# LepistaBioinformatics/classeq2

Measured on AMD Instinct MI355X. Metric: query placements/sec, 10k-leaf tree, 150 bp reads, higher is better.
Workload: dtype u64

## Files before the change

classeq2_amd/_abi.py:

```python

import ctypes as C

ABI_VERSION = 2
SETS_EXPLICIT, SETS_LEAVES = 0, 1

KIND_ROOT, KIND_NODE, KIND_LEAF = 0, 1, 2
NO_PARENT = (1 << 64) - 1

HAS_MAX_ITERATIONS = 1
HAS_MIN_MATCH_COVERAGE = 2
HAS_REMOVE_INTERSECTION = 4

(
    UNCLASSIFIABLE_NO_MATCH,
    UNCLASSIFIABLE_NO_ROOT,
    UNCLASSIFIABLE_COVERAGE,
    UNCLASSIFIABLE_LEVEL1,
    IDENTITY_FOUND,
    MAX_RESOLUTION,
    INCONCLUSIVE,
    ERR_TOO_FEW_KMERS,
    ERR_MAX_ITER,
    ERR_ROOT_NO_CHILDREN,
    ERR_INVALID_BASE,
    ERR_READ_TOO_LONG,
) = range(12)

STATUS_NAMES = [
    "UNCLASSIFIABLE_NO_MATCH",
    "UNCLASSIFIABLE_NO_ROOT",
    "UNCLASSIFIABLE_COVERAGE",
    "UNCLASSIFIABLE_LEVEL1",
    "IDENTITY_FOUND",
    "MAX_RESOLUTION",
    "INCONCLUSIVE",
    "ERR_TOO_FEW_KMERS",
    "ERR_MAX_ITER",
    "ERR_ROOT_NO_CHILDREN",
    "ERR_INVALID_BASE",
    "ERR_READ_TOO_LONG",
]


class Node(C.Structure):
    _fields_ = [
        ("id", C.c_uint64),
        ("parent", C.c_uint64),
        ("first_child", C.c_uint32),
        ("n_children", C.c_uint32),
        ("kind", C.c_uint8),
        ("has_children", C.c_uint8),
        ("pad_", C.c_uint8 * 6),
    ]


class DbDesc(C.Structure):
    _fields_ = [
        ("abi_version", C.c_uint32),
        ("n_nodes", C.c_uint32),
        ("nodes", C.POINTER(Node)),
        ("k_size", C.c_uint64),
        ("m_size", C.c_uint64),
        ("n_buckets", C.c_uint64),
        ("bucket_key", C.POINTER(C.c_uint64)),
        ("bucket_kmer_off", C.POINTER(C.c_uint64)),
        ("n_kmers", C.c_uint64),
        ("kmer_hash", C.POINTER(C.c_uint64)),
        ("kmer_node_off", C.POINTER(C.c_uint64)),
        ("node_ids", C.POINTER(C.c_uint64)),
        ("node_set_kind", C.c_uint32),
        ("pad_", C.c_uint32),
    ]


BUILD_REFERENCE_HEADER_SHIFT, BUILD_FORWARD_ONLY, BUILD_LEAVES_ONLY = 1, 2, 4


class BuildDesc(C.Structure):
    _fields_ = [
        ("abi_version", C.c_uint32),
        ("n_nodes", C.c_uint32),
        ("nodes", C.POINTER(Node)),
        ("k_size", C.c_uint64),
        ("m_size", C.c_uint64),
        ("n_records", C.c_uint32),
        ("flags", C.c_uint32),
        ("bases", C.c_void_p),
        ("offsets", C.POINTER(C.c_uint64)),
        ("leaf_id", C.POINTER(C.c_uint64)),
    ]


class KmersInfo(C.Structure):
    _fields_ = [
        ("n_windows", C.c_uint64),
        ("n_kmers", C.c_uint64),
        ("n_leaf_postings", C.c_uint64),
        ("n_node_ids", C.c_uint64),
        ("n_buckets", C.c_uint64),
        ("peak_device_bytes", C.c_uint64),
        ("ms_hash", C.c_double),
        ("ms_sort", C.c_double),
        ("ms_group", C.c_double),
        ("ms_d2h", C.c_double),
        ("ms_expand", C.c_double),
        ("sort_passes", C.c_uint32),
        ("full_key", C.c_uint32),
    ]


class Params(C.Structure):
    _fields_ = [
        ("flags", C.c_uint32),
        ("max_iterations", C.c_int32),
        ("min_match_coverage", C.c_double),
        ("remove_intersection", C.c_uint8),
        ("pad_", C.c_uint8 * 7),
    ]


class Placement(C.Structure):
    _fields_ = [
        ("status", C.c_uint8),
        ("pad_", C.c_uint8 * 3),
        ("one", C.c_int32),
        ("rest", C.c_int32),
        ("levels", C.c_uint32),
        ("clade_id", C.c_uint64),
    ]


class QueryStats(C.Structure):
    _fields_ = [
        ("n_query_kmers", C.c_uint32),
        ("n_matched", C.c_uint32),
        ("n_with_root", C.c_uint32),
        ("index_bytes", C.c_uint32),
        ("leaf_postings", C.c_uint64),
    ]


class DbInfo(C.Structure):
    _fields_ = [
        ("n_nodes", C.c_uint32),
        ("max_depth", C.c_uint32),
        ("max_nonleaf_arity", C.c_uint32),
        ("k_size", C.c_uint32),
        ("m_size", C.c_uint32),
        ("n_buckets", C.c_uint32),
        ("n_kmers", C.c_uint64),
        ("n_closed_kmers", C.c_uint64),
        ("table_slots", C.c_uint64),
        ("postings_words", C.c_uint64),
        ("hbm_bytes", C.c_uint64),
        ("max_read_kmers", C.c_uint32),
        ("device", C.c_int32),
        ("format", C.c_uint32),
        ("binary_tree", C.c_uint32),
        ("direct_table", C.c_uint32),
        ("n_tip_sets", C.c_uint32),
        ("scratch_slots", C.c_uint32),
# ... 103 lines not shown
```

classeq2_amd/csrc/cls_api.cpp:

```cpp
#include <hip/hip_runtime.h>
#include <ctype.h>
#include <stdio.h>
#include <stdlib.h>
#include <string.h>

#include <algorithm>
#include <mutex>
#include <new>
#include <string>
#include <thread>
#include <vector>

#include "cls_db.h"
#include "cls_device.h"
#include "cls_kernels.h"
#include "cls_pair.h"
#include "cls_place.h"
#include "cls_tally.h"
#include "cls_tuning.h"

namespace {

thread_local std::string g_err;

int fail(int code, const std::string& msg) {
    g_err = msg;
    return code;
}

#define CLS_HIP(expr)                                                                       \
    do {                                                                                    \
        hipError_t e_ = (expr);                                                             \
        if (e_ != hipSuccess) return fail(CLS_E_HIP, std::string(#expr) + ": " + hipGetErrorString(e_)); \
    } while (0)

struct Workspace {
    uint32_t* ptr = nullptr;
    uint64_t words = 0;
    hipEvent_t done = nullptr;
    hipStream_t stream = nullptr;
    uint64_t seq = 0;
    int launching = 0;
    bool busy = false;
    bool recorded = false;
};
struct TimedPair {
    hipEvent_t t0 = nullptr, t1 = nullptr;
    bool pending = false;
    bool in_use = false;
};
constexpr size_t MAX_WS_SLOTS = 8;
constexpr size_t MAX_TIMED_PAIRS = 256;

struct CallSlot {
    hipStream_t stream = nullptr;
    void *d_bases = nullptr, *d_off = nullptr, *d_out = nullptr, *d_stats = nullptr;
    uint64_t cap_bytes = 0;
    uint32_t cap_reads = 0, cap_stats = 0;
    bool busy = false;
};

cls::PlaceParams resolve(const cls_params* p) {
    cls::PlaceParams r;
    r.max_iterations = (p && (p->flags & CLS_HAS_MAX_ITERATIONS)) ? p->max_iterations : 1000;
    r.remove_intersection = (p && (p->flags & CLS_HAS_REMOVE_INTERSECTION)) ? (p->remove_intersection != 0) : 0;
    double c = 0.7;
    if (p && (p->flags & CLS_HAS_MIN_MATCH_COVERAGE)) {
        c = p->min_match_coverage;
        if (c > 1.0) c = 1.0; else if (c < 0.0) c = 0.0;
    }
    r.min_match_coverage = c;
    return r;
}

}

struct cls_db {
    int device = 0;
    int n_cu = 0;
    cls::DbDev dev{};
    cls_db_info info{};
    void* d_nodes = nullptr;
    void* d_kids = nullptr;
    void* d_table = nullptr;
    void* d_postings = nullptr;
    void* d_postings2 = nullptr;
    void* d_bucket_key = nullptr;
    void* d_mz_bucket = nullptr;
    void* d_direct = nullptr;
    void* d_direct16 = nullptr;
    void* d_sets = nullptr;
    void* d_sets2 = nullptr;
    std::mutex ws_mu;
    uint64_t max_read_len = 0;
    double kernel_ms_sum = 0.0;
    uint64_t kernel_launches = 0;
    std::vector<Workspace> ws;
    std::vector<TimedPair> timed;
    uint64_t ws_seq = 0;
    std::vector<CallSlot> calls;
    struct TreeRow { uint64_t id; uint32_t pre, size; };
    std::vector<TreeRow> tree_rows;
};

namespace cls {
Tuning& tuning() {
    static Tuning t;
    return t;
}
}
namespace {
struct Knob { const char* name; int cls::Tuning::*field; };
const Knob KNOBS[] = {
    {"no_fast", &cls::Tuning::no_fast}, {"no_order", &cls::Tuning::no_order}, {"force_list", &cls::Tuning::force_list},
    {"no_mask_halves", &cls::Tuning::no_mask_halves}, {"no_fat_direct", &cls::Tuning::no_fat_direct}, {"no_tile", &cls::Tuning::no_tile}, {"tile_pass_codes", &cls::Tuning::tile_pass_codes}, {"tile_set_words", &cls::Tuning::tile_set_words}, {"time_class", &cls::Tuning::time_class}, {"tile_one_per_cu", &cls::Tuning::tile_one_per_cu}, {"tile_min_kmers", &cls::Tuning::tile_min_kmers}, {"no_tile_order", &cls::Tuning::no_tile_order}, {"tile_deal", &cls::Tuning::tile_deal}, {"blocks_per_cu", &cls::Tuning::blocks_per_cu}, {"key_blocks_per_cu", &cls::Tuning::key_blocks_per_cu},
    {"long_blocks_per_cu", &cls::Tuning::long_blocks_per_cu}, {"order_mode", &cls::Tuning::order_mode},
    {"order_windows", &cls::Tuning::order_windows}, {"order_both_strands", &cls::Tuning::order_both_strands},
    {"order_block_shift", &cls::Tuning::order_block_shift}, {"order_sample_shift", &cls::Tuning::order_sample_shift},
    {"profile_stop", &cls::Tuning::profile_stop}, {"timing", &cls::Tuning::timing},
    {"build_full_key", &cls::Tuning::build_full_key}, {"tally_no_wave_combine", &cls::Tuning::tally_no_wave_combine},
};
}

extern "C" int cls_set_tuning(const char* name, int value) {
    if (!name) return fail(CLS_E_INVALID_ARG, "cls_set_tuning: null name");
    for (const Knob& k : KNOBS)
        if (strcmp(k.name, name) == 0) { cls::tuning().*(k.field) = value; return CLS_OK; }
    return fail(CLS_E_INVALID_ARG, std::string("cls_set_tuning: unknown knob ") + name);
}

extern "C" void cls_tuning_from_env(void) {
    for (const Knob& k : KNOBS) {
        std::string var = "CLS_";
        for (const char* c = k.name; *c; ++c) var += (char)toupper((unsigned char)*c);
        if (const char* v = getenv(var.c_str())) cls::tuning().*(k.field) = *v ? atoi(v) : 1;
    }
}

extern "C" const char* cls_last_error(void) { return g_err.c_str(); }
extern "C" void cls_internal_set_error(const char* msg) { g_err = msg ? msg : ""; }

extern "C" const char* cls_version(void) { return "classeq2_amd 0.1.0 gfx950 abi1"; }

extern "C" int cls_device_count(void) {
    int n = 0;
    if (hipGetDeviceCount(&n) != hipSuccess) return 0;
    return n;
}

extern "C" void cls_db_destroy(cls_db* db) {
    if (!db) return;
    int prev = 0;
    bool have_prev = hipGetDevice(&prev) == hipSuccess;
    (void)hipSetDevice(db->device);
    for (auto& w : db->ws) {
        if (w.done) { if (w.recorded) (void)hipEventSynchronize(w.done); (void)hipEventDestroy(w.done); }
        if (w.ptr) (void)hipFree(w.ptr);
    }
    for (auto& t : db->timed) {
        if (t.t0) (void)hipEventDestroy(t.t0);
        if (t.t1) (void)hipEventDestroy(t.t1);
    }
    for (auto& c : db->calls) {
        if (c.stream) { (void)hipStreamSynchronize(c.stream); (void)hipStreamDestroy(c.stream); }
        for (void* p : {c.d_bases, c.d_off, c.d_out, c.d_stats}) if (p) (void)hipFree(p);
    }
    if (db->d_nodes) (void)hipFree(db->d_nodes);
    if (db->d_kids) (void)hipFree(db->d_kids);
    if (db->d_table) (void)hipFree(db->d_table);
    if (db->d_postings) (void)hipFree(db->d_postings);
    if (db->d_postings2) (void)hipFree(db->d_postings2);
    if (db->d_bucket_key) (void)hipFree(db->d_bucket_key);
    if (db->d_mz_bucket) (void)hipFree(db->d_mz_bucket);
    if (db->d_direct) (void)hipFree(db->d_direct);
    if (db->d_direct16) (void)hipFree(db->d_direct16);
    if (db->d_sets) (void)hipFree(db->d_sets);
    if (db->d_sets2) (void)hipFree(db->d_sets2);
    if (have_prev) (void)hipSetDevice(prev);
    delete db;
}

static int encode(const cls_db_desc* d, cls::EncodedDb& E, const char* who) {
    std::string err;
    int rc = cls::encode_db(d, E, err);
    if (rc != CLS_OK) return fail(rc, std::string(who) + ": " + err);
    if (E.format == cls::FMT_LIST && E.postings.size() >= (1ULL << 32)) return fail(CLS_E_BAD_DB, std::string(who) + ": sorted-list postings exceed 2^32 words");
    return CLS_OK;
}

static int upload(const cls::EncodedDb& E, uint32_t n_buckets, int device, cls_db** out) {
    *out = nullptr;
    int n_dev = 0;
    if (hipGetDeviceCount(&n_dev) != hipSuccess || n_dev == 0)
        return fail(CLS_E_NO_DEVICE, "cls_db_create: no HIP device is visible (the placement path has no CPU fallback)");
    if (device < 0) CLS_HIP(hipGetDevice(&device));
    if (device >= n_dev) return fail(CLS_E_INVALID_ARG, "cls_db_create: device ordinal out of range");
    CLS_HIP(hipSetDevice(device));
    hipDeviceProp_t prop;
    CLS_HIP(hipGetDeviceProperties(&prop, device));
    std::vector<cls_db::TreeRow> tree_rows(E.nodes.size());
    for (size_t r = 0; r < E.nodes.size(); ++r) tree_rows[E.desc_row[r]] = {E.nodes[r].id, E.nodes[r].pre, E.nodes[r].size};
    cls_db* db = new cls_db();
    db->device = device;
    db->n_cu = prop.multiProcessorCount;
    db->tree_rows = std::move(tree_rows);
    auto up = [&](void** dst, const void* src, size_t bytes) -> hipError_t {
        hipError_t e = hipMalloc(dst, bytes + 64);
        if (e != hipSuccess) return e;
        return bytes ? hipMemcpy(*dst, src, bytes, hipMemcpyHostToDevice) : hipSuccess;
    };
    hipError_t e;
    if ((e = up(&db->d_nodes, E.nodes.data(), E.nodes.size() * sizeof(cls::DNode))) != hipSuccess ||
        (e = up(&db->d_kids, E.kids.data(), E.kids.size() * 4)) != hipSuccess ||
        (e = up(&db->d_table, E.table.data(), E.table.size() * sizeof(cls::Slot))) != hipSuccess ||
        (e = up(&db->d_postings, E.postings.data(), E.postings.size() * 4)) != hipSuccess ||
        (!E.postings2.empty() && (e = up(&db->d_postings2, E.postings2.data(), E.postings2.size() * 4)) != hipSuccess) ||
        (e = up(&db->d_bucket_key, E.bucket_key.data(), E.bucket_key.size() * 8)) != hipSuccess ||
        (!E.mz_bucket.empty() && (e = up(&db->d_mz_bucket, E.mz_bucket.data(), E.mz_bucket.size() * 4)) != hipSuccess) ||
        (!E.direct.empty() && (e = up(&db->d_direct, E.direct.data(), E.direct.size() * 4)) != hipSuccess) ||
        (!E.direct16.empty() && (e = up(&db->d_direct16, E.direct16.data(), E.direct16.size() * 4)) != hipSuccess) ||
        (!E.sets.empty() && (e = up(&db->d_sets, E.sets.data(), E.sets.size() * sizeof(cls::SetRec))) != hipSuccess) ||
        (!E.sets2.empty() && (e = up(&db->d_sets2, E.sets2.data(), E.sets2.size() * sizeof(cls::SetRec))) != hipSuccess)) {
        cls_db_destroy(db);
        return fail(e == hipErrorOutOfMemory ? CLS_E_NOMEM : CLS_E_HIP, std::string("cls_db_create: upload failed: ") + hipGetErrorString(e));
    }
    cls::DbDev& v = db->dev;
    v.nodes = (const cls::DNode*)db->d_nodes;
    v.kids = (const uint32_t*)db->d_kids;
    v.table = (const cls::Slot*)db->d_table;
    v.postings = (const uint32_t*)db->d_postings;
    v.postings2 = (const uint32_t*)db->d_postings2;
    v.bucket_key = (const uint64_t*)db->d_bucket_key;
    v.mz_bucket = (const uint32_t*)db->d_mz_bucket;
    v.direct = (const uint32_t*)db->d_direct;
    v.direct16 = (const uint32_t*)db->d_direct16;
    v.sets = (const cls::SetRec*)db->d_sets;
    v.sets2 = (const cls::SetRec*)db->d_sets2;
    v.table_mask = E.table.size() - 1;
    v.n_nodes = (uint32_t)E.nodes.size();
    v.n_buckets = (uint32_t)E.bucket_key.size();
    v.k = E.k;
    v.m_eff = E.m_eff;
    v.max_nonleaf_arity = E.max_nonleaf_arity;
    v.format = E.format;
    v.binary_tree = E.strictly_binary ? 1u : 0u;
    v.canonical = E.canonical ? 1u : 0u;
    v.n_sets = (uint32_t)E.sets.size();
    v.set_bits = 1;
    while (v.set_bits < 32 && (1ull << v.set_bits) < (uint64_t)E.sets.size()) ++v.set_bits;
    v.addr32 = (E.postings.size() * 4 < (1ull << 32) && E.direct.size() * 4 < (1ull << 32) && E.sets.size() * sizeof(cls::SetRec) < (1ull << 32)) ? 1u : 0u;
    cls_db_info& i = db->info;
    i.n_nodes = v.n_nodes;
    i.max_depth = E.max_depth;
    i.max_nonleaf_arity = E.max_nonleaf_arity;
    i.k_size = E.k;
    i.m_size = E.m;
    i.n_buckets = n_buckets;
    i.n_kmers = E.n_kmers;
    i.n_closed_kmers = E.n_closed;
    i.table_slots = E.table.size();
    i.postings_words = E.postings.size();
    i.hbm_bytes = E.nodes.size() * sizeof(cls::DNode) + E.table.size() * sizeof(cls::Slot) + (E.postings.size() + E.postings2.size()) * 4 + E.bucket_key.size() * 8 + E.mz_bucket.size() * 4 + E.direct.size() * 4 + E.direct16.size() * 4 + (E.sets.size() + E.sets2.size()) * sizeof(cls::SetRec);
    i.device = device;
    i.format = E.format;
    i.binary_tree = E.strictly_binary ? 1u : 0u;
    i.direct_table = E.direct.empty() ? 0u : (E.canonical ? 2u : 1u);
    i.n_tip_sets = (uint32_t)E.n_sets;
    i.fat_direct_table = E.direct16.empty() ? 0u : 1u;
    *out = db;
    return CLS_OK;
}

extern "C" int cls_db_create(const cls_db_desc* d, int device, cls_db** out) {
    if (!out) return fail(CLS_E_INVALID_ARG, "cls_db_create: out is null");
    *out = nullptr;
    try {
        cls::EncodedDb E;
        int rc = encode(d, E, "cls_db_create");
        if (rc != CLS_OK) return rc;
        return upload(E, (uint32_t)d->n_buckets, device, out);
    } catch (const std::bad_alloc&) {
        return fail(CLS_E_NOMEM, "cls_db_create: out of host memory");
    } catch (const std::exception& ex) {
        return fail(CLS_E_INTERNAL, std::string("cls_db_create: ") + ex.what());
    } catch (...) {
        return fail(CLS_E_INTERNAL, "cls_db_create: unknown exception");
    }
}

extern "C" int cls_db_validate(const cls_db_desc* d) {
    try {
        cls::EncodedDb E;
        std::string err;
        int rc = cls::encode_db(d, E, err);
        if (rc != CLS_OK) return fail(rc, "cls_db_validate: " + err);
        return CLS_OK;
    } catch (const std::bad_alloc&) {
        return fail(CLS_E_NOMEM, "cls_db_validate: out of host memory");
    } catch (...) {
        return fail(CLS_E_INTERNAL, "cls_db_validate: unknown exception");
    }
}

static cls::PlacePlan device_plan(const cls_db* db, uint64_t n_bases, bool stats) {
    return cls::plan_place(db->dev, 4096, (uint32_t)db->n_cu, stats, (uint32_t)(2 * n_bases), n_bases ? 4096 : 0);
}

static uint64_t declared_read_len(const cls_db* db) {
    std::lock_guard<std::mutex> g(const_cast<cls_db*>(db)->ws_mu);
    return db->max_read_len;
}

extern "C" int cls_db_info_get(const cls_db* db, cls_db_info* info) {
    if (!db || !info) return fail(CLS_E_INVALID_ARG, "cls_db_info_get: null argument");
    try {
        uint32_t cap[cls::N_LISTS];
        device_plan(db, declared_read_len(db), false).class_caps(cap);
        cls_db* mdb = const_cast<cls_db*>(db);
        std::lock_guard<std::mutex> g(mdb->ws_mu);
        *info = db->info;
        info->scratch_slots = (uint32_t)db->ws.size();
        info->max_read_kmers = *std::max_element(cap, cap + cls::N_LISTS);
        return CLS_OK;
    } catch (...) {
        return fail(CLS_E_INTERNAL, "cls_db_info_get: unknown exception");
    }
}

extern "C" int cls_db_info_get2(const cls_db* db, void* info, size_t info_size) {
    if (!db || !info) return fail(CLS_E_INVALID_ARG, "cls_db_info_get2: null argument");
    cls_db_info full;
    const int rc = cls_db_info_get(db, &full);
    if (rc != CLS_OK) return rc;
    memcpy(info, &full, info_size < sizeof(full) ? info_size : sizeof(full));
    return CLS_OK;
}

static void harvest(cls_db* db, bool wait) {
    for (auto& t : db->timed) {
        if (!t.pending) continue;
        if (wait ? hipEventSynchronize(t.t1) != hipSuccess : hipEventQuery(t.t1) != hipSuccess) continue;
        float ms = 0.f;
        if (hipEventElapsedTime(&ms, t.t0, t.t1) == hipSuccess) { db->kernel_ms_sum += ms; db->kernel_launches++; }
        t.pending = false;
    }
}

static size_t acquire_timed(cls_db* db) {
    harvest(db, false);
    for (size_t i = 0; i < db->timed.size(); ++i)
        if (!db->timed[i].pending && !db->timed[i].in_use && db->timed[i].t0) { db->timed[i].in_use = true; return i; }
    if (db->timed.size() >= MAX_TIMED_PAIRS) return SIZE_MAX;
    TimedPair t;
    if (hipEventCreate(&t.t0) != hipSuccess) return SIZE_MAX;
    if (hipEventCreate(&t.t1) != hipSuccess) { (void)hipEventDestroy(t.t0); return SIZE_MAX; }
    t.in_use = true;
    db->timed.push_back(t);
    return db->timed.size() - 1;
}

static int acquire_ws(cls_db* db, uint64_t words, hipStream_t stream, size_t* slot, Workspace* use) {
    std::unique_lock<std::mutex> g(db->ws_mu);
    for (;;) {
        size_t oldest = SIZE_MAX;
        for (size_t i = 0; i < db->ws.size(); ++i) {
            Workspace& w = db->ws[i];
            if (w.busy && w.recorded && w.launching == 0 && hipEventQuery(w.done) == hipSuccess) w.busy = false;
            const bool same_stream = w.busy && w.recorded && w.launching == 0 && w.stream == stream && stream != hipStreamPerThread;
            if ((!w.busy || same_stream) && w.words >= words) {
                w.busy = true; w.recorded = false; w.launching = 1; w.stream = stream; w.seq = ++db->ws_seq;
                *slot = i; *use = w;
                return CLS_OK;
            }
            if (w.busy && w.recorded && w.launching == 0 && (oldest == SIZE_MAX || w.seq < db->ws[oldest].seq)) oldest = i;
        }
        for (size_t i = 0; i < db->ws.size();) {
            Workspace& w = db->ws[i];
            if (!w.busy) {
                (void)hipEventDestroy(w.done);
                (void)hipFree(w.ptr);
                db->ws.erase(db->ws.begin() + (ptrdiff_t)i);
                oldest = SIZE_MAX;
            } else ++i;
        }
        if (db->ws.size() < MAX_WS_SLOTS) break;
        if (oldest == SIZE_MAX) {
            for (size_t i = 0; i < db->ws.size(); ++i)
                if (db->ws[i].busy && db->ws[i].recorded && db->ws[i].launching == 0 && (oldest == SIZE_MAX || db->ws[i].seq < db->ws[oldest].seq)) oldest = i;
        }
        if (oldest == SIZE_MAX) {
            g.unlock();
            std::this_thread::yield();
            g.lock();
            continue;
        }
        hipEvent_t ev = db->ws[oldest].done;
        g.unlock();
        if (hipEventSynchronize(ev) != hipSuccess) return fail(CLS_E_HIP, "hipEventSynchronize failed while waiting for a scratch slot");
        g.lock();
    }
    Workspace w;
    if (hipMalloc((void**)&w.ptr, words * 4) != hipSuccess) return fail(CLS_E_NOMEM, "scratch workspace allocation failed");
    if (hipEventCreateWithFlags(&w.done, hipEventDisableTiming) != hipSuccess) {
        (void)hipFree(w.ptr);
        return fail(CLS_E_HIP, "hipEventCreate failed");
    }
    w.words = words;
    w.busy = true;
    w.recorded = false;
    w.launching = 1;
    w.stream = stream;
    w.seq = ++db->ws_seq;
    db->ws.push_back(w);
    *slot = db->ws.size() - 1;
    *use = w;
    return CLS_OK;
}

static constexpr uint64_t HARD_MAX_READ_LEN = 1ull << 25;

extern "C" int cls_db_set_max_read_len(cls_db* db, uint64_t n_bases) {
    if (!db) return fail(CLS_E_INVALID_ARG, "cls_db_set_max_read_len: null handle");
    if (n_bases > HARD_MAX_READ_LEN) return fail(CLS_E_INVALID_ARG, "cls_db_set_max_read_len: at most 2^25 bases per read");
    std::lock_guard<std::mutex> g(db->ws_mu);
    db->max_read_len = n_bases;
    return CLS_OK;
}

static int place_device(cls_db* db, const void* d_bases, const void* d_offsets, uint32_t n, const cls_params* params,
                        void* d_out, void* d_stats, hipStream_t stream, uint32_t long_cap, uint32_t n_long) {
    const cls::PlaceParams prm = resolve(params);
    const cls::PlacePlan plan = cls::plan_place(db->dev, n, (uint32_t)db->n_cu, d_stats != nullptr, long_cap, n_long);
    size_t slot = 0;
    Workspace use;
    int rc = acquire_ws(db, (plan.ws_bytes + 3) / 4, stream, &slot, &use);
    if (rc != CLS_OK) return rc;
    size_t tp = SIZE_MAX;
    hipEvent_t t0 = nullptr, t1 = nullptr;
    {
        std::lock_guard<std::mutex> g(db->ws_mu);
        tp = acquire_timed(db);
        if (tp != SIZE_MAX) { t0 = db->timed[tp].t0; t1 = db->timed[tp].t1; }
    }
    hipError_t e = cls::launch_place(db->dev, prm, plan, (const uint8_t*)d_bases, (const uint64_t*)d_offsets, n,
                                     (cls_placement*)d_out, (cls_query_stats*)d_stats, use.ptr, stream, t0, t1);
    bool record_failed = false;
    {
        std::lock_guard<std::mutex> g(db->ws_mu);
        if (tp != SIZE_MAX) { db->timed[tp].pending = (e == hipSuccess); db->timed[tp].in_use = false; }
        for (size_t i = 0; i < db->ws.size(); ++i)
            if (db->ws[i].ptr == use.ptr) { slot = i; break; }
        record_failed = hipEventRecord(db->ws[slot].done, stream) != hipSuccess;
    }
    if (record_failed) (void)hipStreamSynchronize(stream);
    {
        std::lock_guard<std::mutex> g(db->ws_mu);
        for (size_t i = 0; i < db->ws.size(); ++i)
            if (db->ws[i].ptr == use.ptr) { slot = i; break; }
        db->ws[slot].launching = 0;
        db->ws[slot].recorded = !record_failed;
        if (record_failed) db->ws[slot].busy = false;
    }
    if (e != hipSuccess) return fail(CLS_E_HIP, std::string("kernel launch failed: ") + hipGetErrorString(e));
    return CLS_OK;
}

extern "C" int cls_place_batch_device(cls_db* db, const void* d_bases, const void* d_offsets, uint32_t n,
                                      const cls_params* params, void* d_out, void* d_stats, void* hip_stream) {
    if (!db) return fail(CLS_E_INVALID_ARG, "cls_place_batch_device: null handle");
    if (n == 0) return CLS_OK;
    if (!d_offsets || !d_out) return fail(CLS_E_INVALID_ARG, "cls_place_batch_device: null buffer");
    int prev = 0;
    CLS_HIP(hipGetDevice(&prev));
    if (prev != db->device) CLS_HIP(hipSetDevice(db->device));
    int rc;
    try {
        uint64_t max_len;
        { std::lock_guard<std::mutex> g(db->ws_mu); max_len = db->max_read_len; }
        rc = place_device(db, d_bases, d_offsets, n, params, d_out, d_stats, (hipStream_t)hip_stream, (uint32_t)(2 * max_len), max_len ? n : 0);
    } catch (...) {
        rc = fail(CLS_E_INTERNAL, "cls_place_batch_device: unknown exception");
    }
    if (prev != db->device) (void)hipSetDevice(prev);
    return rc;
}

extern "C" int cls_db_kernel_name(const cls_db* db, char* buf, size_t len) {
    if (!db || !buf || !len) return fail(CLS_E_INVALID_ARG, "cls_db_kernel_name: null argument");
    try {
        snprintf(buf, len, "%s", device_plan(db, declared_read_len(db), false).timed_name.c_str());
        return CLS_OK;
    } catch (...) {
        return fail(CLS_E_INTERNAL, "cls_db_kernel_name: unknown exception");
    }
}

extern "C" int cls_db_read_classes(const cls_db* db, uint64_t n_bases, int stats, cls_read_class* out, int max, int* n_out) {
    if (!db || !n_out || max < 0 || (max > 0 && !out)) return fail(CLS_E_INVALID_ARG, "cls_db_read_classes: null argument");
    if (n_bases > HARD_MAX_READ_LEN) return fail(CLS_E_INVALID_ARG, "cls_db_read_classes: at most 2^25 bases per read");
    try {
        const cls::PlacePlan plan = device_plan(db, n_bases, stats != 0);
        uint32_t cap[cls::N_LISTS];
        plan.class_caps(cap);
        int n = 0;
        uint32_t below = 0;
        for (int c = 0; c < cls::N_LISTS; ++c) {
            if (c > 0 && cap[c] <= below) continue;
            below = cap[c];
            if (n < max) {
                out[n].list = (uint32_t)c;
                out[n].max_kmers = cap[c];
                snprintf(out[n].kernel, sizeof out[n].kernel, "%s", plan.class_kernel_name(db->dev, c, stats != 0).c_str());
            }
            ++n;
        }
        *n_out = n;
        return CLS_OK;
    } catch (...) {
        return fail(CLS_E_INTERNAL, "cls_db_read_classes: unknown exception");
    }
}

extern "C" int cls_db_kernel_time(cls_db* db, double* sum_ms, uint64_t* launches, int reset) {
    if (!db) return fail(CLS_E_INVALID_ARG, "cls_db_kernel_time: null handle");
    std::lock_guard<std::mutex> g(db->ws_mu);
    harvest(db, true);
    if (sum_ms) *sum_ms = db->kernel_ms_sum;
    if (launches) *launches = db->kernel_launches;
    if (reset) { db->kernel_ms_sum = 0.0; db->kernel_launches = 0; }
    return CLS_OK;
}

static int check_host_args(const char* bases, const uint64_t* offsets, uint32_t n, const cls_placement* out) {
    if (!offsets || !out || (!bases && offsets[n] != offsets[0])) return fail(CLS_E_INVALID_ARG, "cls_place_batch: null buffer");
    for (uint32_t i = 0; i < n; ++i)
        if (offsets[i] > offsets[i + 1]) return fail(CLS_E_INVALID_ARG, "cls_place_batch: offsets not monotone");
    return CLS_OK;
}

static int place_host_checked(cls_db* db, const char* bases, const uint64_t* offsets, uint32_t n, const cls_params* params,
                              cls_placement* out, cls_query_stats* stats);

static int place_host(cls_db* db, const char* bases, const uint64_t* offsets, uint32_t n, const cls_params* params,
                      cls_placement* out, cls_query_stats* stats) {
    if (!db) return fail(CLS_E_INVALID_ARG, "cls_place_batch: null handle");
    if (n == 0) return CLS_OK;
    const int rc = check_host_args(bases, offsets, n, out);
    if (rc != CLS_OK) return rc;
    return place_host_checked(db, bases, offsets, n, params, out, stats);
}

static int place_host_checked(cls_db* db, const char* bases, const uint64_t* offsets, uint32_t n, const cls_params* params,
                              cls_placement* out, cls_query_stats* stats) {
    int prev = 0;
    CLS_HIP(hipGetDevice(&prev));
    CLS_HIP(hipSetDevice(db->device));
    const uint32_t chunk_reads = 256u << 10;
    const uint64_t chunk_bytes = 256ull << 20;
    const bool two = n > chunk_reads || offsets[n] - offsets[0] > chunk_bytes;
    size_t ci[2] = {0, 0};
    CallSlot cs[2];
    const int n_slots = two ? 2 : 1;
    {
        std::lock_guard<std::mutex> g(db->ws_mu);
        for (int k = 0; k < n_slots; ++k) {
            size_t i = 0;
            while (i < db->calls.size() && db->calls[i].busy) ++i;
            if (i == db->calls.size()) db->calls.emplace_back();
            db->calls[i].busy = true;
            ci[k] = i;
            cs[k] = db->calls[i];
        }
    }
    auto cleanup = [&]() {
        for (int k = 0; k < n_slots; ++k) if (cs[k].stream) (void)hipStreamSynchronize(cs[k].stream);
        std::lock_guard<std::mutex> g(db->ws_mu);
        for (int k = 0; k < n_slots; ++k) { cs[k].busy = false; db->calls[ci[k]] = cs[k]; }
        (void)hipSetDevice(prev);
    };
#define CLS_TRY(expr)                                                                                     \
    do {                                                                                                  \
        hipError_t e_ = (expr);                                                                           \
        if (e_ != hipSuccess) { cleanup(); return fail(e_ == hipErrorOutOfMemory ? CLS_E_NOMEM : CLS_E_HIP, std::string(#expr) + ": " + hipGetErrorString(e_)); } \
    } while (0)
    try {
        std::vector<uint64_t> rel[2];
        struct Pending { bool on = false; uint32_t first = 0, cnt = 0; } pend[2];
        auto copy_out = [&](int k) -> hipError_t {
            if (!pend[k].on) return hipSuccess;
            pend[k].on = false;
            hipError_t e = hipMemcpyAsync(out + pend[k].first, cs[k].d_out, (size_t)pend[k].cnt * sizeof(cls_placement), hipMemcpyDeviceToHost, cs[k].stream);
            if (e == hipSuccess && stats)
                e = hipMemcpyAsync(stats + pend[k].first, cs[k].d_stats, (size_t)pend[k].cnt * sizeof(cls_query_stats), hipMemcpyDeviceToHost, cs[k].stream);
            return e;
        };
        int turn = 0;
        for (uint32_t first = 0; first < n; turn ^= (n_slots - 1)) {
            CallSlot& c = cs[turn];
            uint32_t cnt = 0;
            while (first + cnt < n && cnt < chunk_reads && (cnt == 0 || offsets[first + cnt + 1] - offsets[first] <= chunk_bytes)) ++cnt;
            const uint64_t nbytes = offsets[first + cnt] - offsets[first];
            CLS_TRY(copy_out(turn));
            if (!c.stream) CLS_TRY(hipStreamCreateWithFlags(&c.stream, hipStreamNonBlocking));
            if (nbytes > c.cap_bytes || !c.d_bases) {
                CLS_TRY(hipStreamSynchronize(c.stream));
                if (c.d_bases) { (void)hipFree(c.d_bases); c.d_bases = nullptr; c.cap_bytes = 0; }
                const uint64_t want = std::max<uint64_t>(nbytes + nbytes / 4, 1 << 16);
                CLS_TRY(hipMalloc(&c.d_bases, want));
                c.cap_bytes = want;
            }
            if (cnt > c.cap_reads) {
                CLS_TRY(hipStreamSynchronize(c.stream));
                for (void** pp : {&c.d_off, &c.d_out, &c.d_stats}) if (*pp) { (void)hipFree(*pp); *pp = nullptr; }
                c.cap_reads = c.cap_stats = 0;
                const uint32_t want = (uint32_t)std::max<uint64_t>((uint64_t)cnt + cnt / 4, 1024);
                CLS_TRY(hipMalloc(&c.d_off, ((size_t)want + 1) * 8));
                CLS_TRY(hipMalloc(&c.d_out, (size_t)want * sizeof(cls_placement)));
                c.cap_reads = want;
            }
            if (stats && c.cap_stats < c.cap_reads) {
                CLS_TRY(hipStreamSynchronize(c.stream));
                if (c.d_stats) { (void)hipFree(c.d_stats); c.d_stats = nullptr; }
                CLS_TRY(hipMalloc(&c.d_stats, (size_t)c.cap_reads * sizeof(cls_query_stats)));
                c.cap_stats = c.cap_reads;
            }
            std::vector<uint64_t>& ro = rel[turn];
            ro.resize((size_t)cnt + 1);
            for (uint32_t i = 0; i <= cnt; ++i) ro[i] = offsets[first + i] - offsets[first];
            uint64_t longest = 1;
            uint32_t n_long = 1;
            for (uint32_t i = 0; i < cnt; ++i) {
                const uint64_t len = ro[i + 1] - ro[i];
                const uint64_t nk = len < db->dev.k ? 0 : 2 * (len - db->dev.k + 1);
                longest = std::max(longest, std::min(len, HARD_MAX_READ_LEN));
                if (nk > cls::MAX_READ_KMERS) ++n_long;
// ... 1141 lines not shown
```

classeq2_amd/csrc/cls_db.cpp:

```cpp
#include "cls_db.h"

#include "cls_murmur.h"
#include "cls_tuning.h"

#include <stdio.h>
#include <stdlib.h>
#include <string.h>

#include <algorithm>
#include <atomic>
#include <chrono>
#include <exception>
#include <functional>
#include <mutex>
#include <thread>

namespace cls {

namespace {

struct WorkerError {
    std::mutex mu;
    std::exception_ptr first;
    void capture() { std::lock_guard<std::mutex> g(mu); if (!first) first = std::current_exception(); }
// ... 382 lines not shown
                    while (!stk.empty()) {
                        const uint32_t x = stk.back(); stk.pop_back();
                        pos[x] = next++;
                        const uint32_t l = L[x], r = R[x];
                        if (l) { span_lo[l] = span_lo[x]; span_hi[l] = x; }
                        if (r) { span_lo[r] = x; span_hi[r] = span_hi[x]; }
                        const bool left_heavy = (x - span_lo[x]) >= (span_hi[x] - x);
                        if (left_heavy) { if (r) stk.push_back(r); if (l) stk.push_back(l); }
                        else { if (l) stk.push_back(l); if (r) stk.push_back(r); }
                    }
                }
                auto at = [&](uint32_t i) { return (uint32_t)(base + pos[i]); };
                for (uint32_t i = 1; i < n; ++i) {
                    uint32_t* t = &recs[(size_t)at(i) * 4];
                    t[0] = tip[i - 1];
                    t[1] = L[i] ? at(L[i]) : 0;
                    t[2] = tip[i];
                    t[3] = R[i] ? at(R[i]) : 0;
                    if (mask_halves) {
                        uint32_t* u = &recs2[(size_t)at(i) * 4];
                        u[0] = t[0]; u[1] = t[1]; u[2] = t[2]; u[3] = t[3];
                        const uint32_t l0 = span_lo[i], r1 = span_hi[i];
                        if (tip[i - 1] - tip[l0] < MASK_HALF_SPAN) {
                            uint32_t bits = 0;
                            for (uint32_t j = l0; j < i; ++j) bits |= 1u << (tip[j] - tip[l0]);
                            u[0] = tip[i - 1] | MASK_HALF; u[1] = bits;
                        }
                        if (tip[r1 - 1] - tip[i] < MASK_HALF_SPAN) {
                            uint32_t bits = 0;
                            for (uint32_t j = i; j < r1; ++j) bits |= 1u << (tip[j] - tip[i]);
                            u[2] = tip[i] | MASK_HALF; u[3] = bits;
                        }
                    }
                }
                if (mask_halves && n && tip[n - 1] - tip[0] < MASK_HALF_SPAN) {
                    uint32_t bits = 0;
                    for (uint32_t j = 0; j < n; ++j) bits |= 1u << (tip[j] - tip[0]);
                    set_mask[g + 1] = bits;
                }
                uint32_t lg = 0;
                while (lg < 31 && (1u << lg) <= n) ++lg;
                SetRec& sr = E.sets[g + 1];
                sr.x = root ? at(root) : 0;
                sr.vlo_lg = n ? ((lg << DIRECT_TIP_BITS) | tip[0]) : 0xFFFFFFFFu;
                sr.vhi_root = (n ? tip[n - 1] : 0u) | ((w[0] & POST_HAS_ROOT) ? 0x80000000u : 0u);
                sr.n_leaf = w[1];
            }
        });
        E.postings.swap(recs);
        E.postings2.swap(recs2);
        if (mask_halves) {
            E.sets2.assign(E.sets.begin(), E.sets.end());
            parallel_chunks(NS + 1, nt, [&](unsigned, uint64_t lo, uint64_t hi) {
                for (uint64_t g = lo; g < hi; ++g)
                    if (set_mask[g]) { E.sets2[g].x = set_mask[g]; E.sets2[g].vhi_root |= FAT_X_IS_BITS; }
            });
        }
        lap("split trees");
    }
    uint64_t cap = 16;
    while (cap < 2 * NK) cap <<= 1;
    if (cap >= (1ULL << 32)) { err = "k-mer table exceeds 2^32 slots"; return CLS_E_BAD_DB; }
    const uint64_t mask = cap - 1;
    const bool split = E.format == FMT_SPLIT;
    E.table.assign(cap, split ? Slot{0, 0} : Slot{0, SLOT_EMPTY});
    {
        uint64_t* raw = reinterpret_cast<uint64_t*>(E.table.data());
        const uint64_t empty = split ? 0ull : SLOT_EMPTY;
        auto tier_of = [&](uint32_t sid) -> uint64_t { const uint32_t lg = E.sets[sid].vlo_lg >> DIRECT_TIP_BITS; return lg <= 3 ? 0 : lg <= 6 ? 1 : lg <= 9 ? 2 : 3; };
        parallel_chunks(NK, nt, [&](unsigned, uint64_t lo, uint64_t hi) {
            for (uint64_t j = lo; j < hi; ++j) {
                const uint64_t h = d->kmer_hash[j];
                const uint64_t val = split ? ((uint64_t)set_of[j] | (((uint64_t)bucket_of[j] | (tier_of(set_of[j]) << TIER_SHIFT)) << 32))
                                           : ((kmer_off[j] << LOC_BUCKET_BITS) | bucket_of[j]);
                for (uint64_t i = h & mask;; i = (i + 1) & mask) {
                    uint64_t expect = empty;
                    if (__atomic_load_n(&raw[2 * i + 1], __ATOMIC_RELAXED) == empty &&
                        __atomic_compare_exchange_n(&raw[2 * i + 1], &expect, val, false, __ATOMIC_ACQ_REL, __ATOMIC_RELAXED)) {
                        raw[2 * i] = h;
                        break;
                    }
                }
            }
        });
        std::atomic<bool> has_dup{false};
        std::atomic<uint64_t> dup{0};
        parallel_chunks(cap, nt, [&](unsigned, uint64_t lo, uint64_t hi) {
            for (uint64_t s = lo; s < hi; ++s) {
                if (raw[2 * s + 1] == empty) continue;
                const uint64_t h = raw[2 * s];
                for (uint64_t i = h & mask; i != s; i = (i + 1) & mask)
                    if (raw[2 * i] == h) { dup.store(h, std::memory_order_relaxed); has_dup.store(true, std::memory_order_relaxed); break; }
            }
        });
        if (has_dup.load()) { err = "k-mer hash " + std::to_string(dup.load()) + " occurs more than once in the index (unsupported)"; return CLS_E_BAD_DB; }
    }
    lap("hash table");
    if (split && d->k_size <= DIRECT_MAX_K && E.n_sets < SET_ID_MASK) {
        const uint32_t K = (uint32_t)d->k_size, M = (uint32_t)std::min<uint64_t>(d->m_size, d->k_size);
        const uint64_t n_codes = 1ULL << (2 * K);
        E.direct.assign(n_codes, 0);
        const TSlot* tab = reinterpret_cast<const TSlot*>(E.table.data());
        std::atomic<bool> foreign{false};
        std::atomic<uint64_t> found{0};
        parallel_chunks(n_codes, nt, [&](unsigned, uint64_t lo, uint64_t hi) {
            static const char LETTER[4] = {'A', 'C', 'T', 'G'};
            constexpr int B = 32;
            char buf[DIRECT_MAX_K + 1];
            uint64_t hs[B];
            uint64_t cnt = 0;
            for (uint64_t c0 = lo; c0 < hi; c0 += B) {
                const int nb = (int)std::min<uint64_t>(B, hi - c0);
                for (int q = 0; q < nb; ++q) {
                    const uint64_t code = c0 + q;
                    for (uint32_t i = 0; i < K; ++i) buf[i] = LETTER[(code >> (2 * i)) & 3];
                    hs[q] = murmur3_h1_bytes(buf, K);
                    __builtin_prefetch(&tab[hs[q] & mask]);
                }
                for (int q = 0; q < nb; ++q) {
                    const uint64_t code = c0 + q, h = hs[q];
                    for (uint64_t i = h & mask; tab[i].set != 0; i = (i + 1) & mask) {
                        if (tab[i].hash != h) continue;
                        for (uint32_t t = 0; t < M; ++t) buf[t] = LETTER[(code >> (2 * t)) & 3];
                        if (d->bucket_key[tab[i].bucket & (uint32_t)LOC_BUCKET_MASK] != (M ? murmur3_h1_bytes(buf, M) : 0ull)) foreign = true;
                        E.direct[code] = tab[i].set | (tab[i].bucket & ~SET_ID_MASK);
                        ++cnt;
                        break;
                    }
                }
            }
            found += cnt;
        });
        if (foreign.load() || found.load() != NK) HugeVec<uint32_t>().swap(E.direct);
        if (!E.direct.empty()) {
            std::atomic<bool> asym{false};
            parallel_chunks(n_codes, nt, [&](unsigned, uint64_t lo, uint64_t hi) {
                for (uint64_t code = lo; code < hi && !asym.load(std::memory_order_relaxed); ++code) {
                    uint64_t rc = 0;
                    for (uint32_t i = 0; i < K; ++i) rc |= (((code >> (2 * i)) & 3) ^ 2) << (2 * (K - 1 - i));
                    if (rc > code && E.direct[code] != E.direct[rc]) asym = true;
                }
            });
            E.canonical = !asym.load();
            if (K <= FAT_DIRECT_MAX_K && !tuning().no_fat_direct) {
                E.direct16.resize(4 * n_codes);
                parallel_chunks(n_codes, nt, [&](unsigned, uint64_t lo, uint64_t hi) {
                    for (uint64_t code = lo; code < hi; ++code) {
                        const uint32_t e = E.direct[code];
                        const SetRec& sr = E.sets[e & SET_ID_MASK];
                        uint32_t* o = &E.direct16[4 * code];
                        o[0] = sr.x; o[1] = sr.vlo_lg; o[2] = sr.vhi_root; o[3] = e;
                        const uint32_t bits = set_mask.empty() ? 0u : set_mask[e & SET_ID_MASK];
                        if (bits) { o[0] = bits; o[2] |= FAT_X_IS_BITS; }
                    }
                });
            }
        }
    }
    lap("direct table");
    E.bucket_key.assign(d->bucket_key, d->bucket_key + d->n_buckets);
    if (E.bucket_key.empty()) E.bucket_key.push_back(0);
    {
        const uint32_t M = (uint32_t)std::min<uint64_t>(d->m_size, d->k_size);
        std::unordered_map<uint64_t, uint32_t> by_key;
        bool distinct = true;
        for (uint64_t b = 0; b < d->n_buckets; ++b) distinct &= by_key.emplace(d->bucket_key[b], (uint32_t)b).second;
        if (M <= MZ_TABLE_MAX_M && distinct) {
            static const char LETTER[4] = {'A', 'C', 'T', 'G'};
            E.mz_bucket.assign((size_t)1 << (2 * M), MZ_NO_BUCKET);
            char buf[MZ_TABLE_MAX_M + 1];
            for (uint32_t code = 0; code < E.mz_bucket.size(); ++code) {
                for (uint32_t t = 0; t < M; ++t) buf[t] = LETTER[(code >> (2 * t)) & 3];
                const auto it = by_key.find(M ? murmur3_h1_bytes(buf, M) : 0ull);
                if (it != by_key.end()) E.mz_bucket[code] = it->second;
            }
        }
    }
    E.k = (uint32_t)d->k_size;
    E.m = (uint32_t)std::min<uint64_t>(d->m_size, UINT32_MAX);
    E.m_eff = (uint32_t)std::min<uint64_t>(d->m_size, d->k_size);
    E.n_kmers = NK;
    E.n_closed = n_closed.load();
    E.root_has_children = d->nodes[0].has_children != 0;
    return CLS_OK;
}

}

extern "C" int cls_db_debug_mask_halves(const cls_db_desc* d, uint64_t* counts) {
    try {
        cls::EncodedDb E;
        std::string err;
        const int rc = cls::encode_db(d, E, err);
        if (rc != CLS_OK) return rc;
        using namespace cls;
        counts[0] = counts[1] = counts[2] = 0;
        if (E.format != FMT_SPLIT || E.postings2.empty()) return CLS_OK;
        if (E.postings2.size() != E.postings.size()) return CLS_E_INTERNAL;
        const TipRec* recs = reinterpret_cast<const TipRec*>(E.postings.data());
        const TipRec* rec2 = reinterpret_cast<const TipRec*>(E.postings2.data());
        const uint64_t n_recs = E.postings.size() / 4;
        std::function<void(uint32_t, uint32_t, int, std::vector<uint32_t>&)> part = [&](uint32_t end_tip, uint32_t x, int side, std::vector<uint32_t>& out) {
            if (!x) { out.push_back(end_tip); return; }
            const TipRec& t = recs[x];
            part(t.tip_prev, t.l, 0, out);
            part(t.tip, t.r, 1, out);
            (void)side;
        };
        std::vector<uint32_t> tips;
        for (uint64_t x = 1; x + 1 < n_recs; ++x) {
            const TipRec& t = recs[x];
            const TipRec& u = rec2[x];
            if (t.tip_prev == 0 && t.tip == 0 && t.l == 0 && t.r == 0) continue;
            ++counts[0];
            for (int side = 0; side < 2; ++side) {
                const uint32_t end_tip = side ? t.tip : t.tip_prev, sub = side ? t.r : t.l;
                const uint32_t uw = side ? u.tip : u.tip_prev, ux = side ? u.r : u.l;
                tips.clear();
                part(end_tip, sub, side, tips);
                if (!std::is_sorted(tips.begin(), tips.end()) || (side ? tips.front() : tips.back()) != end_tip) return CLS_E_INTERNAL;
                const bool narrow = tips.back() - tips.front() < MASK_HALF_SPAN;
                if (uw & MASK_HALF) {
                    uint32_t bits = 0;
                    for (uint32_t v : tips) bits |= 1u << (v - tips.front());
                    if (!narrow || (uw & ~MASK_HALF) != end_tip || ux != bits) return CLS_E_INTERNAL;
                    ++counts[1];
                } else {
                    if (narrow || uw != end_tip || ux != sub) return CLS_E_INTERNAL;
                    ++counts[2];
                }
            }
        }
        return CLS_OK;
    } catch (const std::bad_alloc&) {
        return CLS_E_NOMEM;
    } catch (...) {
        return CLS_E_INTERNAL;
    }
}

extern "C" int cls_db_debug_members(const cls_db_desc* d, const uint64_t* hashes, const uint64_t* clade_ids, uint64_t n, uint8_t* out) {
    try {
        cls::EncodedDb E;
        std::string err;
        const int rc = cls::encode_db(d, E, err);
        if (rc != CLS_OK) return rc;
        using namespace cls;
        std::vector<std::pair<uint64_t, uint32_t>> id2row(E.nodes.size());
        for (uint32_t r = 0; r < E.nodes.size(); ++r) id2row[r] = {E.nodes[r].id, r};
        std::sort(id2row.begin(), id2row.end());
        const uint64_t mask = E.table.size() - 1;
        std::vector<uint32_t> tips, stk;
        for (uint64_t i = 0; i < n; ++i) {
            auto it = std::lower_bound(id2row.begin(), id2row.end(), std::make_pair(clade_ids[i], (uint32_t)0));
            if (it == id2row.end() || it->first != clade_ids[i]) { out[i] = 3; continue; }
            const DNode& c = E.nodes[it->second];
            const uint64_t h = hashes[i];
            bool found = false, has_root = false, closed = true;
            tips.clear();
            if (E.format == FMT_SPLIT) {
                const TSlot* tab = reinterpret_cast<const TSlot*>(E.table.data());
                for (uint64_t s = h & mask; tab[s].set != 0; s = (s + 1) & mask) {
                    if (tab[s].hash != h) continue;
                    found = true;
                    const SetRec& sr = E.sets[tab[s].set];
                    has_root = (sr.vhi_root >> 31) != 0;
                    if (sr.vlo_lg != 0xFFFFFFFFu) {
                        const uint32_t lo = sr.vlo_lg & DIRECT_TIP_MASK, hi = sr.vhi_root & 0x7FFFFFFFu;
                        if (!sr.x) { tips.push_back(lo); if (hi != lo) return CLS_E_INTERNAL; }
                        else {
                            const TipRec* recs = reinterpret_cast<const TipRec*>(E.postings.data());
                            std::vector<std::pair<uint32_t, int>> st{{sr.x, 0}};
                            tips.push_back(lo);
                            while (!st.empty()) {
                                auto [x, phase] = st.back();
                                st.pop_back();
                                const TipRec& t = recs[x];
                                if (phase == 0) { st.push_back({x, 1}); if (t.l) st.push_back({t.l, 0}); }
                                else { if (tips.back() != t.tip_prev) return CLS_E_INTERNAL; tips.push_back(t.tip); if (t.r) st.push_back({t.r, 0}); }
                            }
                            if (tips.back() != hi) return CLS_E_INTERNAL;
                        }
                    }
                    break;
                }
            } else {
                for (uint64_t s = h & mask; E.table[s].loc != SLOT_EMPTY; s = (s + 1) & mask) {
                    if (E.table[s].hash != h) continue;
                    found = true;
                    const uint32_t* w = &E.postings[E.table[s].loc >> LOC_BUCKET_BITS];
                    has_root = (w[0] & POST_HAS_ROOT) != 0;
                    closed = (w[0] & POST_CLOSED) != 0;
                    tips.assign(w + POST_HEADER_WORDS, w + POST_HEADER_WORDS + (w[0] & POST_LEN_MASK));
                    break;
                }
            }
            if (!found) { out[i] = 2; continue; }
            bool in = false;
            if (c.pre == 0) in = has_root;
            else if (closed) { auto t = std::lower_bound(tips.begin(), tips.end(), c.pre); in = t != tips.end() && *t < c.pre + c.size; }
            else in = std::binary_search(tips.begin(), tips.end(), c.pre);
            out[i] = in ? 1 : 0;
        }
        return CLS_OK;
    } catch (...) {
        return CLS_E_INTERNAL;
    }
}
```

classeq2_amd/csrc/cls_db.h:

```cpp
#pragma once
#include <stdlib.h>
#include <sys/mman.h>

#include <new>
#include <string>
#include <vector>

#include "cls_device.h"

namespace cls {

constexpr uint64_t MAX_K = 1024;

template <class T>
struct HugeAlloc {
    using value_type = T;
    HugeAlloc() = default;
    template <class U> HugeAlloc(const HugeAlloc<U>&) {}
    T* allocate(size_t n) {
        const size_t bytes = n * sizeof(T);
        if (bytes < (8u << 20)) { void* p = malloc(bytes ? bytes : 1); if (!p) throw std::bad_alloc(); return static_cast<T*>(p); }
        const size_t huge = 2u << 20, padded = (bytes + huge - 1) & ~(huge - 1);
        void* p = aligned_alloc(huge, padded);
        if (!p) throw std::bad_alloc();
        (void)madvise(p, padded, MADV_HUGEPAGE);
        return static_cast<T*>(p);
    }
    void deallocate(T* p, size_t) { free(p); }
    template <class U> bool operator==(const HugeAlloc<U>&) const { return true; }
    template <class U> bool operator!=(const HugeAlloc<U>&) const { return false; }
};
template <class T> using HugeVec = std::vector<T, HugeAlloc<T>>;

struct EncodedDb {
    std::vector<DNode> nodes;
    std::vector<uint32_t> desc_row;
    std::vector<uint32_t> kids;
    HugeVec<Slot> table;
    HugeVec<uint32_t> postings2;
    HugeVec<uint32_t> postings;
    uint32_t format = FMT_LIST;
    bool strictly_binary = false;
    bool canonical = false;
    std::vector<uint64_t> bucket_key;
    std::vector<uint32_t> mz_bucket;
    HugeVec<SetRec> sets;
    HugeVec<SetRec> sets2;
    HugeVec<uint32_t> direct;
    HugeVec<uint32_t> direct16;
    uint32_t k = 0, m = 0, m_eff = 0;
    uint32_t max_depth = 0, max_nonleaf_arity = 0;
    uint64_t n_kmers = 0, n_closed = 0;
    uint64_t n_sets = 0;
    bool root_has_children = false;
};

int encode_db(const cls_db_desc* d, EncodedDb& E, std::string& err);

}
```

classeq2_amd/csrc/cls_device.h:

```cpp
#pragma once
#include <stdint.h>

#include "cls_place.h"

namespace cls {

struct DNode {
    uint32_t pre;
    uint32_t size;
    uint32_t first_child;
    uint32_t n_nonleaf;
    uint64_t id;
    uint32_t split;
    uint32_t flags;
};
static_assert(sizeof(DNode) == 32, "DNode");

struct Slot {
    uint64_t hash;
    uint64_t loc;
};
static_assert(sizeof(Slot) == 16, "Slot");
constexpr uint64_t SLOT_EMPTY = ~0ULL;
struct TSlot {
    uint64_t hash;
    uint32_t set;
    uint32_t bucket;
};
constexpr int TIER_SHIFT = 30;
constexpr uint32_t MZ_TABLE_MAX_M = 8;
constexpr uint32_t MZ_NO_BUCKET = 0xFFFFFFFFu;
constexpr uint32_t SET_ID_MASK = (1u << TIER_SHIFT) - 1;
static_assert(sizeof(TSlot) == 16, "TSlot");
constexpr int LOC_BUCKET_BITS = 24;
constexpr uint64_t LOC_BUCKET_MASK = (1ULL << LOC_BUCKET_BITS) - 1;

constexpr uint32_t POST_HAS_ROOT = 1u << 31;
constexpr uint32_t POST_CLOSED = 1u << 30;
constexpr uint32_t POST_LEN_MASK = (1u << 30) - 1;
constexpr uint32_t POST_HEADER_WORDS = 2;

struct SetRec {
    uint32_t x;
    uint32_t vlo_lg;
    uint32_t vhi_root;
    uint32_t n_leaf;
};
static_assert(sizeof(SetRec) == 16, "SetRec");
constexpr uint32_t DIRECT_MAX_K = 15;
constexpr uint32_t FAT_DIRECT_MAX_K = 12;
constexpr uint32_t DIRECT_TIP_BITS = 27;
constexpr uint32_t DIRECT_TIP_MASK = (1u << DIRECT_TIP_BITS) - 1;
struct TipRec {
    uint32_t tip_prev;
    uint32_t l;
    uint32_t tip;
    uint32_t r;
};
static_assert(sizeof(TipRec) == 16, "TipRec");
constexpr uint32_t MASK_HALF = 0x80000000u;
constexpr uint32_t MASK_HALF_SPAN = 32;
constexpr uint32_t FAT_X_IS_BITS = 0x40000000u;

enum : uint32_t { FMT_LIST = 0, FMT_SPLIT = 1 };

struct DbDev {
    const DNode* nodes;
    const uint32_t* kids;
    const Slot* table;
    const uint32_t* postings;
    const uint32_t* postings2;
    const uint64_t* bucket_key;
    const uint32_t* mz_bucket;
    const uint32_t* direct;
    const uint32_t* direct16;
    const SetRec* sets;
    const SetRec* sets2;
    uint64_t table_mask;
    uint32_t n_nodes;
    uint32_t n_buckets;
    uint32_t k;
    uint32_t m_eff;
    uint32_t max_nonleaf_arity;
    uint32_t format;
    uint32_t addr32;
    uint32_t binary_tree;
    uint32_t canonical;
    uint32_t set_bits;
    uint32_t n_sets;
};

struct PlaceParams {
    int32_t max_iterations;
    uint32_t remove_intersection;
    double min_match_coverage;
};

constexpr uint32_t MAX_READ_KMERS = 64 * 8 * 16;

}
```

classeq2_amd/csrc/cls_kernels.h:

```cpp
#pragma once
#include <hip/hip_runtime.h>

#include <string>
#include <tuple>
#include <type_traits>
#include <utility>

#include "cls_device.h"

namespace cls {

template <int V> using Int = std::integral_constant<int, V>;
template <class F> auto with_bool(bool b, F&& f) { return b ? f(std::true_type{}) : f(std::false_type{}); }
template <class... V> std::string instance_name(const char* kernel, V...) {
    auto arg = [](auto v) { if constexpr (std::is_same_v<decltype(v), bool>) return std::string(v ? "true" : "false"); else return std::to_string(v); };
    std::string s = std::string(kernel) + "<";
    const char* sep = "";
    ((s += sep + arg(V::value), sep = ", "), ...);
    return s + ">";
}
template <class F> struct Pick {
    F* fn;
    size_t smem;
    std::string name;
};
template <class F, class... V> Pick<F> pick(F* fn, size_t smem, const char* kernel, V... v) { return {fn, smem, instance_name(kernel, v...)}; }
template <class... P, class... A>
hipError_t launch_kernel(void (*kfn)(P...), dim3 grid, dim3 block, size_t smem, hipStream_t stream, A&&... a) {
    static_assert(sizeof...(P) == sizeof...(A), "launch_kernel: one argument per kernel parameter");
    const void* f = reinterpret_cast<const void*>(kfn);
    hipError_t e = smem > 64 * 1024 ? hipFuncSetAttribute(f, hipFuncAttributeMaxDynamicSharedMemorySize, (int)smem) : hipSuccess;
    if (e == hipSuccess) {
        std::tuple<P...> v{P{std::forward<A>(a)}...};
        e = std::apply([&](auto&... x) { void* args[] = {&x...}; return hipLaunchKernel(f, grid, block, args, smem, stream); }, v);
    }
    if (e != hipSuccess) (void)hipGetLastError();
    return e;
}

struct TileCfg {
    uint32_t threads, grid, lookups, bases, cap_kmers, set_words, cap_entries;
    size_t smem;
    uint64_t scratch_off;
};
constexpr int TILE_MAX_SUB = 3;
struct TilePlan {
    TileCfg sub[TILE_MAX_SUB];
    uint32_t n_sub;
    TileCfg whole;
    uint64_t scratch_words;
    std::string name;
};

constexpr int N_LISTS = 8;

struct PlacePlan {
    uint32_t grid[2];
    uint32_t grid_blk;
    uint32_t grid_key;
    bool ordered;
    uint64_t keys_off_words;
    uint64_t sort_off_words;
    size_t sort_bytes;
    uint64_t child_off_words;
    uint32_t grid_long;
    uint32_t long_cap;
    uint32_t long_arity;
    uint64_t long_set;
    uint64_t long_stride_words;
    uint64_t long_off_words;
    uint32_t max_kmers;
    bool blk;
    bool tiled;
    TilePlan tile;
    uint32_t tile_from;
    uint64_t tile_off_words;
    enum Timed : uint8_t { TIME_CLASS0, TIME_BLOCK, TIME_TILE } timed;
    std::string timed_name;
    uint64_t ws_bytes;
    void class_caps(uint32_t (&cap)[N_LISTS]) const;
    std::string class_kernel_name(const DbDev& db, int c, bool stats) const;
};
bool tile_usable(const DbDev& db);
TilePlan tile_plan(const DbDev& db, bool stats, uint32_t from_kmers, uint32_t max_kmers, uint32_t n_reads, uint32_t n_cu);
std::string tile_kernel_name(const DbDev& db, bool stats, const TileCfg& c);
hipError_t tile_launch(const DbDev& db, const PlaceParams& prm, const TilePlan& p, bool stats, const uint8_t* d_bases, const uint64_t* d_offsets,
                       const uint32_t* const* sub_lists, const uint32_t* const* sub_lens, uint32_t* big_list, uint32_t* big_len,
                       cls_placement* d_out, cls_query_stats* d_stats, uint32_t* spill_list, uint32_t* spill_len, uint32_t* scratch, bool ordered, hipStream_t stream);
PlacePlan plan_place(const DbDev& db, uint32_t n_reads, uint32_t n_cu, bool stats, uint32_t long_cap, uint32_t n_long);
hipError_t launch_place(const DbDev& db, const PlaceParams& prm, const PlacePlan& plan, const uint8_t* d_bases,
                        const uint64_t* d_offsets, uint32_t n_reads, cls_placement* d_out, cls_query_stats* d_stats,
                        uint32_t* d_ws, hipStream_t stream, hipEvent_t ev_start, hipEvent_t ev_stop);

}
```

classeq2_amd/csrc/cls_kernels.hip:

```cpp
#include <hip/hip_runtime.h>
#include <stdlib.h>

#include <algorithm>
#include <type_traits>

#include "cls_device.h"
#include "cls_devutil.h"
#include "cls_kernels.h"
#include "cls_murmur.h"
#include "cls_sort.h"
#include "cls_tuning.h"

namespace cls {

namespace {

constexpr int WAVES_PER_BLOCK = 4;
#ifndef MIN_WAVES_PER_EU
#define MIN_WAVES_PER_EU 4
#endif
#ifndef FAST_MIN_WAVES
#define FAST_MIN_WAVES 5
#endif
#ifndef CLS_NARROW_CANON_BITS
// ... 1340 lines not shown
    uint32_t nm_lane = 0;
#pragma unroll
    for (int s = 0; s < LS; ++s) {
        sid[s] &= SET_ID_MASK;
        if (sid[s] != 0) {
            uint32_t pos = (key[s] * 2654435761u) >> (32 - tb);
#pragma unroll 1
            for (;;) {
                const uint32_t old = atomicCAS(&cx.set[pos], SET_EMPTY, key[s]);
                if (old == SET_EMPTY) break;
                if (old == key[s]) { sid[s] = 0; kw[s] = 0; break; }
                pos = (pos + 1) & ((1u << tb) - 1);
            }
        }
        nm_lane += sid[s] != 0 ? kw[s] : 0u;
    }
    if (profile_stop == 1) { write_record(out, r, 0xFE, (int32_t)(sid[0] + sid[LS - 1]), 0, 0, 0); return; }
    uint32_t pos[LS];
    uint32_t owner = 0;
#pragma unroll
    for (int s = 0; s < LS; ++s) {
        pos[s] = 0;
        if (sid[s] != 0) {
            uint32_t p = (sid[s] * 2654435761u) >> (32 - tb);
#pragma unroll 1
            for (;;) {
                const uint32_t old = atomicCAS(&cx.gkey[p], SET_EMPTY, sid[s]);
                if (old == SET_EMPTY) { owner |= 1u << s; break; }
                if (old == sid[s]) break;
                p = (p + 1) & ((1u << tb) - 1);
            }
            atomicAdd(&cx.gcnt[p], kw[s]);
            pos[s] = p;
        }
    }
    wave_sync();
#pragma unroll
    for (int s = 0; s < LS; ++s) pos[s] = ((owner >> s) & 1u) ? cx.gcnt[pos[s]] : 0u;
    wave_sync();
    const uint4* __restrict__ sets = reinterpret_cast<const uint4*>(db.sets2 ? db.sets2 : db.sets);
    uint32_t cnt = nm_lane;
    uint64_t leafp = 0;
    uint32_t n_sets = 0;
    constexpr int G = LS <= 4 ? LS : 4;
#pragma unroll
    for (int g0 = 0; g0 < LS; g0 += G) {
        uint4 sr[G];
#pragma unroll
        for (int i = 0; i < G; ++i) {
            const int s = g0 + i;
            const bool own = s < LS && ((owner >> s) & 1u);
            if constexpr (FAT) {
                const FatRec fr = frec[s < LS ? s : 0];
                sr[i] = own ? uint4{fr.x, fr.vlo_lg, fr.vhi_root, 0u} : uint4{0u, 0xFFFFFFFFu, 0u, 0u};
                if (STATS && own) sr[i].w = ldx<uint4, ADDR32>(sets, sid[s < LS ? s : 0]).w;
            } else {
                sr[i] = ldx<uint4, ADDR32>(sets, own ? sid[s < LS ? s : 0] : 0u);
                if (STATS && own) ib += 16;
            }
        }
#pragma unroll
        for (int i = 0; i < G; ++i) {
            const int s = g0 + i;
            if (s >= LS) continue;
            const uint32_t w = pos[s];
            cnt += ((sr[i].z >> 31) * w) << 16;
            if (STATS) leafp += (uint64_t)w * sr[i].w;
            const bool live = ((owner >> s) & 1u) && sr[i].y != 0xFFFFFFFFu;
            const uint64_t m = __ballot(live);
            if (live)
                cx.stage[n_sets + popc64(m & ((1ull << lane) - 1))] = uint4{sr[i].y & DIRECT_TIP_MASK, sr[i].z & DIRECT_TIP_MASK, sr[i].x,
                                                                              w | ((sr[i].z & FAT_X_IS_BITS) << 1)};
            n_sets += popc64(m);
        }
    }
    cnt = wave_sum(cnt);
    const uint32_t n_m = cnt & 0xFFFFu, n_root = cnt >> 16;
    if (STATS) {
        for (int o = 32; o > 0; o >>= 1) leafp += ((uint64_t)__shfl_xor((uint32_t)(leafp >> 32), o) << 32) | __shfl_xor((uint32_t)leafp, o);
        put_stats(nk, n_m, n_root, leafp);
    }
    if (profile_stop == 2) { write_record(out, r, 0xFE, (int32_t)n_sets, 0, 0, 0); return; }
    if (n_m == 0) { put_index_bytes(); write_record(out, r, CLS_UNCLASSIFIABLE_NO_MATCH, 0, 0, 0, 0); return; }
    if (n_root == 0) { put_index_bytes(); write_record(out, r, CLS_UNCLASSIFIABLE_NO_ROOT, 0, 0, 0, 0); return; }
    snode_t P = load_node(db.nodes, 0);
    if (STATS && lane == 0) ib += 32;
    if (!(P.s[7] & 1u)) { put_index_bytes(); write_record(out, r, CLS_ERR_ROOT_NO_CHILDREN, 0, 0, 0, 0); return; }
    {
        const double expected = round((double)n_m * prm.min_match_coverage);
        const uint64_t exp_usize = (expected != expected) ? 0ull : (uint64_t)expected;
        if ((uint64_t)n_root < exp_usize) { put_index_bytes(); write_record(out, r, CLS_UNCLASSIFIABLE_COVERAGE, (int32_t)n_root, 0, 0, 0); return; }
    }
    bool in_registers = false;
    if constexpr (!POLY) in_registers = uniform(n_sets) <= 128;
    constexpr bool REG2 = !POLY || MODE != 2;
    if (in_registers) descend_groups<ADDR32, POLY, STATS, false, REG2>(db, prm, cx, n_sets, P, r, out, ib);
    else descend_groups<ADDR32, POLY, STATS, true, REG2>(db, prm, cx, n_sets, P, r, out, ib);
    put_index_bytes();
}

template <int SLOTS, int SET_BITS, bool STATS, bool ADDR32, int MODE, bool POLY>
__global__ __launch_bounds__(64 * WAVES_PER_BLOCK, SLOTS > 5 ? FAST_MIN_WAVES_WIDE : POLY ? FAST_MIN_WAVES_POLY : FAST_MIN_WAVES) void place_fast_kernel(
    DbDev db, PlaceParams prm, const uint8_t* __restrict__ bases, const uint64_t* __restrict__ offsets,
    const uint32_t* __restrict__ list, const uint32_t* __restrict__ list_len, uint32_t list_n, uint32_t xcd_chunks,
    cls_placement* __restrict__ out, cls_query_stats* __restrict__ stats, uint32_t ascii_cap, uint32_t profile_stop) {
    extern __shared__ __align__(16) uint8_t smem[];
    const uint32_t wave = threadIdx.x >> 6;
    const uint32_t packed_words = MODE == 2 ? 0u : ((ascii_cap >> 4) + 2 + 3) & ~3u;
    constexpr bool FITS = (12u << SET_BITS) >= 16u * 64 * ((MODE == 1 || MODE == 4) ? (SLOTS + 1) / 2 : SLOTS);
    if constexpr (FITS) {
    const uint32_t per_wave = ascii_cap + 4u * packed_words + (12u << SET_BITS) + (POLY ? 12u * FAST_MAX_ARITY + 16u : 0u);
    FastCtx cx;
    cx.ascii = smem + wave * per_wave;
    cx.packed = reinterpret_cast<uint32_t*>(cx.ascii + ascii_cap);
    cx.set = cx.packed + packed_words;
    cx.gkey = cx.set + (1u << SET_BITS);
    cx.gcnt = cx.gkey + (1u << SET_BITS);
    cx.stage = reinterpret_cast<uint4*>(cx.set);
    cx.ccnt = cx.gcnt + (1u << SET_BITS);
    cx.conly = cx.ccnt + FAST_MAX_ARITY;
    cx.cpre = cx.conly + FAST_MAX_ARITY;
    if (xcd_chunks && SLOTS > FAST_SLOTS_NARROW && *list_len == 0) return;
    const uint32_t n_list = xcd_chunks ? list_n : *list_len;
    const uint32_t xcd = blockIdx.x & 7u, bpx = gridDim.x >> 3;
    const uint32_t chunk = xcd_chunks ? (n_list + 7u) >> 3 : n_list;
    const uint32_t first = xcd_chunks ? (blockIdx.x >> 3) * WAVES_PER_BLOCK + wave : blockIdx.x * WAVES_PER_BLOCK + wave;
    const uint32_t stride = (xcd_chunks ? bpx : gridDim.x) * WAVES_PER_BLOCK;
    const uint32_t origin = xcd_chunks ? xcd * chunk : 0u;
    constexpr uint32_t cap = 64 * SLOTS;
    for (uint32_t ql = first; ql < chunk; ql += stride) {
        const uint32_t q = origin + ql;
        if (q >= n_list) break;
        const uint32_t r = list[q];
        const uint64_t b0 = offsets[r], b1 = offsets[r + 1];
        if (xcd_chunks) {
            const uint64_t L64 = b1 - b0;
            if (L64 >= db.k && 2 * (L64 - db.k + 1) > cap) continue;
            if (SLOTS > FAST_SLOTS_NARROW && (L64 < db.k || 2 * (L64 - db.k + 1) <= 64 * FAST_SLOTS_NARROW)) continue;
        }
        place_read_fast<SLOTS, SET_BITS, STATS, ADDR32, MODE, POLY>(db, prm, cx, bases, b0, b1, r, out, stats, profile_stop);
        wave_sync();
    }
    }
}

__device__ __forceinline__ uint64_t make_order_key(uint32_t key_mode, uint32_t median, uint32_t mh_spec, uint32_t mh_all, uint32_t block_shift, uint32_t set_bits) {
    if (key_mode == 1) return ((uint64_t)(mh_all >> 12) << set_bits) | median;
    return ((uint64_t)(median >> block_shift) << 16) | (mh_spec >> 16);
}

template <int SLOTS, bool ADDR32, bool FWD, bool HASHED>
__global__ __launch_bounds__(64 * WAVES_PER_BLOCK) void order_key_kernel(DbDev db, const uint8_t* __restrict__ bases,
                                                                       const uint64_t* __restrict__ offsets, uint32_t n_reads,
                                                                       uint64_t* __restrict__ keys, uint32_t* __restrict__ idx,
                                                                       uint32_t ascii_cap, uint32_t key_mode,
                                                                       uint32_t block_shift, uint32_t sample_shift, uint32_t fwd_only,
                                                                       uint32_t key_cap) {
    extern __shared__ __align__(16) uint8_t smem[];
    const uint32_t wave = threadIdx.x >> 6, lane = threadIdx.x & 63;
    const uint32_t packed_words = HASHED ? 0u : ((ascii_cap >> 4) + 2 + 3) & ~3u;
    const uint32_t per_wave = ascii_cap + 4u * packed_words + 16u;
    FastCtx cx;
    cx.ascii = smem + wave * per_wave;
    cx.packed = reinterpret_cast<uint32_t*>(cx.ascii + ascii_cap);
    cx.set = cx.packed + packed_words;
    cx.gkey = cx.gcnt = nullptr;
    cx.stage = nullptr;
    const uint32_t gw = blockIdx.x * WAVES_PER_BLOCK + wave;
    const uint32_t n_waves = gridDim.x * WAVES_PER_BLOCK;
    for (uint32_t r = gw; r < n_reads; r += n_waves) {
        const uint64_t b0 = offsets[r], L64 = offsets[r + 1] - b0;
        uint64_t key = ~0ull;
        if (L64 >= db.k && 2 * (L64 - db.k + 1) <= (uint64_t)key_cap) {
            const uint32_t L = (uint32_t)std::min<uint64_t>(L64, 32 * SLOTS + db.k - 1), nf = L - db.k + 1, nk = 2 * nf;
            constexpr int LS = FWD ? (SLOTS + 1) / 2 : SLOTS;
            uint32_t e[LS], code[LS], kw[LS];
            bool valid_read;
            uint32_t ib_unused = 0;
            if constexpr (HASHED) valid_read = hash_front<LS, 0, ADDR32>(db, cx, bases, b0, L, nf, FWD ? nf : nk, e, code, kw, 0, ib_unused);
            else { FatRec unused[LS]; valid_read = fast_front<LS, 0, ADDR32>(db, cx, bases, b0, L, nf, FWD ? nf : nk, e, code, kw, unused, sample_shift, FWD); }
            if (valid_read) {
                uint32_t cand = 0, n_cand = 0;
                for (uint32_t tier = 0; tier < 4 && n_cand < 4; ++tier) {
                    cand = 0; n_cand = 0;
#pragma unroll
                    for (int s = 0; s < LS; ++s) {
                        const bool c = (e[s] & SET_ID_MASK) != 0 && (e[s] >> TIER_SHIFT) <= tier;
                        cand |= (c ? 1u : 0u) << s;
                        n_cand += popc64(__ballot(c));
                    }
                }
                if (n_cand) {
                    uint32_t rank = n_cand >> 1, prefix = 0;
                    for (int bit = (int)db.set_bits - 1; bit >= 0; --bit) {
                        uint32_t c0 = 0;
#pragma unroll
                        for (int s = 0; s < LS; ++s) {
                            const uint32_t t = e[s] & SET_ID_MASK;
                            const bool z = ((cand >> s) & 1u) && ((t ^ prefix) >> (bit + 1)) == 0 && !((t >> bit) & 1u);
                            c0 += popc64(__ballot(z));
                        }
                        if (rank >= c0) { rank -= c0; prefix |= 1u << bit; }
                    }
                    uint32_t mh = 0xFFFFFFFFu, mha = 0xFFFFFFFFu;
#pragma unroll
                    for (int s = 0; s < LS; ++s) {
                        const uint32_t hsh = mix32(code[s]);
                        if ((cand >> s) & 1u) mh = hsh < mh ? hsh : mh;
                        if ((e[s] & SET_ID_MASK) != 0) mha = hsh < mha ? hsh : mha;
                    }
                    for (int o = 32; o > 0; o >>= 1) {
                        const uint32_t o1 = __shfl_xor(mh, o), o2 = __shfl_xor(mha, o);
                        mh = o1 < mh ? o1 : mh;
                        mha = o2 < mha ? o2 : mha;
                    }
                    key = make_order_key(key_mode, prefix, mh, mha, block_shift, db.set_bits);
                }
            }
            wave_sync();
        }
        if (lane == 0) { keys[r] = key; idx[r] = r; }
    }
}

template <bool ADDR32>
__global__ __launch_bounds__(64 * WAVES_PER_BLOCK) void order_key_half_kernel(DbDev db, const uint8_t* __restrict__ bases,
                                                                            const uint64_t* __restrict__ offsets, uint32_t n_reads,
                                                                            uint64_t* __restrict__ keys, uint32_t* __restrict__ idx,
                                                                            uint32_t key_mode, uint32_t block_shift,
                                                                            uint32_t key_cap) {
    constexpr uint32_t MAXL = 64 + DIRECT_MAX_K - 1 + 1;
    constexpr uint32_t WORDS = (MAXL + 15) / 16 + 2;
    __shared__ __align__(16) uint8_t s_ascii[WAVES_PER_BLOCK * 2][(MAXL + 19) & ~3u];
    __shared__ uint32_t s_packed[WAVES_PER_BLOCK * 2][WORDS];
    const uint32_t wave = threadIdx.x >> 6, lane = threadIdx.x & 63, half = lane >> 5, hl = lane & 31;
    uint8_t* ascii = s_ascii[wave * 2 + half];
    uint32_t* packed = s_packed[wave * 2 + half];
    const uint32_t k = db.k;
    const uint32_t kmask = (1u << (2 * k)) - 1u;
    const uint32_t* __restrict__ direct = db.direct;
    const uint32_t pair0 = (blockIdx.x * WAVES_PER_BLOCK + wave) * 2, stride = gridDim.x * WAVES_PER_BLOCK * 2;
    auto half_of = [&](uint64_t m) { return (uint32_t)(m >> (32 * half)); };
    for (uint32_t r0 = pair0; r0 < n_reads; r0 += stride) {
        const uint32_t r = r0 + half;
        const bool have = r < n_reads;
        const uint64_t b0 = have ? offsets[r] : 0, L64 = have ? offsets[r + 1] - b0 : 0;
        const bool keyed = have && L64 >= k && 2 * (L64 - k + 1) <= (uint64_t)key_cap;
        const uint32_t L = keyed ? (uint32_t)std::min<uint64_t>(L64, 64 + k - 1) : 0, nf = keyed ? L - k + 1 : 0;
        bool bad = false;
        for (uint32_t i = hl; i < L; i += 32) {
            uint8_t c = bases[b0 + i];
            if (c >= 'a' && c <= 'z') c -= 32;
            bad |= !(c == 'A' || c == 'C' || c == 'G' || c == 'T');
            ascii[i] = c;
        }
        const bool ok = keyed && half_of(__ballot(bad)) == 0;
        wave_sync();
        for (uint32_t w = hl; w < (L + 15) / 16 + 1; w += 32) {
            uint32_t acc = 0;
#pragma unroll
            for (int q = 0; q < 4; ++q) {
                uint32_t t = *reinterpret_cast<const uint32_t*>(ascii + 16 * w + 4 * q);
                t = (t >> 1) & 0x03030303u;
                t = (t | (t >> 6) | (t >> 12) | (t >> 18)) & 0xFFu;
                acc |= t << (8 * q);
            }
            if (w < WORDS) packed[w] = acc;
        }
        wave_sync();
        uint32_t e[2], hs[2];
#pragma unroll
        for (int s = 0; s < 2; ++s) {
            const uint32_t p = hl + 32 * s;
            const bool valid = ok && p < nf;
            const uint32_t w = valid ? p >> 4 : 0, sh = valid ? (2 * p) & 31 : 0;
            const uint32_t d0 = packed[w], d1 = packed[w + 1];
            uint32_t code = (uint32_t)((((uint64_t)d1 << 32) | d0) >> sh) & kmask;
            uint32_t rcc = __builtin_bitreverse32(code ^ (0xAAAAAAAAu & kmask));
            rcc = ((rcc >> 1) & 0x55555555u) | ((rcc & 0x55555555u) << 1);
            rcc >>= (32 - 2 * k);
            code = rcc < code ? rcc : code;
            const uint32_t v = ldx<uint32_t, ADDR32>(direct, valid ? code : 0u);
            e[s] = valid ? v : 0u;
            hs[s] = mix32(code);
        }
        uint32_t cand = 0, n_cand = 0;
        for (uint32_t tier = 0; tier < 4; ++tier) {
            const bool need = n_cand < 4;
            uint32_t c_new = 0, n_new = 0;
#pragma unroll
            for (int s = 0; s < 2; ++s) {
                const bool c = (e[s] & SET_ID_MASK) != 0 && (e[s] >> TIER_SHIFT) <= tier;
                c_new |= (c ? 1u : 0u) << s;
                n_new += (uint32_t)__popc(half_of(__ballot(c)));
            }
            if (need) { cand = c_new; n_cand = n_new; }
            if (__ballot(n_cand < 4) == 0) break;
        }
        uint32_t rank = n_cand >> 1, prefix = 0;
        for (int bit = (int)db.set_bits - 1; bit >= 0; --bit) {
            uint32_t c0 = 0;
#pragma unroll
            for (int s = 0; s < 2; ++s) {
                const uint32_t t = e[s] & SET_ID_MASK;
                const bool z = ((cand >> s) & 1u) && ((t ^ prefix) >> (bit + 1)) == 0 && !((t >> bit) & 1u);
                c0 += (uint32_t)__popc(half_of(__ballot(z)));
            }
            if (rank >= c0) { rank -= c0; prefix |= 1u << bit; }
        }
        uint32_t mh = 0xFFFFFFFFu, mha = 0xFFFFFFFFu;
#pragma unroll
        for (int s = 0; s < 2; ++s) {
            if ((cand >> s) & 1u) mh = hs[s] < mh ? hs[s] : mh;
            if ((e[s] & SET_ID_MASK) != 0) mha = hs[s] < mha ? hs[s] : mha;
        }
        for (int o = 16; o > 0; o >>= 1) {
            const uint32_t o1 = __shfl_xor(mh, o), o2 = __shfl_xor(mha, o);
            mh = o1 < mh ? o1 : mh;
            mha = o2 < mha ? o2 : mha;
        }
        if (have && hl == 0) {
            keys[r] = (ok && n_cand) ? make_order_key(key_mode, prefix, mh, mha, block_shift, db.set_bits) : ~0ull;
            idx[r] = r;
        }
        wave_sync();
    }
}

constexpr int LONG_THREADS = 256;
constexpr int LONG_STATE_WORDS = 5;

constexpr uint32_t LONG_LDS_ARITY = 256;
struct LongSh {
    uint32_t acc[4];
    unsigned long long acc64;
    uint32_t n_next;
    uint32_t n_pass, n_best, best_row;
    int32_t best_diff, best_one, best_rest;
    uint32_t cpre[LONG_LDS_ARITY + 1];
    uint32_t cnt_l[LONG_LDS_ARITY], only_l[LONG_LDS_ARITY];
};

__device__ __forceinline__ uint32_t append_slot(bool keep, uint32_t* counter) {
    const uint32_t lane = threadIdx.x & 63;
    const uint64_t m = __ballot(keep);
    if (!m) return 0;
    const int leader = __ffsll((unsigned long long)m) - 1;
    uint32_t base = 0;
    if ((int)lane == leader) base = atomicAdd(counter, (uint32_t)__popcll(m));
    base = __shfl(base, leader);
    return base + (uint32_t)__popcll(m & ((1ull << lane) - 1));
}

template <int N>
__device__ __forceinline__ void long_sum(uint32_t (&v)[N], LongSh& sh) {
    __syncthreads();
    if (threadIdx.x < N) sh.acc[threadIdx.x] = 0;
    __syncthreads();
#pragma unroll
    for (int i = 0; i < N; ++i) {
        const uint32_t w = wave_sum(v[i]);
        if ((threadIdx.x & 63) == 0 && w) atomicAdd(&sh.acc[i], w);
    }
    __syncthreads();
#pragma unroll
    for (int i = 0; i < N; ++i) v[i] = sh.acc[i];
}

template <bool SPLIT, bool STATS>
__global__ __launch_bounds__(LONG_THREADS) void place_long_kernel(DbDev db, PlaceParams prm, const uint8_t* __restrict__ bases,
                                                                  const uint64_t* __restrict__ offsets,
                                                                  const uint32_t* __restrict__ list,
                                                                  const uint32_t* __restrict__ list_len,
                                                                  cls_placement* __restrict__ out, cls_query_stats* __restrict__ stats,
                                                                  uint32_t* __restrict__ ws, uint64_t ws_stride_words, uint32_t cap,
                                                                  uint32_t set_size, uint32_t arity_pad) {
    __shared__ LongSh sh;
    constexpr uint32_t NT = LONG_THREADS;
    const uint32_t tid = threadIdx.x, lane = tid & 63;
    uint32_t* const buf0 = ws + (size_t)blockIdx.x * ws_stride_words;
    uint32_t* const buf1 = buf0 + (size_t)LONG_STATE_WORDS * cap;
    uint32_t* const cnt = buf1 + (size_t)LONG_STATE_WORDS * cap;
    uint32_t* const only = cnt + arity_pad;
    uint32_t* const set = buf1;
    uint32_t* const ent = buf0 + 4 * (size_t)cap;
    const DNode* __restrict__ nodes = db.nodes;
    const uint32_t* __restrict__ post = db.postings;
    const uint4* __restrict__ recs = reinterpret_cast<const uint4*>(db.postings);
    const uint32_t k = db.k, m_eff = db.m_eff;
    const bool rm = prm.remove_intersection != 0;
    const uint32_t n_list = *list_len;
    for (uint32_t li = blockIdx.x; li < n_list; li += gridDim.x) {
        __syncthreads();
        const uint32_t r = list[li];
        const uint64_t b0 = offsets[r], L64 = offsets[r + 1] - b0;
        auto put_stats = [&](uint32_t nk_, uint32_t nm, uint32_t nr, uint64_t lp) {
            if (STATS && stats && tid == 0) {
                uint64_t* s = reinterpret_cast<uint64_t*>(stats + r);
                s[0] = (uint64_t)nk_ | ((uint64_t)nm << 32);
                s[1] = (uint64_t)nr;
                s[2] = lp;
            }
        };
        auto record = [&](uint32_t status, int32_t one, int32_t rest, uint32_t levels, uint64_t clade) {
            if (tid == 0) {
                uint64_t* o = reinterpret_cast<uint64_t*>(out + r);
                o[0] = (uint64_t)(status & 0xFF) | ((uint64_t)(uint32_t)one << 32);
                o[1] = (uint64_t)(uint32_t)rest | ((uint64_t)levels << 32);
                o[2] = clade;
            }
        };
        if (L64 < k) { put_stats(0, 0, 0, 0); record(CLS_ERR_TOO_FEW_KMERS, 0, 0, 0, 0); continue; }
        const uint64_t nk64 = 2 * (L64 - k + 1);
        if (nk64 > cap) { put_stats(nk64 > 0xFFFFFFFFull ? 0xFFFFFFFFu : (uint32_t)nk64, 0, 0, 0); record(CLS_ERR_READ_TOO_LONG, 0, 0, 0, 0); continue; }
        const uint32_t L = (uint32_t)L64, nf = L - k + 1, nk = 2 * nf;
        bool bad = false;
        for (uint32_t i = tid; i < L; i += NT) {
            uint8_t c = bases[b0 + i];
            if (c >= 'a' && c <= 'z') c -= 32;
            bad |= !(c == 'A' || c == 'C' || c == 'G' || c == 'T');
        }
        for (uint32_t i = tid; i < set_size; i += NT) set[i] = SET_EMPTY;
        if (__syncthreads_or(bad ? 1 : 0)) { put_stats(0, 0, 0, 0); record(CLS_ERR_INVALID_BASE, 0, 0, 0, 0); continue; }
        auto kmer_char = [&](uint32_t j, uint32_t t) -> uint8_t {
            const bool rc = j >= nf;
            uint8_t c = bases[b0 + (rc ? (L - 1 - (j - nf) - t) : (j + t))];
            if (c >= 'a' && c <= 'z') c -= 32;
            return rc ? (uint8_t)(c ^ ((c & 2) ? 0x04 : 0x15)) : c;
        };
        const bool use_direct = SPLIT && db.direct != nullptr;
        for (uint32_t j = tid; j < nk; j += NT) {
            if (use_direct) {
                uint32_t code = 0;
                for (uint32_t t = 0; t < k; ++t) code |= (uint32_t)((kmer_char(j, t) >> 1) & 3u) << (2 * t);
                const uint32_t sid = db.direct[code] & SET_ID_MASK;
                uint32_t e = SET_EMPTY;
                if (sid) {
                    uint32_t pos = (code * 2654435761u) & (set_size - 1);
                    for (;;) {
                        const uint32_t old = atomicCAS(&set[pos], SET_EMPTY, code);
                        if (old == SET_EMPTY) { e = sid; break; }
                        if (old == code) break;
                        pos = (pos + 1) & (set_size - 1);
                    }
                }
                ent[j] = e;
                continue;
            }
            const uint64_t h = murmur3_h1([&](uint32_t t) { return kmer_char(j, t); }, k);
            const uint64_t mz = murmur3_h1([&](uint32_t t) { return kmer_char(j, t); }, m_eff);
            bool hit = false;
            uint64_t loc = 0;
            uint32_t tidx = 0;
            uint64_t idx = h & db.table_mask;
            for (;;) {
                const Slot sl = db.table[idx];
                if (SPLIT ? (uint32_t)sl.loc == 0u : sl.loc == SLOT_EMPTY) break;
                if (sl.hash == h) { hit = true; loc = sl.loc; tidx = (uint32_t)idx; break; }
                idx = (idx + 1) & db.table_mask;
            }
            bool ok = false;
            if (hit) {
                const uint64_t bk = db.bucket_key[SPLIT ? (uint32_t)(loc >> 32) & (uint32_t)LOC_BUCKET_MASK : (uint32_t)(loc & LOC_BUCKET_MASK)];
                ok = bk == mz;
                if (!ok) {
                    for (uint32_t jj = 0; jj < nk && !ok; ++jj)
                        ok = murmur3_h1([&](uint32_t t) { return kmer_char(jj, t); }, m_eff) == bk;
                }
            }
            uint32_t e = SET_EMPTY;
            if (hit && ok) {
                uint32_t pos = (tidx * 2654435761u) & (set_size - 1);
                for (;;) {
                    const uint32_t old = atomicCAS(&set[pos], SET_EMPTY, tidx);
                    if (old == SET_EMPTY) { e = SPLIT ? (uint32_t)loc : (uint32_t)(loc >> LOC_BUCKET_BITS); break; }
                    if (old == tidx) break;
                    pos = (pos + 1) & (set_size - 1);
// ... 221 lines not shown
    if (threadIdx.x < N_LISTS) s_cnt[threadIdx.x] = 0;
    __syncthreads();
    const uint32_t lane = threadIdx.x & 63;
    const uint32_t first = blockIdx.x * (CLASSIFY_THREADS * CLASSIFY_PER_THREAD) + threadIdx.x;
    int cls_id[CLASSIFY_PER_THREAD];
    uint32_t pos[CLASSIFY_PER_THREAD], rd[CLASSIFY_PER_THREAD];
#pragma unroll
    for (int i = 0; i < CLASSIFY_PER_THREAD; ++i) {
        const uint32_t at = first + i * CLASSIFY_THREADS;
        const uint32_t r = (order && at < n_reads) ? order[at] : at;
        rd[i] = r;
        cls_id[i] = -1;
        pos[i] = 0;
        if (at < n_reads) {
            const uint64_t L = offsets[r + 1] - offsets[r];
            const uint64_t nk = L < k ? 0 : 2 * (L - k + 1);
#pragma unroll
            for (int c = N_LISTS - 1; c >= 0; --c) if (nk <= caps.cap[c]) cls_id[i] = c;
            if (cls_id[i] < 0) {
                uint64_t* o = reinterpret_cast<uint64_t*>(out + r);
                o[0] = CLS_ERR_READ_TOO_LONG; o[1] = 0; o[2] = 0;
                if (stats) {
                    uint64_t* st = reinterpret_cast<uint64_t*>(stats + r);
                    st[0] = nk > 0xFFFFFFFFull ? 0xFFFFFFFFull : nk; st[1] = 0; st[2] = 0;
                }
            }
        }
#pragma unroll
        for (int c = 0; c < N_LISTS; ++c) {
            const uint64_t m = __ballot(cls_id[i] == c);
            if (!m) continue;
            uint32_t base = 0;
            if (lane == 0) base = atomicAdd(&s_cnt[c], (uint32_t)__popcll(m));
            base = __shfl(base, 0);
            if (cls_id[i] == c) pos[i] = base + (uint32_t)__popcll(m & ((1ull << lane) - 1));
        }
    }
    __syncthreads();
    if (threadIdx.x < N_LISTS) s_base[threadIdx.x] = s_cnt[threadIdx.x] ? atomicAdd(&counts[threadIdx.x], s_cnt[threadIdx.x]) : 0u;
    __syncthreads();
#pragma unroll
    for (int i = 0; i < CLASSIFY_PER_THREAD; ++i) {
        const int c = cls_id[i];
        if (c >= 0) lists[(size_t)c * n_reads + s_base[c] + pos[i]] = rd[i];
    }
}

}

namespace {
constexpr int N_CLASSES = 2;
constexpr int BLK_WAVES = 8, BLK_SLOTS = 16, BLK_SET_BITS = 14;
constexpr int ORDER_KEY_BITS_MAX = TIER_SHIFT + 20;
int order_key_bits(const DbDev& db) {
    const Tuning& tn = tuning();
    const int bits = tn.order_mode == 1 ? (int)db.set_bits + 20 : std::max(1, (int)db.set_bits - tn.order_block_shift) + 16;
    return std::min<int>(64, bits + 1);
}
constexpr int CLS_SLOTS[N_CLASSES] = {5, 16};
constexpr int CLS_SET_BITS[N_CLASSES] = {9, 11};
constexpr int NARROW_CANON_BITS = CLS_NARROW_CANON_BITS;

bool use_fast(const DbDev& db);
bool use_order(const DbDev& db, uint32_t n_reads) {
    return use_fast(db) && !tuning().no_order && n_reads >= 4096;
}
bool use_fast(const DbDev& db) {
    const bool front = db.direct != nullptr || (db.addr32 && db.k <= 256);
    return db.format == FMT_SPLIT && (db.binary_tree || db.max_nonleaf_arity <= FAST_MAX_ARITY) && front && !tuning().no_fast;
}
int fast_mode(const DbDev& db) { return db.direct == nullptr ? 2 : (db.direct16 && db.addr32) ? (db.canonical ? 4 : 3) : db.canonical ? 1 : 0; }
bool mode_canonical(int mode) { return mode == 1 || mode == 4; }
int set_bits_of(const DbDev& db, int c) { return (c == 0 && use_fast(db) && mode_canonical(fast_mode(db))) ? NARROW_CANON_BITS : CLS_SET_BITS[c]; }
uint32_t seq_cap_of(const DbDev& db, int c) { return (2 * (64 * CLS_SLOTS[c] / 2 + db.k) + 15) & ~15u; }
uint32_t ascii_cap_of(const DbDev& db, int c) {
    const uint32_t fwd = 64 * CLS_SLOTS[c] / 2 + db.k + 16;
    return ((db.direct ? fwd : 2 * fwd) + 15) & ~15u;
}
uint32_t child_ws_stride(const DbDev& db);
constexpr uint32_t CHILD_LDS_MAX = 256;
bool child_in_lds(const DbDev& db) { return child_ws_stride(db) != 0 && child_ws_stride(db) <= CHILD_LDS_MAX; }
size_t smem_of(const DbDev& db, int c) {
    if (use_fast(db)) {
        const uint32_t ac = ascii_cap_of(db, c);
        const uint32_t packed = db.direct ? 4u * (((ac >> 4) + 2 + 3) & ~3u) : 0u;
        return (size_t)WAVES_PER_BLOCK * (ac + packed + (12u << set_bits_of(db, c)) + (db.binary_tree ? 0u : 12u * FAST_MAX_ARITY + 16u));
    }
    return (size_t)WAVES_PER_BLOCK * (seq_cap_of(db, c) + (4u << CLS_SET_BITS[c]) + 4u * 64 * CLS_SLOTS[c]) +
           (child_in_lds(db) ? (size_t)WAVES_PER_BLOCK * 2 * child_ws_stride(db) * 4 : 0);
}

using FastFn = decltype(place_fast_kernel<CLS_SLOTS[0], CLS_SET_BITS[0], false, false, 0, false>);
using SplitFn = decltype(place_split_kernel<CLS_SLOTS[0], CLS_SET_BITS[0], false, false>);
using WaveFn = decltype(place_wave_kernel<CLS_SLOTS[0], CLS_SET_BITS[0], false, false>);
struct ClassKernel {
    FastFn* fast;
    SplitFn* split;
    WaveFn* wave;
    size_t smem;
    std::string name;
    const void* fn() const { return fast ? (const void*)fast : split ? (const void*)split : (const void*)wave; }
};
template <int SLOTS, int SET_BITS>
ClassKernel class_kernel_t(const DbDev& db, int c, bool stats) {
    const size_t smem = smem_of(db, c);
    auto fast = [&](auto... v) { return ClassKernel{place_fast_kernel<decltype(v)::value...>, nullptr, nullptr, smem, instance_name("place_fast_kernel", v...)}; };
    auto split = [&](auto... v) { return ClassKernel{nullptr, place_split_kernel<decltype(v)::value...>, nullptr, smem, instance_name("place_split_kernel", v...)}; };
    auto wave = [&](auto... v) { return ClassKernel{nullptr, nullptr, place_wave_kernel<decltype(v)::value...>, smem, instance_name("place_wave_kernel", v...)}; };
    const Int<SLOTS> sl;
    const Int<SET_BITS> sb;
    return with_bool(stats, [&](auto st) {
        if (use_fast(db)) {
            return with_bool(!db.binary_tree, [&](auto poly) {
                const std::true_type addr32;
                switch (fast_mode(db)) {
                    case 2: return fast(sl, sb, st, addr32, Int<2>{}, poly);
                    case 3: return fast(sl, sb, st, addr32, Int<3>{}, poly);
                    case 4: return fast(sl, sb, st, addr32, Int<4>{}, poly);
                }
                return with_bool(db.addr32, [&](auto a32) { return fast_mode(db) == 1 ? fast(sl, sb, st, a32, Int<1>{}, poly) : fast(sl, sb, st, a32, Int<0>{}, poly); });
            });
        }
        if (db.format == FMT_SPLIT) return with_bool(!db.binary_tree, [&](auto poly) { return split(sl, sb, st, poly); });
        return with_bool(db.max_nonleaf_arity <= 2, [&](auto binary) { return wave(sl, sb, st, binary); });
    });
}
ClassKernel class_kernel(const DbDev& db, int c, bool stats) {
    if (c == 1) return class_kernel_t<CLS_SLOTS[1], CLS_SET_BITS[1]>(db, 1, stats);
    if (set_bits_of(db, 0) != CLS_SET_BITS[0]) return class_kernel_t<CLS_SLOTS[0], NARROW_CANON_BITS>(db, 0, stats);
    return class_kernel_t<CLS_SLOTS[0], CLS_SET_BITS[0]>(db, 0, stats);
}

uint32_t child_ws_stride(const DbDev& db) {
    if (db.format == FMT_SPLIT) return db.binary_tree ? 0u : ((std::max(db.max_nonleaf_arity, 1u) + 63) & ~63u);
    return db.max_nonleaf_arity <= 2 ? 0u : ((db.max_nonleaf_arity + 63) & ~63u);
}
uint32_t blk_seq_cap(const DbDev& db) { return (2 * (64 * BLK_WAVES * BLK_SLOTS / 2 + db.k) + 15) & ~15u; }
auto block_kernel(const DbDev& db, bool stats) {
    const size_t smem = (size_t)blk_seq_cap(db) + (4u << BLK_SET_BITS) + 4u * 64 * BLK_WAVES * BLK_SLOTS + 64 +
                        (child_in_lds(db) ? (size_t)2 * child_ws_stride(db) * 4 : 0);
    auto inst = [&](auto... v) { return pick(place_block_kernel<decltype(v)::value...>, smem, "place_block_kernel", v...); };
    const bool split = db.format == FMT_SPLIT, binary = split ? db.binary_tree != 0 : db.max_nonleaf_arity <= 2;
    return with_bool(stats, [&](auto st) { return with_bool(binary, [&](auto bi) { return with_bool(split, [&](auto sp) {
        return inst(Int<BLK_WAVES>{}, Int<BLK_SLOTS>{}, Int<BLK_SET_BITS>{}, st, bi, sp);
    }); }); });
}
auto long_kernel(const DbDev& db, bool stats) {
    auto inst = [&](auto... v) { return pick(place_long_kernel<decltype(v)::value...>, 0, "place_long_kernel", v...); };
    return with_bool(db.format == FMT_SPLIT, [&](auto sp) { return with_bool(stats, [&](auto st) { return inst(sp, st); }); });
}

using KeyFn = decltype(order_key_kernel<2, true, true, false>);
using KeyHalfFn = decltype(order_key_half_kernel<true>);
struct KeyKernel {
    KeyFn* full;
    KeyHalfFn* half;
    size_t smem;
    std::string name;
    const void* fn() const { return full ? (const void*)full : (const void*)half; }
};
KeyKernel key_kernel(const DbDev& db, bool sizing) {
    const Tuning& tn = tuning();
    const bool fwd = !tn.order_both_strands, hashed = fast_mode(db) == 2;
    if (!sizing && !hashed && fwd && tn.order_windows == 64 && (uint32_t)tn.order_sample_shift >= 32)
        return with_bool(db.addr32, [&](auto a32) { return KeyKernel{nullptr, order_key_half_kernel<decltype(a32)::value>, 0, instance_name("order_key_half_kernel", a32)}; });
    const uint32_t ac = ascii_cap_of(db, 0);
    const size_t smem = (size_t)WAVES_PER_BLOCK * (ac + (db.direct ? 4u * (((ac >> 4) + 2 + 3) & ~3u) : 0u) + 16u);
    auto inst = [&](auto... v) { return KeyKernel{order_key_kernel<decltype(v)::value...>, nullptr, smem, instance_name("order_key_kernel", v...)}; };
    auto of = [&](auto a32, auto hs) {
        if (fwd && tn.order_windows <= 64) return inst(Int<2>{}, a32, std::true_type{}, hs);
        if (fwd || sizing) return inst(Int<CLS_SLOTS[0]>{}, a32, std::true_type{}, hs);
        return inst(Int<CLS_SLOTS[0]>{}, a32, std::false_type{}, hs);
    };
    if (hashed) return of(std::true_type{}, std::true_type{});
    return db.addr32 ? of(std::true_type{}, std::false_type{}) : of(std::false_type{}, std::false_type{});
}
}

void PlacePlan::class_caps(uint32_t (&cap)[N_LISTS]) const {
    for (uint32_t& c : cap) c = 0;
    cap[0] = (uint32_t)(64 * CLS_SLOTS[0]);
    if (max_kmers > cap[0]) cap[1] = (uint32_t)(64 * CLS_SLOTS[1]);
    if (max_kmers > (uint32_t)(64 * CLS_SLOTS[1])) cap[2] = tiled ? tile_from : (uint32_t)(64 * BLK_WAVES * BLK_SLOTS);
    if (tiled) {
        for (uint32_t i = 0; i < tile.n_sub; ++i) cap[3 + i] = tile.sub[i].cap_kmers;
        cap[6] = tile.whole.cap_kmers;
    }
    cap[7] = long_cap;
}

std::string PlacePlan::class_kernel_name(const DbDev& db, int c, bool stats) const {
    if (c < 2) return class_kernel(db, c, stats).name;
    if (c == 2) return block_kernel(db, stats).name;
    if (c < 6) return tile_kernel_name(db, stats, tile.sub[c - 3]);
    if (c == 6) return tile_kernel_name(db, stats, tile.whole);
    return long_kernel(db, stats).name;
}

PlacePlan plan_place(const DbDev& db, uint32_t n_reads, uint32_t n_cu, bool stats, uint32_t long_cap, uint32_t n_long) {
    PlacePlan p{};
    const int forced = tuning().blocks_per_cu;
    const uint32_t want = (n_reads + WAVES_PER_BLOCK - 1) / WAVES_PER_BLOCK;
    uint64_t child_words = 0;
    for (int c = 0; c < N_CLASSES; ++c) {
        int per_cu = forced;
        const ClassKernel k = class_kernel(db, c, stats);
        if (per_cu <= 0 && (hipOccupancyMaxActiveBlocksPerMultiprocessor(&per_cu, k.fn(), 64 * WAVES_PER_BLOCK, k.smem) != hipSuccess || per_cu <= 0))
            per_cu = 1;
        uint32_t cap = n_cu * (uint32_t)per_cu;
        if (child_ws_stride(db) && !child_in_lds(db)) {
            const uint64_t per_block = (uint64_t)WAVES_PER_BLOCK * 2 * child_ws_stride(db) * 4;
            const uint64_t fit = std::max<uint64_t>(1, (128ull << 20) / per_block);
            if (cap > fit) cap = (uint32_t)fit;
        }
        p.grid[c] = want < cap ? (want ? want : 1) : cap;
        if (!child_in_lds(db)) child_words = std::max<uint64_t>(child_words, (uint64_t)p.grid[c] * WAVES_PER_BLOCK * 2 * child_ws_stride(db));
    }
    p.grid_blk = std::max<uint32_t>(1, std::min<uint32_t>(n_reads, n_cu));
    if (!child_in_lds(db)) child_words = std::max<uint64_t>(child_words, (uint64_t)p.grid_blk * 2 * child_ws_stride(db));
    p.ordered = use_order(db, n_reads);
    uint64_t w = 16 + (uint64_t)N_LISTS * n_reads;
    w += w & 1;
    if (p.ordered) {
        p.grid[0] = std::max<uint32_t>(8, p.grid[0] & ~7u);
        p.grid[1] = std::max<uint32_t>(8, p.grid[1] & ~7u);
        {
            int per_cu = tuning().key_blocks_per_cu;
            const KeyKernel k = key_kernel(db, true);
            if (per_cu <= 0 && (hipOccupancyMaxActiveBlocksPerMultiprocessor(&per_cu, k.fn(), 64 * WAVES_PER_BLOCK, k.smem) != hipSuccess || per_cu <= 0)) per_cu = 4;
            if (tuning().key_blocks_per_cu <= 0 && fast_mode(db) == 2) per_cu *= 2;
            p.grid_key = std::max<uint32_t>(1, std::min<uint32_t>(want, n_cu * (uint32_t)per_cu));
        }
        p.keys_off_words = w;
        w += 6 * (uint64_t)n_reads;
        p.sort_off_words = w;
        p.sort_bytes = order_temp_bytes(n_reads);
        w += (p.sort_bytes + 3) / 4 + 2;
        w += w & 1;
    }
    p.child_off_words = w;
    w += child_words;
    w += w & 1;
    p.max_kmers = n_long ? std::max<uint32_t>(long_cap, 2u) : MAX_READ_KMERS;
    const uint32_t blk_cap = (uint32_t)(64 * BLK_WAVES * BLK_SLOTS);
    p.tile_from = blk_cap;
    if (tile_usable(db)) {
        p.tile_from = tuning().tile_min_kmers > 0 ? std::min<uint32_t>(blk_cap, (uint32_t)tuning().tile_min_kmers) : (uint32_t)(64 * CLS_SLOTS[1]);
        if (p.max_kmers > p.tile_from) {
            p.tile = tile_plan(db, stats, p.tile_from, p.max_kmers, n_reads, n_cu);
            p.tiled = p.tile.whole.cap_kmers > p.tile_from;
        }
    }
    if (p.tiled) {
        p.tile_off_words = w;
        w += p.tile.scratch_words;
        w += w & 1;
    } else p.tile_from = blk_cap;
    if (p.max_kmers > MAX_READ_KMERS || p.tiled) {
        long_cap = p.max_kmers;
        p.long_cap = long_cap;
        p.long_set = 1;
        while (p.long_set < 2 * (uint64_t)long_cap) p.long_set <<= 1;
        p.long_arity = (std::max(db.max_nonleaf_arity, 1u) + 63) & ~63u;
        p.long_stride_words = 2 * (uint64_t)LONG_STATE_WORDS * long_cap + 2 * (uint64_t)p.long_arity;
        const uint64_t fit = std::max<uint64_t>(1, (2ull << 30) / (p.long_stride_words * 4));
        const uint64_t per_cu_long = (uint64_t)std::max(1, tuning().long_blocks_per_cu);
        p.grid_long = (uint32_t)std::min<uint64_t>({(uint64_t)std::max<uint32_t>(1u, n_long ? n_long : n_reads), (uint64_t)n_cu * per_cu_long, fit});
        if (p.tiled && p.tile.whole.cap_kmers >= long_cap) p.grid_long = std::min<uint32_t>(p.grid_long, 8u);
        p.long_off_words = w;
        w += p.long_stride_words * p.grid_long;
    }
    p.ws_bytes = w * 4;
    p.blk = p.max_kmers > (uint32_t)(64 * CLS_SLOTS[1]) && (!p.tiled || p.tile_from > (uint32_t)(64 * CLS_SLOTS[1]));
    const bool gene = tuning().time_class == 2;
    p.timed = p.tiled && (p.max_kmers > MAX_READ_KMERS || gene) ? PlacePlan::TIME_TILE : p.blk && gene ? PlacePlan::TIME_BLOCK : PlacePlan::TIME_CLASS0;
    p.timed_name = p.timed == PlacePlan::TIME_TILE ? p.tile.name : p.timed == PlacePlan::TIME_BLOCK ? block_kernel(db, stats).name : class_kernel(db, 0, stats).name;
    return p;
}

hipError_t launch_place(const DbDev& db, const PlaceParams& prm, const PlacePlan& plan, const uint8_t* d_bases,
                        const uint64_t* d_offsets, uint32_t n_reads, cls_placement* d_out, cls_query_stats* d_stats,
                        uint32_t* d_ws, hipStream_t stream, hipEvent_t ev_start, hipEvent_t ev_stop) {
    if (n_reads == 0) return hipSuccess;
    uint32_t* counts = d_ws;
    uint32_t* lists[N_LISTS];
    for (int c = 0; c < N_LISTS; ++c) lists[c] = d_ws + 16 + (size_t)c * n_reads;
    uint32_t* child_ws = (child_ws_stride(db) && !child_in_lds(db)) ? d_ws + plan.child_off_words : nullptr;
    hipError_t e = hipMemsetAsync(counts, 0, 64, stream);
    if (e != hipSuccess) return e;
    const uint32_t profile_stop = (uint32_t)tuning().profile_stop;
    const uint32_t ws_stride = child_ws_stride(db);
    const bool st = d_stats != nullptr;
    auto classify = [&](const uint32_t* order) {
        ClassCaps caps{};
        plan.class_caps(caps.cap);
        return launch_kernel(classify_kernel, dim3((n_reads + CLASSIFY_THREADS * CLASSIFY_PER_THREAD - 1) / (CLASSIFY_THREADS * CLASSIFY_PER_THREAD)), dim3(CLASSIFY_THREADS), 0,
                             stream, d_offsets, order, n_reads, db.k, caps, lists[0], counts, d_out, d_stats);
    };
    const uint32_t* list0 = lists[0];
    uint32_t list0_n = 0, xcd_chunks = 0;
    if (!plan.ordered) e = classify(nullptr);
    else {
        uint64_t* keys_in = reinterpret_cast<uint64_t*>(d_ws + plan.keys_off_words);
        uint64_t* keys_out = keys_in + n_reads;
        uint32_t* idx_in = reinterpret_cast<uint32_t*>(keys_out + n_reads);
        uint32_t* idx_out = idx_in + n_reads;
        const Tuning& tn = tuning();
        const uint32_t key_mode = (uint32_t)tn.order_mode;
        const uint32_t block_shift = (uint32_t)tn.order_block_shift;
        const uint32_t key_cap = (plan.tiled && !tn.no_tile_order) ? 0xFFFFFFFFu : (uint32_t)(64 * CLS_SLOTS[1]);
        const KeyKernel k = key_kernel(db, false);
        const dim3 block(64 * WAVES_PER_BLOCK);
        if (k.half) {
            const uint32_t grid_half = std::max<uint32_t>(1, std::min<uint32_t>((n_reads + 2 * WAVES_PER_BLOCK - 1) / (2 * WAVES_PER_BLOCK), plan.grid_key));
            e = launch_kernel(k.half, dim3(grid_half), block, k.smem, stream, db, d_bases, d_offsets, n_reads, keys_in, idx_in, key_mode, block_shift, key_cap);
        } else {
            e = launch_kernel(k.full, dim3(plan.grid_key), block, k.smem, stream, db, d_bases, d_offsets, n_reads, keys_in, idx_in, ascii_cap_of(db, 0), key_mode,
                              block_shift, (uint32_t)tn.order_sample_shift, tn.order_both_strands ? 0u : 1u, key_cap);
        }
        if (e != hipSuccess) return e;
        e = order_reads(d_ws + plan.sort_off_words, keys_in, idx_out, n_reads, order_key_bits(db) - 1, stream);
        if (e != hipSuccess) return e;
        list0 = idx_out;
        list0_n = n_reads;
        xcd_chunks = 1;
        e = classify(idx_out);
    }
    if (e != hipSuccess) return e;
    auto launch_class = [&](int c) {
        const ClassKernel k = class_kernel(db, c, st);
        const dim3 grid(plan.grid[c]), block(64 * WAVES_PER_BLOCK);
        if (k.fast) {
            return launch_kernel(k.fast, grid, block, k.smem, stream, db, prm, d_bases, d_offsets, xcd_chunks ? list0 : lists[c], counts + c, list0_n, xcd_chunks,
                                 d_out, d_stats, ascii_cap_of(db, c), profile_stop);
        }
        if (k.split)
            return launch_kernel(k.split, grid, block, k.smem, stream, db, prm, d_bases, d_offsets, lists[c], counts + c, d_out, d_stats, seq_cap_of(db, c),
                                 profile_stop, child_ws, ws_stride);
        return launch_kernel(k.wave, grid, block, k.smem, stream, db, prm, d_bases, d_offsets, lists[c], counts + c, d_out, d_stats, seq_cap_of(db, c), child_ws,
                             ws_stride);
    };
    auto timed = [&](PlacePlan::Timed t, auto&& launch) {
        if (ev_start && plan.timed == t) (void)hipEventRecord(ev_start, stream);
        const hipError_t r = launch();
        if (ev_stop && plan.timed == t) (void)hipEventRecord(ev_stop, stream);
        return r;
    };
    e = timed(PlacePlan::TIME_CLASS0, [&] { return launch_class(0); });
    if (e != hipSuccess) return e;
    if (plan.max_kmers > (uint32_t)(64 * CLS_SLOTS[0])) {
        e = launch_class(1);
        if (e != hipSuccess) return e;
    }
    if (plan.blk) {
        const auto k = block_kernel(db, st);
        e = timed(PlacePlan::TIME_BLOCK, [&] {
            return launch_kernel(k.fn, dim3(plan.grid_blk), dim3(64 * BLK_WAVES), k.smem, stream, db, prm, d_bases, d_offsets, lists[2], counts + 2, d_out, d_stats,
                                 blk_seq_cap(db), child_ws, ws_stride);
        });
        if (e != hipSuccess) return e;
    }
    if (plan.tiled) {
        const uint32_t* sub_lists[TILE_MAX_SUB] = {lists[3], lists[4], lists[5]};
        const uint32_t* sub_lens[TILE_MAX_SUB] = {counts + 3, counts + 4, counts + 5};
        e = timed(PlacePlan::TIME_TILE, [&] {
            return tile_launch(db, prm, plan.tile, st, d_bases, d_offsets, sub_lists, sub_lens, lists[6], counts + 6, d_out, d_stats, lists[7], counts + 7,
                               d_ws + plan.tile_off_words, plan.ordered && !tuning().no_tile_order, stream);
        });
        if (e != hipSuccess) return e;
    }
    if (plan.grid_long) {
        const auto k = long_kernel(db, st);
        e = launch_kernel(k.fn, dim3(plan.grid_long), dim3(LONG_THREADS), k.smem, stream, db, prm, d_bases, d_offsets, lists[7], counts + 7, d_out, d_stats,
                          d_ws + plan.long_off_words, plan.long_stride_words, plan.long_cap, (uint32_t)plan.long_set, plan.long_arity);
    }
    return e;
}

}
```

classeq2_amd/csrc/cls_sort.h:

```cpp
#pragma once
#include <hip/hip_runtime.h>
#include <stddef.h>
#include <stdint.h>

namespace cls {
constexpr int ORDER_BIN_BITS = 12;
constexpr uint32_t ORDER_BINS = 1u << ORDER_BIN_BITS;
size_t order_temp_bytes(uint32_t n);
hipError_t order_reads(void* tmp, const uint64_t* keys, uint32_t* idx_out, uint32_t n, int key_bits, hipStream_t stream);
}
```

classeq2_amd/csrc/cls_sort.hip:

```cpp
#include "cls_sort.h"

namespace cls {

namespace {

constexpr int SORT_THREADS = 1024, SORT_PER_THREAD = 16;

__device__ __forceinline__ uint32_t bin_of(uint64_t key, int shift) {
    return key == ~0ull ? ORDER_BINS - 1 : (uint32_t)(key >> shift) & (ORDER_BINS - 1);
}

__global__ __launch_bounds__(SORT_THREADS) void order_hist_kernel(const uint64_t* __restrict__ keys, uint32_t n, int shift, uint32_t* __restrict__ hist,
                                                                 uint32_t* __restrict__ block_base) {
    __shared__ uint32_t h[ORDER_BINS];
    for (uint32_t i = threadIdx.x; i < ORDER_BINS; i += SORT_THREADS) h[i] = 0;
    __syncthreads();
    const uint32_t base = blockIdx.x * (SORT_THREADS * SORT_PER_THREAD);
#pragma unroll
    for (int q = 0; q < SORT_PER_THREAD; ++q) {
        const uint32_t r = base + q * SORT_THREADS + threadIdx.x;
        if (r < n) atomicAdd(&h[bin_of(keys[r], shift)], 1u);
    }
    __syncthreads();
    for (uint32_t i = threadIdx.x; i < ORDER_BINS; i += SORT_THREADS)
        block_base[(size_t)blockIdx.x * ORDER_BINS + i] = h[i] ? atomicAdd(&hist[i], h[i]) : 0u;
}

__global__ __launch_bounds__(1024) void order_scan_kernel(uint32_t* __restrict__ hist) {
    constexpr uint32_t PER = ORDER_BINS / 1024;
    __shared__ uint32_t wave_tot[16];
    uint32_t v[PER], sum = 0;
#pragma unroll
    for (uint32_t q = 0; q < PER; ++q) { v[q] = hist[threadIdx.x * PER + q]; sum += v[q]; }
    const uint32_t lane = threadIdx.x & 63, wave = threadIdx.x >> 6;
    uint32_t inc = sum;
#pragma unroll
    for (int o = 1; o < 64; o <<= 1) { const uint32_t t = __shfl_up(inc, o); if ((int)lane >= o) inc += t; }
    if (lane == 63) wave_tot[wave] = inc;
    __syncthreads();
    uint32_t before = 0;
    for (uint32_t w = 0; w < wave; ++w) before += wave_tot[w];
    uint32_t at = before + inc - sum;
#pragma unroll
    for (uint32_t q = 0; q < PER; ++q) { hist[threadIdx.x * PER + q] = at; at += v[q]; }
}

__global__ __launch_bounds__(SORT_THREADS) void order_scatter_kernel(const uint64_t* __restrict__ keys, uint32_t n, int shift, const uint32_t* __restrict__ start,
                                                                    const uint32_t* __restrict__ block_base, uint32_t* __restrict__ idx_out) {
    __shared__ uint32_t at[ORDER_BINS];
    for (uint32_t i = threadIdx.x; i < ORDER_BINS; i += SORT_THREADS) at[i] = start[i] + block_base[(size_t)blockIdx.x * ORDER_BINS + i];
    __syncthreads();
    const uint32_t base = blockIdx.x * (SORT_THREADS * SORT_PER_THREAD);
#pragma unroll
    for (int q = 0; q < SORT_PER_THREAD; ++q) {
        const uint32_t r = base + q * SORT_THREADS + threadIdx.x;
        if (r < n) idx_out[atomicAdd(&at[bin_of(keys[r], shift)], 1u)] = r;
    }
}

}

static uint32_t order_blocks(uint32_t n) { return (n + SORT_THREADS * SORT_PER_THREAD - 1) / (SORT_THREADS * SORT_PER_THREAD); }

size_t order_temp_bytes(uint32_t n) { return (1 + (size_t)order_blocks(n)) * ORDER_BINS * sizeof(uint32_t); }

hipError_t order_reads(void* tmp, const uint64_t* keys, uint32_t* idx_out, uint32_t n, int key_bits, hipStream_t stream) {
    uint32_t* hist = static_cast<uint32_t*>(tmp);
    uint32_t* block_base = hist + ORDER_BINS;
    const int shift = key_bits > ORDER_BIN_BITS ? key_bits - ORDER_BIN_BITS : 0;
    hipError_t e = hipMemsetAsync(hist, 0, ORDER_BINS * sizeof(uint32_t), stream);
    if (e != hipSuccess) return e;
    const uint32_t blocks = order_blocks(n);
    hipLaunchKernelGGL(order_hist_kernel, dim3(blocks), dim3(SORT_THREADS), 0, stream, keys, n, shift, hist, block_base);
    hipLaunchKernelGGL(order_scan_kernel, dim3(1), dim3(1024), 0, stream, hist);
    hipLaunchKernelGGL(order_scatter_kernel, dim3(blocks), dim3(SORT_THREADS), 0, stream, keys, n, shift, (const uint32_t*)hist, (const uint32_t*)block_base, idx_out);
    return hipGetLastError();
}

}
```

classeq2_amd/csrc/cls_tuning.h:

```cpp
#pragma once

namespace cls {

struct Tuning {
    int no_fast = 0;
    int no_order = 0;
    int force_list = 0;
    int no_mask_halves = 0;
    int no_fat_direct = 0;
    int no_tile = 0;
    int tile_pass_codes = 0;
    int tile_set_words = 0;
    int tile_min_kmers = 0;
    int tile_deal = 64;
    int no_tile_order = 0;
    int tile_one_per_cu = 0;
    int time_class = 0;
    int blocks_per_cu = 0;
    int key_blocks_per_cu = 0;
    int long_blocks_per_cu = 2;
    int order_mode = 0;
    int order_windows = 64;
    int order_both_strands = 0;
    int order_block_shift = 2;
    int order_sample_shift = 32;
    int profile_stop = 0;
    int timing = 0;
    int build_full_key = 0;
    int tally_no_wave_combine = 0;
};

Tuning& tuning();

}
```

classeq2_amd/engine.py:

```python

from __future__ import annotations

import ctypes as C
import os
from typing import Optional

import numpy as np

from . import _abi
from .flatdb import FlatDb

_HERE = os.path.dirname(os.path.abspath(__file__))
LIB_PATH = os.environ.get("CLS_PLACE_LIB") or os.path.join(_HERE, "csrc", "libclsplace.so")
_LIB = None

EXPORTS = [
    "cls_device_count", "cls_db_create", "cls_db_validate", "cls_db_destroy", "cls_db_info_get", "cls_db_info_get2", "cls_db_kernel_time", "cls_db_kernel_name",
    "cls_db_read_classes", "cls_db_set_max_read_len", "cls_place_batch",
    "cls_db_group_create", "cls_db_group_destroy", "cls_db_group_size", "cls_db_group_replica", "cls_place_batch_group", "cls_fasta_split",
    "cls_place_batch_device", "cls_place_batch_stats", "cls_fasta_parse", "cls_fasta_free", "cls_fasta_scan_device", "cls_fasta_dev_free",
    "cls_fasta_parse_gpu", "cls_place_fasta_text", "cls_fastq_parse", "cls_fastq_split", "cls_fastq_scan_device", "cls_fastq_parse_gpu",
    "cls_place_fastq_text", "cls_last_error",
    "cls_tally_create", "cls_tally_destroy", "cls_tally_reset", "cls_tally_add_device", "cls_tally_add", "cls_tally_read", "cls_tally_host",
    "cls_tally_merge", "cls_tally_fasta_text", "cls_tally_fastq_text",
    "cls_pairer_create", "cls_pairer_destroy", "cls_pairer_totals", "cls_pair_records_device", "cls_pair_records", "cls_pair_host",
    "cls_pair_names_host", "cls_pair_names_device", "cls_place_fastq_pairs_text", "cls_tally_fastq_pairs_text",
    "cls_version", "cls_set_tuning", "cls_tuning_from_env", "cls_kmers_build", "cls_kmers_desc", "cls_kmers_info_get", "cls_kmers_free",
]
HOST_EXPORTS = [
    "cls_tree_load_json", "cls_tree_load", "cls_tree_init_from_file", "cls_tree_from_newick", "cls_tree_serialize", "cls_tree_save", "cls_tree_free", "cls_tree_set_annotations_yaml", "cls_tree_build_kmers_map", "cls_tree_build_kmers_map_device", "cls_tree_desc", "cls_serialize_results",
    "cls_host_free", "cls_place_sequences", "cls_place_sequences_group", "cls_place_sequences_ex", "cls_place_sequences_group_ex",
    "cls_host_last_error", "cls_tally_report", "cls_profile_sequences", "cls_profile_sequences_group", "cls_place_sequences_report", "cls_tree_nodes",
    "cls_place_pairs",
]
SERVICE_EXPORTS = [
    "cls_service_create", "cls_service_destroy", "cls_service_add_model", "cls_service_submit", "cls_service_wait", "cls_service_pause",
    "cls_service_stats_get",
]
FORMAT_YAML, FORMAT_JSONL = 0, 1
DB_FORMAT_ZSTD, DB_FORMAT_YAML, DB_FORMAT_JSON = 0, 1, 2


class ClsError(RuntimeError):
    def __init__(self, code: int, msg: str):
        super().__init__(f"[{code}] {msg}")
        self.code = code
        self.msg = msg


def lib():
    global _LIB
    if _LIB is None:
        if not os.path.exists(LIB_PATH):
            raise RuntimeError(
                f"{LIB_PATH} is missing: build it with `python -c 'import __graft_entry__ as g; g.build()'` "
                "(the placement path has no CPU fallback)"
            )
        L = C.CDLL(LIB_PATH)
        vp, u32, i32 = C.c_void_p, C.c_uint32, C.c_int
        L.cls_device_count.restype = i32
        L.cls_db_create.argtypes = [C.POINTER(_abi.DbDesc), i32, C.POINTER(vp)]
        L.cls_db_create.restype = i32
        L.cls_db_validate.argtypes = [C.POINTER(_abi.DbDesc)]
        L.cls_db_validate.restype = i32
        L.cls_db_destroy.argtypes = [vp]
        L.cls_db_destroy.restype = None
        L.cls_db_info_get.argtypes = [vp, C.POINTER(_abi.DbInfo)]
        L.cls_db_info_get.restype = i32
        L.cls_db_kernel_time.argtypes = [vp, C.POINTER(C.c_double), C.POINTER(C.c_uint64), i32]
        L.cls_db_kernel_time.restype = i32
        L.cls_db_kernel_name.argtypes = [vp, C.c_char_p, C.c_size_t]
        L.cls_db_kernel_name.restype = i32
        L.cls_db_read_classes.argtypes = [vp, C.c_uint64, i32, C.POINTER(_abi.ReadClass), i32, C.POINTER(i32)]
        L.cls_db_read_classes.restype = i32
        L.cls_db_set_max_read_len.argtypes = [vp, C.c_uint64]
        L.cls_db_set_max_read_len.restype = i32
        L.cls_place_batch.argtypes = [vp, vp, vp, u32, C.POINTER(_abi.Params), vp]
        L.cls_place_batch.restype = i32
        L.cls_place_batch_stats.argtypes = [vp, vp, vp, u32, C.POINTER(_abi.Params), vp, vp]
        L.cls_place_batch_stats.restype = i32
        L.cls_place_batch_device.argtypes = [vp, vp, vp, u32, C.POINTER(_abi.Params), vp, vp, vp]
        L.cls_place_batch_device.restype = i32
        L.cls_db_group_create.argtypes = [C.POINTER(_abi.DbDesc), C.POINTER(i32), u32, C.POINTER(vp)]
        L.cls_db_group_create.restype = i32
        L.cls_db_group_destroy.argtypes = [vp]
        L.cls_db_group_destroy.restype = None
        L.cls_db_group_size.argtypes = [vp, C.POINTER(u32)]
        L.cls_db_group_size.restype = i32
        L.cls_db_group_replica.argtypes = [vp, u32, C.POINTER(vp)]
        L.cls_db_group_replica.restype = i32
        L.cls_place_batch_group.argtypes = [vp, vp, vp, u32, C.POINTER(_abi.Params), vp, vp]
        L.cls_place_batch_group.restype = i32
        L.cls_fasta_split.argtypes = [C.c_char_p, C.c_size_t, u32, C.POINTER(C.c_uint64), C.POINTER(u32)]
        L.cls_fasta_split.restype = i32
        L.cls_fasta_parse.argtypes = [C.c_char_p, C.c_size_t, C.POINTER(_abi.Fasta)]
        L.cls_fasta_parse.restype = i32
        L.cls_fasta_parse_gpu.argtypes = [C.c_char_p, C.c_size_t, i32, C.POINTER(_abi.Fasta)]
        L.cls_fasta_parse_gpu.restype = i32
        L.cls_place_fasta_text.argtypes = [vp, C.c_char_p, C.c_size_t, C.POINTER(_abi.Params), C.POINTER(_abi.Fasta), C.POINTER(vp)]
        L.cls_place_fasta_text.restype = i32
        L.cls_fastq_parse.argtypes = [C.c_char_p, C.c_size_t, C.POINTER(_abi.FastqOpts), C.POINTER(_abi.Fasta)]
        L.cls_fastq_parse.restype = i32
        L.cls_fastq_parse_gpu.argtypes = [C.c_char_p, C.c_size_t, C.POINTER(_abi.FastqOpts), i32, C.POINTER(_abi.Fasta)]
        L.cls_fastq_parse_gpu.restype = i32
        L.cls_fastq_split.argtypes = [C.c_char_p, C.c_size_t, u32, C.POINTER(C.c_uint64), C.POINTER(u32)]
        L.cls_fastq_split.restype = i32
        L.cls_place_fastq_text.argtypes = [vp, C.c_char_p, C.c_size_t, C.POINTER(_abi.Params), C.POINTER(_abi.FastqOpts), C.POINTER(_abi.Fasta),
                                           C.POINTER(vp)]
        L.cls_place_fastq_text.restype = i32
        L.cls_tally_create.argtypes = [vp, C.POINTER(vp)]
        L.cls_tally_create.restype = i32
        L.cls_tally_destroy.argtypes = [vp]
        L.cls_tally_destroy.restype = None
        L.cls_tally_reset.argtypes = [vp]
        L.cls_tally_reset.restype = i32
        L.cls_tally_add_device.argtypes = [vp, vp, u32, vp]
        L.cls_tally_add_device.restype = i32
        L.cls_tally_add.argtypes = [vp, vp, u32]
        L.cls_tally_add.restype = i32
        L.cls_tally_read.argtypes = [vp, vp, u32, vp]
        L.cls_tally_read.restype = i32
        L.cls_tally_host.argtypes = [vp, u32, vp, C.c_uint64, vp, vp]
        L.cls_tally_host.restype = i32
        L.cls_tally_merge.argtypes = [vp, vp, vp, vp, u32]
        L.cls_tally_merge.restype = i32
        L.cls_tally_fasta_text.argtypes = [vp, vp, C.c_char_p, C.c_size_t, C.POINTER(_abi.Params), C.POINTER(u32), C.POINTER(u32)]
        L.cls_tally_fasta_text.restype = i32
        L.cls_tally_fastq_text.argtypes = [vp, vp, C.c_char_p, C.c_size_t, C.POINTER(_abi.Params), C.POINTER(_abi.FastqOpts), C.POINTER(u32),
                                           C.POINTER(u32)]
        L.cls_tally_fastq_text.restype = i32
        u64 = C.c_uint64
        L.cls_pairer_create.argtypes = [vp, C.POINTER(vp)]
        L.cls_pairer_create.restype = i32
        L.cls_pairer_destroy.argtypes = [vp]
        L.cls_pairer_destroy.restype = None
        L.cls_pairer_totals.argtypes = [vp, vp, i32]
        L.cls_pairer_totals.restype = i32
        L.cls_pair_records_device.argtypes = [vp, vp, vp, u32, u32, u32, vp, vp, vp]
        L.cls_pair_records_device.restype = i32
        L.cls_pair_records.argtypes = [vp, vp, vp, u32, u32, u32, vp, vp]
        L.cls_pair_records.restype = i32
        L.cls_pair_host.argtypes = [vp, u32, vp, vp, u32, u64, u32, vp, vp, vp]
        L.cls_pair_host.restype = i32
        L.cls_pair_names_host.argtypes = [vp, vp, vp, vp, u32, u64, C.POINTER(u64), C.POINTER(u64)]
        L.cls_pair_names_host.restype = i32
        L.cls_pair_names_device.argtypes = [vp, vp, vp, vp, u32, u32, C.POINTER(u64), C.POINTER(u64), vp]
        L.cls_pair_names_device.restype = i32
        L.cls_place_fastq_pairs_text.argtypes = [vp, vp, C.c_char_p, C.c_size_t, C.c_char_p, C.c_size_t, C.POINTER(_abi.Params),
                                                 C.POINTER(_abi.FastqOpts), u32, C.POINTER(_abi.Fasta), C.POINTER(vp), C.POINTER(vp)]
        L.cls_place_fastq_pairs_text.restype = i32
        L.cls_tally_fastq_pairs_text.argtypes = [vp, vp, vp, C.c_char_p, C.c_size_t, C.c_char_p, C.c_size_t, C.POINTER(_abi.Params),
                                                 C.POINTER(_abi.FastqOpts), u32, C.POINTER(u32), C.POINTER(u32)]
        L.cls_tally_fastq_pairs_text.restype = i32
        L.cls_fasta_free.argtypes = [C.POINTER(_abi.Fasta)]
        L.cls_fasta_free.restype = None
        L.cls_last_error.restype = C.c_char_p
        L.cls_version.restype = C.c_char_p
        L.cls_set_tuning.argtypes = [C.c_char_p, i32]
        L.cls_set_tuning.restype = i32
        L.cls_tuning_from_env.argtypes = []
        L.cls_tuning_from_env.restype = None
        L.cls_kmers_build.argtypes = [C.POINTER(_abi.BuildDesc), i32, C.POINTER(vp)]
        L.cls_kmers_build.restype = i32
        L.cls_kmers_desc.argtypes = [vp, C.POINTER(_abi.BuildDesc), C.POINTER(_abi.DbDesc)]
        L.cls_kmers_desc.restype = i32
        L.cls_kmers_info_get.argtypes = [vp, C.POINTER(_abi.KmersInfo)]
        L.cls_kmers_info_get.restype = i32
        L.cls_kmers_free.argtypes = [vp]
        L.cls_kmers_free.restype = None
        L.cls_tree_load_json.argtypes = [C.c_char_p, C.POINTER(vp)]
        L.cls_tree_load_json.restype = i32
        L.cls_tree_load.argtypes = [C.c_char_p, C.POINTER(vp)]
        L.cls_tree_load.restype = i32
        L.cls_tree_init_from_file.argtypes = [C.c_char_p, C.c_double, C.POINTER(vp)]
        L.cls_tree_init_from_file.restype = i32
        L.cls_tree_from_newick.argtypes = [C.c_char_p, C.c_char_p, C.c_double, C.POINTER(vp)]
        L.cls_tree_from_newick.restype = i32
        L.cls_tree_serialize.argtypes = [vp, i32, i32, C.POINTER(vp), C.POINTER(C.c_size_t)]
        L.cls_tree_serialize.restype = i32
        L.cls_tree_save.argtypes = [vp, C.c_char_p, i32, i32]
        L.cls_tree_save.restype = i32
        L.cls_tree_free.argtypes = [vp]
        L.cls_tree_free.restype = None
        L.cls_tree_set_annotations_yaml.argtypes = [vp, C.c_char_p]
        L.cls_tree_set_annotations_yaml.restype = i32
        L.cls_tree_build_kmers_map.argtypes = [vp, C.c_char_p, C.c_size_t, C.c_uint64, C.c_uint64, u32]
        L.cls_tree_build_kmers_map.restype = i32
        L.cls_tree_build_kmers_map_device.argtypes = [vp, C.c_char_p, C.c_size_t, C.c_uint64, C.c_uint64, u32, i32]
        L.cls_tree_build_kmers_map_device.restype = i32
        L.cls_tree_desc.argtypes = [vp, C.POINTER(_abi.DbDesc)]
        L.cls_tree_desc.restype = i32
        L.cls_serialize_results.argtypes = [vp, C.c_char_p, vp, u32, vp, i32, C.POINTER(vp), C.POINTER(C.c_size_t),
                                            C.POINTER(vp), C.POINTER(C.c_size_t)]
        L.cls_serialize_results.restype = i32
        L.cls_host_free.argtypes = [vp]
        L.cls_host_free.restype = None
        L.cls_place_sequences.argtypes = [vp, vp, C.c_char_p, C.c_char_p, C.POINTER(_abi.Params), i32, i32,
                                          C.POINTER(u32), C.POINTER(C.c_double)]
        L.cls_place_sequences.restype = i32
        L.cls_place_sequences_group.argtypes = [vp, vp, C.c_char_p, C.c_char_p, C.POINTER(_abi.Params), i32, i32,
                                                C.POINTER(u32), C.POINTER(C.c_double)]
        L.cls_place_sequences_group.restype = i32
        for name in ("cls_place_sequences_ex", "cls_place_sequences_group_ex"):
            getattr(L, name).argtypes = [vp, vp, C.c_char_p, C.c_char_p, C.POINTER(_abi.Params), i32, i32, i32, C.POINTER(_abi.FastqOpts),
                                         C.POINTER(u32), C.POINTER(C.c_double)]
            getattr(L, name).restype = i32
        L.cls_host_last_error.restype = C.c_char_p
        L.cls_tree_nodes.argtypes = [vp, C.POINTER(C.POINTER(_abi.Node)), C.POINTER(u32)]
        L.cls_tree_nodes.restype = i32
        L.cls_tally_report.argtypes = [vp, vp, vp, i32, C.POINTER(vp), C.POINTER(C.c_size_t)]
        L.cls_tally_report.restype = i32
        for name in ("cls_profile_sequences", "cls_profile_sequences_group"):
            getattr(L, name).argtypes = [vp, vp, C.c_char_p, C.c_char_p, C.POINTER(_abi.Params), i32, i32, C.POINTER(_abi.FastqOpts), C.c_uint64, i32,
                                         C.POINTER(u32), C.POINTER(C.c_double)]
            getattr(L, name).restype = i32
        L.cls_place_sequences_report.argtypes = [vp, vp, vp, C.c_char_p, C.c_char_p, C.POINTER(_abi.Params), i32, i32, i32, C.POINTER(_abi.FastqOpts),
                                                 C.c_char_p, i32, C.POINTER(u32), C.POINTER(C.c_double)]
        L.cls_place_sequences_report.restype = i32
        L.cls_place_pairs.argtypes = [vp, vp, C.c_char_p, C.c_char_p, C.c_char_p, C.c_char_p, C.c_char_p, C.POINTER(_abi.Params),
                                      C.POINTER(_abi.FastqOpts), u32, i32, i32, i32, C.POINTER(u32), C.POINTER(C.c_double)]
        L.cls_place_pairs.restype = i32
        L.cls_service_create.argtypes = [C.POINTER(vp)]
        L.cls_service_create.restype = i32
        L.cls_service_destroy.argtypes = [vp]
        L.cls_service_destroy.restype = None
        L.cls_service_add_model.argtypes = [vp, C.c_char_p, vp]
        L.cls_service_add_model.restype = i32
        L.cls_service_submit.argtypes = [vp, C.c_char_p, C.c_char_p, C.c_size_t, C.POINTER(_abi.Params), C.POINTER(C.c_uint64)]
        L.cls_service_submit.restype = i32
        L.cls_service_wait.argtypes = [vp, C.c_uint64, C.POINTER(_abi.Fasta), C.POINTER(vp)]
        L.cls_service_wait.restype = i32
        L.cls_service_pause.argtypes = [vp, i32]
        L.cls_service_pause.restype = i32
        L.cls_service_stats_get.argtypes = [vp, C.POINTER(_abi.ServiceStats)]
        L.cls_service_stats_get.restype = i32
        _LIB = L
    return _LIB


def _check(rc: int):
    if rc != 0:
        raise ClsError(rc, lib().cls_last_error().decode(errors="replace"))


def make_params(max_iterations: Optional[int] = None, min_match_coverage: Optional[float] = None,
                remove_intersection: Optional[bool] = None) -> _abi.Params:
    p = _abi.Params()
    if max_iterations is not None:
        p.flags |= _abi.HAS_MAX_ITERATIONS
        p.max_iterations = max_iterations
    if min_match_coverage is not None:
        p.flags |= _abi.HAS_MIN_MATCH_COVERAGE
        p.min_match_coverage = min_match_coverage
    if remove_intersection is not None:
        p.flags |= _abi.HAS_REMOVE_INTERSECTION
        p.remove_intersection = 1 if remove_intersection else 0
    return p


def set_tuning(name: str, value: int) -> None:
    _check(lib().cls_set_tuning(name.encode(), int(value)))


def tuning_from_env() -> None:
    lib().cls_tuning_from_env()


def device_count() -> int:
    return lib().cls_device_count()


def validate(flat: FlatDb) -> None:
    d = flat.desc()
    _check(lib().cls_db_validate(C.byref(d)))


def fasta_parse(text: bytes, device: Optional[int] = None):
    f = _abi.Fasta()
    if device is None:
        _check(lib().cls_fasta_parse(text, len(text), C.byref(f)))
    else:
        _check(lib().cls_fasta_parse_gpu(text, len(text), device, C.byref(f)))
    try:
        n = f.n
        hoff = np.ctypeslib.as_array(f.header_off, shape=(n + 1,)).copy()
        boff = np.ctypeslib.as_array(f.base_off, shape=(n + 1,)).copy()
        hraw = C.string_at(f.headers, int(hoff[-1]))
        bases = np.frombuffer(C.string_at(f.bases, int(boff[-1])), dtype=np.uint8).copy()
        headers = [hraw[int(hoff[i]) : int(hoff[i + 1])] for i in range(n)]
        return headers, bases, boff, bool(f.truncated)
    finally:
        lib().cls_fasta_free(C.byref(f))


def _fastq_opts(trim_5p: int = 0, trim_3p: int = 0) -> _abi.FastqOpts:
    o = _abi.FastqOpts()
    o.trim_5p, o.trim_3p = int(trim_5p), int(trim_3p)
    return o


def fastq_parse(text: bytes, device: Optional[int] = None, trim_5p: int = 0, trim_3p: int = 0):
    f = _abi.Fasta()
    o = _fastq_opts(trim_5p, trim_3p)
    if device is None:
        _check(lib().cls_fastq_parse(text, len(text), C.byref(o), C.byref(f)))
    else:
        _check(lib().cls_fastq_parse_gpu(text, len(text), C.byref(o), device, C.byref(f)))
    try:
        n = f.n
        hoff = np.ctypeslib.as_array(f.header_off, shape=(n + 1,)).copy()
        boff = np.ctypeslib.as_array(f.base_off, shape=(n + 1,)).copy()
        hraw = C.string_at(f.headers, int(hoff[-1]))
        bases = np.frombuffer(C.string_at(f.bases, int(boff[-1])), dtype=np.uint8).copy()
        headers = [hraw[int(hoff[i]) : int(hoff[i + 1])] for i in range(n)]
        return headers, bases, boff, bool(f.truncated)
    finally:
        lib().cls_fasta_free(C.byref(f))


def fastq_split(text: bytes, max_pieces: int) -> list:
    cuts = (C.c_uint64 * (max_pieces + 1))()
    n = C.c_uint32(0)
    _check(lib().cls_fastq_split(text, len(text), max_pieces, cuts, C.byref(n)))
    return [int(c) for c in cuts[: n.value + 1]]


def build_kmers(nodes: np.ndarray, bases: np.ndarray, offsets: np.ndarray, leaf_ids: np.ndarray, k: int, m: int, *,
                leaves_only: bool = False, forward_only: bool = False, device: int = 0, return_info: bool = False):
    nodes = np.ascontiguousarray(nodes, dtype=_abi.NODE_DTYPE)
    bases = np.ascontiguousarray(np.frombuffer(bases, dtype=np.uint8) if isinstance(bases, (bytes, bytearray)) else bases, dtype=np.uint8)
    offsets = np.ascontiguousarray(offsets, dtype=np.uint64)
    leaf_ids = np.ascontiguousarray(leaf_ids, dtype=np.uint64)
    if len(offsets) != len(leaf_ids) + 1:
        raise ValueError("offsets must hold one entry more than leaf_ids")
    b = _abi.BuildDesc()
    b.abi_version = _abi.ABI_VERSION
    b.n_nodes = len(nodes)
    b.nodes = nodes.ctypes.data_as(C.POINTER(_abi.Node))
    b.k_size, b.m_size = k, m
    b.n_records = len(leaf_ids)
    b.flags = (_abi.BUILD_LEAVES_ONLY if leaves_only else 0) | (_abi.BUILD_FORWARD_ONLY if forward_only else 0)
    b.bases = bases.ctypes.data
    b.offsets = offsets.ctypes.data_as(C.POINTER(C.c_uint64))
    b.leaf_id = leaf_ids.ctypes.data_as(C.POINTER(C.c_uint64))
    km = C.c_void_p()
    _check(lib().cls_kmers_build(C.byref(b), device, C.byref(km)))
    try:
        d = _abi.DbDesc()
        _check(lib().cls_kmers_desc(km, C.byref(b), C.byref(d)))
        flat = FlatDb.from_desc(d, copy=True)
        inf = _abi.KmersInfo()
        _check(lib().cls_kmers_info_get(km, C.byref(inf)))
    finally:
        lib().cls_kmers_free(km)
    if return_info:
        return flat, {name: getattr(inf, name) for name, _ in _abi.KmersInfo._fields_}
    return flat


def fasta_split(text: bytes, max_pieces: int) -> list:
    cuts = (C.c_uint64 * (max_pieces + 1))()
    n = C.c_uint32(0)
    _check(lib().cls_fasta_split(text, len(text), max_pieces, cuts, C.byref(n)))
    return [int(c) for c in cuts[: n.value + 1]]


class PlacementDb:

    def __init__(self, flat: FlatDb, device: int = -1):
        self._h = C.c_void_p()
        d = flat.desc()
        _check(lib().cls_db_create(C.byref(d), device, C.byref(self._h)))
        info = _abi.DbInfo()
        _check(lib().cls_db_info_get(self._h, C.byref(info)))
        self.info = info

    def close(self):
        if getattr(self, "_h", None):
            lib().cls_db_destroy(self._h)
            self._h = C.c_void_p()

    def __del__(self):
        try:
            self.close()
        except Exception:
            pass

    def __enter__(self):
        return self

    def __exit__(self, *a):
        self.close()

    def refresh_info(self):
        _check(lib().cls_db_info_get(self._h, C.byref(self.info)))
        return self.info

    def kernel_name(self) -> str:
        buf = C.create_string_buffer(256)
        _check(lib().cls_db_kernel_name(self._h, buf, len(buf)))
        return buf.value.decode()

    def read_classes(self, n_bases: int = 0, stats: bool = False):
        buf = (_abi.ReadClass * 8)()
        n = C.c_int(0)
        _check(lib().cls_db_read_classes(self._h, n_bases, 1 if stats else 0, buf, len(buf), C.byref(n)))
        assert n.value <= len(buf)
        return [(int(c.list), int(c.max_kmers), c.kernel.decode()) for c in buf[:n.value]]

    def place_batch(self, bases: np.ndarray, offsets: np.ndarray, params: Optional[_abi.Params] = None,
                    want_stats: bool = False, out: Optional[np.ndarray] = None):
        bases = np.ascontiguousarray(bases, dtype=np.uint8)
        offsets = np.ascontiguousarray(offsets, dtype=np.uint64)
        n = len(offsets) - 1
        if out is None:
            out = np.zeros(n, dtype=_abi.PLACEMENT_DTYPE)
        assert out.dtype == _abi.PLACEMENT_DTYPE and len(out) >= n and out.flags.c_contiguous
        pp = C.byref(params) if params is not None else None
        if want_stats:
            stats = np.zeros(n, dtype=_abi.STATS_DTYPE)
            _check(lib().cls_place_batch_stats(self._h, bases.ctypes.data, offsets.ctypes.data, n, pp,
                                               out.ctypes.data, stats.ctypes.data))
            return out, stats
        _check(lib().cls_place_batch(self._h, bases.ctypes.data, offsets.ctypes.data, n, pp, out.ctypes.data))
        return out

    def kernel_time(self, reset: bool = False):
        ms, cnt = C.c_double(0), C.c_uint64(0)
        _check(lib().cls_db_kernel_time(self._h, C.byref(ms), C.byref(cnt), 1 if reset else 0))
        return ms.value, cnt.value

    def place_fasta_text(self, text: bytes, params: Optional[_abi.Params] = None):
        f = _abi.Fasta()
        recs = C.c_void_p()
        pp = C.byref(params) if params is not None else None
        _check(lib().cls_place_fasta_text(self._h, text, len(text), pp, C.byref(f), C.byref(recs)))
        try:
            n = f.n
            hoff = np.ctypeslib.as_array(f.header_off, shape=(n + 1,)).copy()
            hraw = C.string_at(f.headers, int(hoff[-1]))
            headers = [hraw[int(hoff[i]) : int(hoff[i + 1])] for i in range(n)]
            out = np.frombuffer(C.string_at(recs, n * 24), dtype=_abi.PLACEMENT_DTYPE).copy() if n else np.zeros(0, _abi.PLACEMENT_DTYPE)
            return headers, out, bool(f.truncated)
        finally:
            lib().cls_fasta_free(C.byref(f))
            lib().cls_host_free(recs)

    def place_fastq_text(self, text: bytes, params: Optional[_abi.Params] = None, trim_5p: int = 0, trim_3p: int = 0):
        f = _abi.Fasta()
        recs = C.c_void_p()
        pp = C.byref(params) if params is not None else None
        o = _fastq_opts(trim_5p, trim_3p)
        _check(lib().cls_place_fastq_text(self._h, text, len(text), pp, C.byref(o), C.byref(f), C.byref(recs)))
        try:
            n = f.n
            hoff = np.ctypeslib.as_array(f.header_off, shape=(n + 1,)).copy()
            hraw = C.string_at(f.headers, int(hoff[-1]))
            headers = [hraw[int(hoff[i]) : int(hoff[i + 1])] for i in range(n)]
            out = np.frombuffer(C.string_at(recs, n * 24), dtype=_abi.PLACEMENT_DTYPE).copy() if n else np.zeros(0, _abi.PLACEMENT_DTYPE)
            return headers, out, bool(f.truncated)
        finally:
            lib().cls_fasta_free(C.byref(f))
            lib().cls_host_free(recs)

    def tally_fasta_text(self, tally: "Tally", text: bytes, params: Optional[_abi.Params] = None):
        n, tr = C.c_uint32(0), C.c_uint32(0)
        pp = C.byref(params) if params is not None else None
        _check(lib().cls_tally_fasta_text(self._h, tally._h, text, len(text), pp, C.byref(n), C.byref(tr)))
        return n.value, bool(tr.value)

    def tally_fastq_text(self, tally: "Tally", text: bytes, params: Optional[_abi.Params] = None, trim_5p: int = 0, trim_3p: int = 0):
        n, tr = C.c_uint32(0), C.c_uint32(0)
        pp = C.byref(params) if params is not None else None
        o = _fastq_opts(trim_5p, trim_3p)
        _check(lib().cls_tally_fastq_text(self._h, tally._h, text, len(text), pp, C.byref(o), C.byref(n), C.byref(tr)))
        return n.value, bool(tr.value)

    def place_fastq_pairs_text(self, pairer: "Pairer", text1: bytes, text2: Optional[bytes] = None, params: Optional[_abi.Params] = None,
                               trim_5p: int = 0, trim_3p: int = 0, flags: int = 0):
        f = _abi.Fasta()
        recs, how = C.c_void_p(), C.c_void_p()
        pp = C.byref(params) if params is not None else None
        o = _fastq_opts(trim_5p, trim_3p)
        _check(lib().cls_place_fastq_pairs_text(self._h, pairer._h, text1, len(text1), text2, len(text2) if text2 is not None else 0, pp,
                                                C.byref(o), flags, C.byref(f), C.byref(recs), C.byref(how)))
        try:
            n = f.n
            hoff = np.ctypeslib.as_array(f.header_off, shape=(n + 1,)).copy()
            hraw = C.string_at(f.headers, int(hoff[-1]))
            headers = [hraw[int(hoff[i]) : int(hoff[i + 1])] for i in range(n)]
            out = np.frombuffer(C.string_at(recs, n * 24), dtype=_abi.PLACEMENT_DTYPE).copy() if n else np.zeros(0, _abi.PLACEMENT_DTYPE)
            hw = np.frombuffer(C.string_at(how, n), dtype=np.uint8).copy() if n else np.zeros(0, np.uint8)
            return headers, out, hw, bool(f.truncated)
        finally:
            lib().cls_fasta_free(C.byref(f))
            lib().cls_host_free(recs)
            lib().cls_host_free(how)

    def tally_fastq_pairs_text(self, pairer: "Pairer", tally: "Tally", text1: bytes, text2: Optional[bytes] = None,
                               params: Optional[_abi.Params] = None, trim_5p: int = 0, trim_3p: int = 0, flags: int = 0):
        n, tr = C.c_uint32(0), C.c_uint32(0)
        pp = C.byref(params) if params is not None else None
        o = _fastq_opts(trim_5p, trim_3p)
        _check(lib().cls_tally_fastq_pairs_text(self._h, pairer._h, tally._h, text1, len(text1), text2, len(text2) if text2 is not None else 0,
                                                pp, C.byref(o), flags, C.byref(n), C.byref(tr)))
        return n.value, bool(tr.value)

    def set_max_read_len(self, n_bases: int) -> None:
        _check(lib().cls_db_set_max_read_len(self._h, n_bases))
        _check(lib().cls_db_info_get(self._h, C.byref(self.info)))

    def place_batch_device(self, d_bases: int, d_offsets: int, n: int, d_out: int, params: Optional[_abi.Params] = None,
                           d_stats: int = 0, stream: int = 0) -> None:
        pp = C.byref(params) if params is not None else None
        _check(lib().cls_place_batch_device(self._h, d_bases, d_offsets, n, pp, d_out, d_stats or None, stream or None))


class Tally:

    def __init__(self, db: PlacementDb):
        self._db = db
        self._h = C.c_void_p()
        _check(lib().cls_tally_create(db._h, C.byref(self._h)))
        self.n_nodes = int(db.info.n_nodes)

    def add(self, records: np.ndarray) -> None:
        recs = np.ascontiguousarray(records, dtype=_abi.PLACEMENT_DTYPE)
        _check(lib().cls_tally_add(self._h, recs.ctypes.data, len(recs)))

    def add_device(self, d_records: int, n: int, stream: int = 0) -> None:
        _check(lib().cls_tally_add_device(self._h, d_records or None, n, stream or None))

    def read(self):
        rows = np.zeros(self.n_nodes, dtype=_abi.TALLY_ROW_DTYPE)
        totals = np.zeros(1, dtype=_abi.TALLY_TOTALS_DTYPE)
        _check(lib().cls_tally_read(self._h, rows.ctypes.data, len(rows), totals.ctypes.data))
        return rows, totals[0]

    def reset(self) -> None:
        _check(lib().cls_tally_reset(self._h))

    def close(self):
        if getattr(self, "_h", None):
            lib().cls_tally_destroy(self._h)
            self._h = C.c_void_p()

    def __del__(self):
        try:
            self.close()
        except Exception:
            pass

    def __enter__(self):
        return self

    def __exit__(self, *a):
        self.close()


def tally_host(flat: FlatDb, records: np.ndarray, rows: Optional[np.ndarray] = None, totals: Optional[np.ndarray] = None):
    nodes = np.ascontiguousarray(flat.nodes, dtype=_abi.NODE_DTYPE)
    recs = np.ascontiguousarray(records, dtype=_abi.PLACEMENT_DTYPE)
    if rows is None:
        rows = np.zeros(len(nodes), dtype=_abi.TALLY_ROW_DTYPE)
    if totals is None:
        totals = np.zeros(1, dtype=_abi.TALLY_TOTALS_DTYPE)
    assert rows.dtype == _abi.TALLY_ROW_DTYPE and len(rows) == len(nodes) and rows.flags.c_contiguous
    assert totals.dtype == _abi.TALLY_TOTALS_DTYPE and totals.shape == (1,)
    _check(lib().cls_tally_host(nodes.ctypes.data, len(nodes), recs.ctypes.data, len(recs), rows.ctypes.data, totals.ctypes.data))
    return rows, totals


def tally_merge(rows: np.ndarray, totals: np.ndarray, add_rows: np.ndarray, add_totals) -> None:
    add_rows = np.ascontiguousarray(add_rows, dtype=_abi.TALLY_ROW_DTYPE)
    add_totals = np.ascontiguousarray(np.atleast_1d(add_totals), dtype=_abi.TALLY_TOTALS_DTYPE)
    assert rows.dtype == _abi.TALLY_ROW_DTYPE and len(rows) == len(add_rows) and rows.flags.c_contiguous
    assert totals.dtype == _abi.TALLY_TOTALS_DTYPE and totals.shape == (1,)
    _check(lib().cls_tally_merge(rows.ctypes.data, totals.ctypes.data, add_rows.ctypes.data, add_totals.ctypes.data, len(rows)))


class Pairer:

    def __init__(self, db: PlacementDb):
        self._db = db
        self._h = C.c_void_p()
        _check(lib().cls_pairer_create(db._h, C.byref(self._h)))

    def pair_device(self, d_a: int, d_b: int, stride: int, n: int, d_out: int, d_how: int = 0, flags: int = 0, stream: int = 0) -> None:
        _check(lib().cls_pair_records_device(self._h, d_a or None, d_b or None, stride, n, flags, d_out or None, d_how or None, stream or None))

    def pair(self, a: np.ndarray, b: Optional[np.ndarray] = None, flags: int = 0):
        return _pair_call(lambda *args: lib().cls_pair_records(self._h, *args), a, b, flags, totals=False)

    def totals(self, reset: bool = False):
        t = np.zeros(1, dtype=_abi.PAIR_TOTALS_DTYPE)
        _check(lib().cls_pairer_totals(self._h, t.ctypes.data, 1 if reset else 0))
        return t[0]

    def close(self):
        if getattr(self, "_h", None):
            lib().cls_pairer_destroy(self._h)
            self._h = C.c_void_p()

    def __del__(self):
        try:
            self.close()
        except Exception:
            pass

    def __enter__(self):
        return self

    def __exit__(self, *a):
        self.close()


def _pair_call(fn, a, b, flags, totals):
    a = np.ascontiguousarray(a, dtype=_abi.PLACEMENT_DTYPE)
    if b is None:
        if len(a) % 2:
            raise ValueError("an interleaved batch holds an even number of records")
        stride, n, pb = 2, len(a) // 2, a.ctypes.data + 24
    else:
        b = np.ascontiguousarray(b, dtype=_abi.PLACEMENT_DTYPE)
        if len(a) != len(b):
            raise ValueError("the two mates' record arrays differ in length")
        stride, n, pb = 1, len(a), b.ctypes.data
    out = np.full(n, 0xFF, dtype=np.uint8).repeat(24).view(_abi.PLACEMENT_DTYPE)
    how = np.full(n, 0xFF, dtype=np.uint8)
    if totals:
        tot = np.zeros(1, dtype=_abi.PAIR_TOTALS_DTYPE)
        _check(fn(a.ctypes.data, pb, stride, n, flags, out.ctypes.data, how.ctypes.data, tot.ctypes.data))
        return out, how, tot[0]
    _check(fn(a.ctypes.data, pb, stride, n, flags, out.ctypes.data, how.ctypes.data))
    return out, how


def pair_host(flat, a: np.ndarray, b: Optional[np.ndarray] = None, flags: int = 0):
    nodes = np.ascontiguousarray(flat.nodes, dtype=_abi.NODE_DTYPE)
    return _pair_call(lambda *args: lib().cls_pair_host(nodes.ctypes.data, len(nodes), *args), a, b, flags, totals=True)


def pair_names_host(headers1, headers2=None):
    def pack(hs):
        hb = [h if isinstance(h, bytes) else h.encode() for h in hs]
        return b"".join(hb), np.concatenate([[0], np.cumsum([len(h) for h in hb])]).astype(np.uint64)

    t1, o1 = pack(headers1)
    if headers2 is None:
        if len(headers1) % 2:
            raise ValueError("an interleaved list holds an even number of headers")
        t2, p2, stride, n = t1, o1.ctypes.data + 8, 2, len(headers1) // 2
    else:
        if len(headers1) != len(headers2):
            raise ValueError("the two header lists differ in length")
        t2, o2 = pack(headers2)
        p2, stride, n = o2.ctypes.data, 1, len(headers1)
    n_bad, first = C.c_uint64(0), C.c_uint64(0)
    _check(lib().cls_pair_names_host(t1, o1.ctypes.data, t2, p2, stride, n, C.byref(n_bad), C.byref(first)))
    return n_bad.value, (first.value if n_bad.value else None)


class _ReplicaView(PlacementDb):

# ... 276 lines not shown
```

Measured before the change: 157.9 million.

## Precompute 16-bit order bins per k-mer code and sort reads on 32-bit bins

Adds a host-built bins16 table mapping each direct-table k-mer code to a tier-tagged 12-bit sort bin, uploaded to the device. A new order_bin_kernel packs two reads per wave and looks up bins from this compact table instead of computing 64-bit order keys, and the radix ordering then runs on 32-bit bins rather than 64-bit keys. The aim is to cut memory traffic in key generation and in the sort's histogram and scatter passes. It adds table memory and build time, falls back when sets are few or the tree is non-canonical, and adds debug entry points.

```diff
diff --git a/classeq2_amd/_abi.py b/classeq2_amd/_abi.py
--- a/classeq2_amd/_abi.py
+++ b/classeq2_amd/_abi.py
@@ -7,6 +7,7 @@
 KIND_ROOT, KIND_NODE, KIND_LEAF = 0, 1, 2
 NO_PARENT = (1 << 64) - 1
 
+BIN_TABLE_META_WORDS = 4
 HAS_MAX_ITERATIONS = 1
 HAS_MIN_MATCH_COVERAGE = 2
 HAS_REMOVE_INTERSECTION = 4
diff --git a/classeq2_amd/csrc/cls_api.cpp b/classeq2_amd/csrc/cls_api.cpp
--- a/classeq2_amd/csrc/cls_api.cpp
+++ b/classeq2_amd/csrc/cls_api.cpp
@@ -89,6 +89,7 @@
     void* d_mz_bucket = nullptr;
     void* d_direct = nullptr;
     void* d_direct16 = nullptr;
+    void* d_bins16 = nullptr;
     void* d_sets = nullptr;
     void* d_sets2 = nullptr;
     std::mutex ws_mu;
@@ -113,7 +114,7 @@
 struct Knob { const char* name; int cls::Tuning::*field; };
 const Knob KNOBS[] = {
     {"no_fast", &cls::Tuning::no_fast}, {"no_order", &cls::Tuning::no_order}, {"force_list", &cls::Tuning::force_list},
-    {"no_mask_halves", &cls::Tuning::no_mask_halves}, {"no_fat_direct", &cls::Tuning::no_fat_direct}, {"no_tile", &cls::Tuning::no_tile}, {"tile_pass_codes", &cls::Tuning::tile_pass_codes}, {"tile_set_words", &cls::Tuning::tile_set_words}, {"time_class", &cls::Tuning::time_class}, {"tile_one_per_cu", &cls::Tuning::tile_one_per_cu}, {"tile_min_kmers", &cls::Tuning::tile_min_kmers}, {"no_tile_order", &cls::Tuning::no_tile_order}, {"tile_deal", &cls::Tuning::tile_deal}, {"blocks_per_cu", &cls::Tuning::blocks_per_cu}, {"key_blocks_per_cu", &cls::Tuning::key_blocks_per_cu},
+    {"no_mask_halves", &cls::Tuning::no_mask_halves}, {"no_fat_direct", &cls::Tuning::no_fat_direct}, {"no_bin_table", &cls::Tuning::no_bin_table}, {"no_tile", &cls::Tuning::no_tile}, {"tile_pass_codes", &cls::Tuning::tile_pass_codes}, {"tile_set_words", &cls::Tuning::tile_set_words}, {"time_class", &cls::Tuning::time_class}, {"tile_one_per_cu", &cls::Tuning::tile_one_per_cu}, {"tile_min_kmers", &cls::Tuning::tile_min_kmers}, {"no_tile_order", &cls::Tuning::no_tile_order}, {"tile_deal", &cls::Tuning::tile_deal}, {"blocks_per_cu", &cls::Tuning::blocks_per_cu}, {"key_blocks_per_cu", &cls::Tuning::key_blocks_per_cu},
     {"long_blocks_per_cu", &cls::Tuning::long_blocks_per_cu}, {"order_mode", &cls::Tuning::order_mode},
     {"order_windows", &cls::Tuning::order_windows}, {"order_both_strands", &cls::Tuning::order_both_strands},
     {"order_block_shift", &cls::Tuning::order_block_shift}, {"order_sample_shift", &cls::Tuning::order_sample_shift},
@@ -174,6 +175,7 @@
     if (db->d_mz_bucket) (void)hipFree(db->d_mz_bucket);
     if (db->d_direct) (void)hipFree(db->d_direct);
     if (db->d_direct16) (void)hipFree(db->d_direct16);
+    if (db->d_bins16) (void)hipFree(db->d_bins16);
     if (db->d_sets) (void)hipFree(db->d_sets);
     if (db->d_sets2) (void)hipFree(db->d_sets2);
     if (have_prev) (void)hipSetDevice(prev);
@@ -219,6 +221,7 @@
         (!E.mz_bucket.empty() && (e = up(&db->d_mz_bucket, E.mz_bucket.data(), E.mz_bucket.size() * 4)) != hipSuccess) ||
         (!E.direct.empty() && (e = up(&db->d_direct, E.direct.data(), E.direct.size() * 4)) != hipSuccess) ||
         (!E.direct16.empty() && (e = up(&db->d_direct16, E.direct16.data(), E.direct16.size() * 4)) != hipSuccess) ||
+        (!E.bins16.empty() && (e = up(&db->d_bins16, E.bins16.data(), E.bins16.size() * 2)) != hipSuccess) ||
         (!E.sets.empty() && (e = up(&db->d_sets, E.sets.data(), E.sets.size() * sizeof(cls::SetRec))) != hipSuccess) ||
         (!E.sets2.empty() && (e = up(&db->d_sets2, E.sets2.data(), E.sets2.size() * sizeof(cls::SetRec))) != hipSuccess)) {
         cls_db_destroy(db);
@@ -234,6 +237,7 @@
     v.mz_bucket = (const uint32_t*)db->d_mz_bucket;
     v.direct = (const uint32_t*)db->d_direct;
     v.direct16 = (const uint32_t*)db->d_direct16;
+    v.bins16 = (const uint16_t*)db->d_bins16;
     v.sets = (const cls::SetRec*)db->d_sets;
     v.sets2 = (const cls::SetRec*)db->d_sets2;
     v.table_mask = E.table.size() - 1;
@@ -246,8 +250,7 @@
     v.binary_tree = E.strictly_binary ? 1u : 0u;
     v.canonical = E.canonical ? 1u : 0u;
     v.n_sets = (uint32_t)E.sets.size();
-    v.set_bits = 1;
-    while (v.set_bits < 32 && (1ull << v.set_bits) < (uint64_t)E.sets.size()) ++v.set_bits;
+    v.set_bits = cls::set_id_bits(E.sets.size());
     v.addr32 = (E.postings.size() * 4 < (1ull << 32) && E.direct.size() * 4 < (1ull << 32) && E.sets.size() * sizeof(cls::SetRec) < (1ull << 32)) ? 1u : 0u;
     cls_db_info& i = db->info;
     i.n_nodes = v.n_nodes;
@@ -260,7 +263,7 @@
     i.n_closed_kmers = E.n_closed;
     i.table_slots = E.table.size();
     i.postings_words = E.postings.size();
-    i.hbm_bytes = E.nodes.size() * sizeof(cls::DNode) + E.table.size() * sizeof(cls::Slot) + (E.postings.size() + E.postings2.size()) * 4 + E.bucket_key.size() * 8 + E.mz_bucket.size() * 4 + E.direct.size() * 4 + E.direct16.size() * 4 + (E.sets.size() + E.sets2.size()) * sizeof(cls::SetRec);
+    i.hbm_bytes = E.nodes.size() * sizeof(cls::DNode) + E.table.size() * sizeof(cls::Slot) + (E.postings.size() + E.postings2.size()) * 4 + E.bucket_key.size() * 8 + E.mz_bucket.size() * 4 + E.direct.size() * 4 + E.direct16.size() * 4 + E.bins16.size() * 2 + (E.sets.size() + E.sets2.size()) * sizeof(cls::SetRec);
     i.device = device;
     i.format = E.format;
     i.binary_tree = E.strictly_binary ? 1u : 0u;
@@ -481,6 +484,32 @@
     } catch (...) {
         rc = fail(CLS_E_INTERNAL, "cls_place_batch_device: unknown exception");
     }
+    if (prev != db->device) (void)hipSetDevice(prev);
+    return rc;
+}
+
+extern "C" int cls_db_debug_order_bins(cls_db* db, const void* d_bases, const void* d_offsets, uint32_t n, int from_table, void* d_bins) {
+    if (!db || !d_offsets || !d_bins) return fail(CLS_E_INVALID_ARG, "cls_db_debug_order_bins: null argument");
+    int prev = 0;
+    CLS_HIP(hipGetDevice(&prev));
+    if (prev != db->device) CLS_HIP(hipSetDevice(db->device));
+    int rc = CLS_OK;
+    void* d_keys = nullptr;
+    try {
+        const cls::PlacePlan plan = cls::plan_place(db->dev, n, (uint32_t)db->n_cu, false, 0, 0);
+        if (!plan.ordered) rc = fail(CLS_E_INVALID_ARG, "cls_db_debug_order_bins: a launch of this size is not ordered");
+        else if (from_table && !plan.bin_keys) rc = fail(CLS_E_INVALID_ARG, "cls_db_debug_order_bins: no bin table in use");
+        else if (hipMalloc(&d_keys, (size_t)n * 8) != hipSuccess) rc = fail(CLS_E_NOMEM, "cls_db_debug_order_bins: scratch allocation failed");
+        else {
+            hipError_t e = cls::debug_order_bins(db->dev, plan, (const uint8_t*)d_bases, (const uint64_t*)d_offsets, n, from_table != 0, (uint32_t*)d_keys,
+                                                 (uint32_t*)d_bins, nullptr);
+            if (e == hipSuccess) e = hipStreamSynchronize(nullptr);
+            if (e != hipSuccess) rc = fail(CLS_E_HIP, std::string("cls_db_debug_order_bins: ") + hipGetErrorString(e));
+        }
+    } catch (...) {
+        rc = fail(CLS_E_INTERNAL, "cls_db_debug_order_bins: unknown exception");
+    }
+    if (d_keys) (void)hipFree(d_keys);
     if (prev != db->device) (void)hipSetDevice(prev);
     return rc;
 }
diff --git a/classeq2_amd/csrc/cls_db.cpp b/classeq2_amd/csrc/cls_db.cpp
--- a/classeq2_amd/csrc/cls_db.cpp
+++ b/classeq2_amd/csrc/cls_db.cpp
@@ -558,6 +558,18 @@
                         o[0] = sr.x; o[1] = sr.vlo_lg; o[2] = sr.vhi_root; o[3] = e;
                         const uint32_t bits = set_mask.empty() ? 0u : set_mask[e & SET_ID_MASK];
                         if (bits) { o[0] = bits; o[2] |= FAT_X_IS_BITS; }
+                    }
+                });
+            }
+            const uint32_t set_bits = set_id_bits(E.sets.size());
+            if (E.canonical && !tuning().no_bin_table && tuning().order_block_shift >= 0 &&
+                (int)set_bits - tuning().order_block_shift >= BIN_TABLE_BITS) {
+                const uint32_t shift = set_bits - BIN_TABLE_BITS;
+                E.bins16.resize(n_codes);
+                parallel_chunks(n_codes, nt, [&](unsigned, uint64_t lo, uint64_t hi) {
+                    for (uint64_t code = lo; code < hi; ++code) {
+                        const uint32_t e = E.direct[code], id = e & SET_ID_MASK;
+                        E.bins16[code] = id ? (uint16_t)((e >> TIER_SHIFT) << BIN_TIER_SHIFT | (1u + (id >> shift))) : (uint16_t)0;
                     }
                 });
             }
@@ -637,6 +649,28 @@
                 }
             }
         }
+        return CLS_OK;
+    } catch (const std::bad_alloc&) {
+        return CLS_E_NOMEM;
+    } catch (...) {
+        return CLS_E_INTERNAL;
+    }
+}
+
+extern "C" int cls_db_debug_bin_table(const cls_db_desc* d, uint32_t* meta, uint32_t* direct_out, uint16_t* bins_out, uint64_t cap) {
+    try {
+        if (!meta) return CLS_E_INVALID_ARG;
+        cls::EncodedDb E;
+        std::string err;
+        const int rc = cls::encode_db(d, E, err);
+        if (rc != CLS_OK) return rc;
+        meta[0] = cls::set_id_bits(E.sets.size());
+        meta[1] = E.direct.empty() ? 0u : 1u;
+        meta[2] = E.canonical ? 1u : 0u;
+        meta[3] = E.bins16.empty() ? 0u : 1u;
+        if (!E.bins16.empty() && E.bins16.size() != E.direct.size()) return CLS_E_INTERNAL;
+        if (direct_out && cap >= E.direct.size()) std::copy(E.direct.begin(), E.direct.end(), direct_out);
+        if (bins_out && cap >= E.bins16.size()) std::copy(E.bins16.begin(), E.bins16.end(), bins_out);
         return CLS_OK;
     } catch (const std::bad_alloc&) {
         return CLS_E_NOMEM;
diff --git a/classeq2_amd/csrc/cls_db.h b/classeq2_amd/csrc/cls_db.h
--- a/classeq2_amd/csrc/cls_db.h
+++ b/classeq2_amd/csrc/cls_db.h
@@ -48,6 +48,7 @@
     HugeVec<SetRec> sets2;
     HugeVec<uint32_t> direct;
     HugeVec<uint32_t> direct16;
+    HugeVec<uint16_t> bins16;
     uint32_t k = 0, m = 0, m_eff = 0;
     uint32_t max_depth = 0, max_nonleaf_arity = 0;
     uint64_t n_kmers = 0, n_closed = 0;
diff --git a/classeq2_amd/csrc/cls_device.h b/classeq2_amd/csrc/cls_device.h
--- a/classeq2_amd/csrc/cls_device.h
+++ b/classeq2_amd/csrc/cls_device.h
@@ -49,6 +49,14 @@
 static_assert(sizeof(SetRec) == 16, "SetRec");
 constexpr uint32_t DIRECT_MAX_K = 15;
 constexpr uint32_t FAT_DIRECT_MAX_K = 12;
+constexpr int BIN_TABLE_BITS = 12;
+constexpr int BIN_TIER_SHIFT = BIN_TABLE_BITS + 1;
+constexpr uint32_t BIN_VALUE_MASK = (1u << BIN_TIER_SHIFT) - 1;
+inline uint32_t set_id_bits(uint64_t n_sets) {
+    uint32_t b = 1;
+    while (b < 32 && (1ull << b) < n_sets) ++b;
+    return b;
+}
 constexpr uint32_t DIRECT_TIP_BITS = 27;
 constexpr uint32_t DIRECT_TIP_MASK = (1u << DIRECT_TIP_BITS) - 1;
 struct TipRec {
@@ -74,6 +82,7 @@
     const uint32_t* mz_bucket;
     const uint32_t* direct;
     const uint32_t* direct16;
+    const uint16_t* bins16;
     const SetRec* sets;
     const SetRec* sets2;
     uint64_t table_mask;
diff --git a/classeq2_amd/csrc/cls_kernels.h b/classeq2_amd/csrc/cls_kernels.h
--- a/classeq2_amd/csrc/cls_kernels.h
+++ b/classeq2_amd/csrc/cls_kernels.h
@@ -59,7 +59,9 @@
     uint32_t grid_blk;
     uint32_t grid_key;
     bool ordered;
+    bool bin_keys;
     uint64_t keys_off_words;
+    uint64_t idx_off_words;
     uint64_t sort_off_words;
     size_t sort_bytes;
     uint64_t child_off_words;
@@ -92,4 +94,7 @@
                         const uint64_t* d_offsets, uint32_t n_reads, cls_placement* d_out, cls_query_stats* d_stats,
                         uint32_t* d_ws, hipStream_t stream, hipEvent_t ev_start, hipEvent_t ev_stop);
 
+hipError_t debug_order_bins(const DbDev& db, PlacePlan plan, const uint8_t* d_bases, const uint64_t* d_offsets, uint32_t n_reads, bool from_table,
+                            uint32_t* d_keys, uint32_t* d_bins, hipStream_t stream);
+
 }
diff --git a/classeq2_amd/csrc/cls_kernels.hip b/classeq2_amd/csrc/cls_kernels.hip
--- a/classeq2_amd/csrc/cls_kernels.hip
+++ b/classeq2_amd/csrc/cls_kernels.hip
@@ -1516,7 +1516,7 @@
 template <int SLOTS, bool ADDR32, bool FWD, bool HASHED>
 __global__ __launch_bounds__(64 * WAVES_PER_BLOCK) void order_key_kernel(DbDev db, const uint8_t* __restrict__ bases,
                                                                        const uint64_t* __restrict__ offsets, uint32_t n_reads,
-                                                                       uint64_t* __restrict__ keys, uint32_t* __restrict__ idx,
+                                                                       uint64_t* __restrict__ keys,
                                                                        uint32_t ascii_cap, uint32_t key_mode,
                                                                        uint32_t block_shift, uint32_t sample_shift, uint32_t fwd_only,
                                                                        uint32_t key_cap) {
@@ -1583,14 +1583,14 @@
             }
             wave_sync();
         }
-        if (lane == 0) { keys[r] = key; idx[r] = r; }
+        if (lane == 0) keys[r] = key;
     }
 }
 
 template <bool ADDR32>
 __global__ __launch_bounds__(64 * WAVES_PER_BLOCK) void order_key_half_kernel(DbDev db, const uint8_t* __restrict__ bases,
                                                                             const uint64_t* __restrict__ offsets, uint32_t n_reads,
-                                                                            uint64_t* __restrict__ keys, uint32_t* __restrict__ idx,
+                                                                            uint64_t* __restrict__ keys,
                                                                             uint32_t key_mode, uint32_t block_shift,
                                                                             uint32_t key_cap) {
     constexpr uint32_t MAXL = 64 + DIRECT_MAX_K - 1 + 1;
@@ -1683,10 +1683,98 @@
             mh = o1 < mh ? o1 : mh;
             mha = o2 < mha ? o2 : mha;
         }
-        if (have && hl == 0) {
-            keys[r] = (ok && n_cand) ? make_order_key(key_mode, prefix, mh, mha, block_shift, db.set_bits) : ~0ull;
-            idx[r] = r;
-        }
+        if (have && hl == 0) keys[r] = (ok && n_cand) ? make_order_key(key_mode, prefix, mh, mha, block_shift, db.set_bits) : ~0ull;
+        wave_sync();
+    }
+}
+
+template <bool ADDR32>
+__global__ __launch_bounds__(64 * WAVES_PER_BLOCK) void order_bin_kernel(DbDev db, const uint8_t* __restrict__ bases,
+                                                                       const uint64_t* __restrict__ offsets, uint32_t n_reads,
+                                                                       uint32_t* __restrict__ bins, uint32_t key_cap) {
+    constexpr uint32_t RPW = 2;
+    static_assert(BIN_TABLE_BITS == ORDER_BIN_BITS, "the table holds the sort's bins");
+    constexpr uint32_t LPR = 64 / RPW, WPL = 64 / LPR;
+    constexpr uint32_t MAXL = 64 + DIRECT_MAX_K - 1 + 1;
+    constexpr uint32_t WORDS = (MAXL + 15) / 16 + 2;
+    static_assert(WORDS <= LPR, "one packed word per lane");
+    __shared__ __align__(16) uint8_t s_ascii[WAVES_PER_BLOCK * RPW][(MAXL + 19) & ~3u];
+    __shared__ uint32_t s_packed[WAVES_PER_BLOCK * RPW][WORDS];
+    const uint32_t wave = threadIdx.x >> 6, lane = threadIdx.x & 63, part = lane / LPR, pl = lane % LPR;
+    uint8_t* ascii = s_ascii[wave * RPW + part];
+    uint32_t* packed = s_packed[wave * RPW + part];
+    const uint32_t k = db.k;
+    const uint32_t kmask = (1u << (2 * k)) - 1u;
+    const uint16_t* __restrict__ table = db.bins16;
+    const uint32_t group0 = (blockIdx.x * WAVES_PER_BLOCK + wave) * RPW, stride = gridDim.x * WAVES_PER_BLOCK * RPW;
+    auto part_of = [&](uint64_t m) { return (uint32_t)((m >> (LPR * part)) & ((1ull << LPR) - 1)); };
+    for (uint32_t r0 = group0; r0 < n_reads; r0 += stride) {
+        const uint32_t r = r0 + part;
+        const bool have = r < n_reads;
+        const uint64_t b0 = have ? offsets[r] : 0, L64 = have ? offsets[r + 1] - b0 : 0;
+        const bool keyed = have && L64 >= k && 2 * (L64 - k + 1) <= (uint64_t)key_cap;
+        const uint32_t L = keyed ? (uint32_t)std::min<uint64_t>(L64, 64 + k - 1) : 0, nf = keyed ? L - k + 1 : 0;
+        bool bad = false;
+        for (uint32_t i = pl; i < L; i += LPR) {
+            uint8_t c = bases[b0 + i];
+            if (c >= 'a' && c <= 'z') c -= 32;
+            bad |= !(c == 'A' || c == 'C' || c == 'G' || c == 'T');
+            ascii[i] = c;
+        }
+        const bool ok = keyed && part_of(__ballot(bad)) == 0;
+        wave_sync();
+        if (const uint32_t w = pl; w < (L + 15) / 16 + 1 && w < WORDS) {
+            uint32_t acc = 0;
+#pragma unroll
+            for (int q = 0; q < 4; ++q) {
+                uint32_t t = *reinterpret_cast<const uint32_t*>(ascii + 16 * w + 4 * q);
+                t = (t >> 1) & 0x03030303u;
+                t = (t | (t >> 6) | (t >> 12) | (t >> 18)) & 0xFFu;
+                acc |= t << (8 * q);
+            }
+            packed[w] = acc;
+        }
+        wave_sync();
+        uint32_t e[WPL];
+#pragma unroll
+        for (int s = 0; s < (int)WPL; ++s) {
+            const uint32_t p = pl + LPR * s;
+            const bool valid = ok && p < nf;
+            const uint32_t w = valid ? p >> 4 : 0, sh = valid ? (2 * p) & 31 : 0;
+            const uint32_t d0 = packed[w], d1 = packed[w + 1];
+            uint32_t code = (uint32_t)((((uint64_t)d1 << 32) | d0) >> sh) & kmask;
+            uint32_t rcc = __builtin_bitreverse32(code ^ (0xAAAAAAAAu & kmask));
+            rcc = ((rcc >> 1) & 0x55555555u) | ((rcc & 0x55555555u) << 1);
+            rcc >>= (32 - 2 * k);
+            code = rcc < code ? rcc : code;
+            const uint32_t v = ldx<uint16_t, ADDR32>(table, valid ? code : 0u);
+            e[s] = valid ? v : 0u;
+        }
+        uint32_t cand = 0, n_cand = 0;
+        for (uint32_t tier = 0; tier < 4; ++tier) {
+            const bool need = n_cand < 4;
+            uint32_t c_new = 0, n_new = 0;
+#pragma unroll
+            for (int s = 0; s < (int)WPL; ++s) {
+                const bool c = e[s] != 0 && (e[s] >> BIN_TIER_SHIFT) <= tier;
+                c_new |= (c ? 1u : 0u) << s;
+                n_new += (uint32_t)__popc(part_of(__ballot(c)));
+            }
+            if (need) { cand = c_new; n_cand = n_new; }
+            if (__ballot(n_cand < 4) == 0) break;
+        }
+        uint32_t rank = n_cand >> 1, prefix = 0;
+        for (int bit = BIN_TABLE_BITS - 1; bit >= 0; --bit) {
+            uint32_t c0 = 0;
+#pragma unroll
+            for (int s = 0; s < (int)WPL; ++s) {
+                const uint32_t t = (e[s] & BIN_VALUE_MASK) - 1u;
+                const bool z = ((cand >> s) & 1u) && ((t ^ prefix) >> (bit + 1)) == 0 && !((t >> bit) & 1u);
+                c0 += (uint32_t)__popc(part_of(__ballot(z)));
+            }
+            if (rank >= c0) { rank -= c0; prefix |= 1u << bit; }
+        }
+        if (have && pl == 0) bins[r] = (ok && n_cand) ? prefix : ORDER_BINS - 1;
         wave_sync();
     }
 }
@@ -2214,21 +2302,33 @@
 
 using KeyFn = decltype(order_key_kernel<2, true, true, false>);
 using KeyHalfFn = decltype(order_key_half_kernel<true>);
+using KeyBinFn = decltype(order_bin_kernel<true>);
 struct KeyKernel {
     KeyFn* full;
     KeyHalfFn* half;
+    KeyBinFn* bin;
+    uint32_t reads_per_wave;
     size_t smem;
     std::string name;
-    const void* fn() const { return full ? (const void*)full : (const void*)half; }
+    const void* fn() const { return full ? (const void*)full : half ? (const void*)half : (const void*)bin; }
 };
+bool bins_are_key_tops(const DbDev& db) {
+    const Tuning& tn = tuning();
+    return db.bins16 != nullptr && db.canonical && tn.order_mode == 0 && tn.order_block_shift >= 0 && (int)db.set_bits - tn.order_block_shift >= ORDER_BIN_BITS;
+}
 KeyKernel key_kernel(const DbDev& db, bool sizing) {
     const Tuning& tn = tuning();
     const bool fwd = !tn.order_both_strands, hashed = fast_mode(db) == 2;
-    if (!sizing && !hashed && fwd && tn.order_windows == 64 && (uint32_t)tn.order_sample_shift >= 32)
-        return with_bool(db.addr32, [&](auto a32) { return KeyKernel{nullptr, order_key_half_kernel<decltype(a32)::value>, 0, instance_name("order_key_half_kernel", a32)}; });
+    if (!sizing && !hashed && fwd && tn.order_windows == 64 && (uint32_t)tn.order_sample_shift >= 32) {
+        if (bins_are_key_tops(db))
+            return with_bool(db.addr32, [&](auto a32) {
+                return KeyKernel{nullptr, nullptr, order_bin_kernel<decltype(a32)::value>, 2, 0, instance_name("order_bin_kernel", a32)};
+            });
+        return with_bool(db.addr32, [&](auto a32) { return KeyKernel{nullptr, order_key_half_kernel<decltype(a32)::value>, nullptr, 2, 0, instance_name("order_key_half_kernel", a32)}; });
+    }
     const uint32_t ac = ascii_cap_of(db, 0);
     const size_t smem = (size_t)WAVES_PER_BLOCK * (ac + (db.direct ? 4u * (((ac >> 4) + 2 + 3) & ~3u) : 0u) + 16u);
-    auto inst = [&](auto... v) { return KeyKernel{order_key_kernel<decltype(v)::value...>, nullptr, smem, instance_name("order_key_kernel", v...)}; };
+    auto inst = [&](auto... v) { return KeyKernel{order_key_kernel<decltype(v)::value...>, nullptr, nullptr, 1, smem, instance_name("order_key_kernel", v...)}; };
     auto of = [&](auto a32, auto hs) {
         if (fwd && tn.order_windows <= 64) return inst(Int<2>{}, a32, std::true_type{}, hs);
         if (fwd || sizing) return inst(Int<CLS_SLOTS[0]>{}, a32, std::true_type{}, hs);
@@ -2293,8 +2393,11 @@
             if (tuning().key_blocks_per_cu <= 0 && fast_mode(db) == 2) per_cu *= 2;
             p.grid_key = std::max<uint32_t>(1, std::min<uint32_t>(want, n_cu * (uint32_t)per_cu));
         }
+        p.bin_keys = key_kernel(db, false).bin != nullptr;
         p.keys_off_words = w;
-        w += 6 * (uint64_t)n_reads;
+        w += (p.bin_keys ? 1 : 2) * (uint64_t)n_reads;
+        p.idx_off_words = w;
+        w += n_reads;
         p.sort_off_words = w;
         p.sort_bytes = order_temp_bytes(n_reads);
         w += (p.sort_bytes + 3) / 4 + 2;
@@ -2338,6 +2441,39 @@
     p.timed = p.tiled && (p.max_kmers > MAX_READ_KMERS || gene) ? PlacePlan::TIME_TILE : p.blk && gene ? PlacePlan::TIME_BLOCK : PlacePlan::TIME_CLASS0;
     p.timed_name = p.timed == PlacePlan::TIME_TILE ? p.tile.name : p.timed == PlacePlan::TIME_BLOCK ? block_kernel(db, stats).name : class_kernel(db, 0, stats).name;
     return p;
+}
+
+static hipError_t launch_order_keys(const DbDev& db, const PlacePlan& plan, const uint8_t* d_bases, const uint64_t* d_offsets, uint32_t n_reads,
+                                    uint32_t* keys, hipStream_t stream) {
+    const Tuning& tn = tuning();
+    const uint32_t key_mode = (uint32_t)tn.order_mode;
+    const uint32_t block_shift = (uint32_t)tn.order_block_shift;
+    const uint32_t key_cap = (plan.tiled && !tn.no_tile_order) ? 0xFFFFFFFFu : (uint32_t)(64 * CLS_SLOTS[1]);
+    const KeyKernel k = key_kernel(db, false);
+    if ((k.bin != nullptr) != plan.bin_keys) return hipErrorInvalidValue;
+    const dim3 block(64 * WAVES_PER_BLOCK);
+    const uint32_t per_block = k.reads_per_wave * WAVES_PER_BLOCK;
+    const uint32_t grid_part = std::max<uint32_t>(1, std::min<uint32_t>((n_reads + per_block - 1) / per_block, plan.grid_key));
+    if (k.bin) return launch_kernel(k.bin, dim3(grid_part), block, k.smem, stream, db, d_bases, d_offsets, n_reads, keys, key_cap);
+    uint64_t* keys64 = reinterpret_cast<uint64_t*>(keys);
+    if (k.half) return launch_kernel(k.half, dim3(grid_part), block, k.smem, stream, db, d_bases, d_offsets, n_reads, keys64, key_mode, block_shift, key_cap);
+    return launch_kernel(k.full, dim3(plan.grid_key), block, k.smem, stream, db, d_bases, d_offsets, n_reads, keys64, ascii_cap_of(db, 0), key_mode, block_shift,
+                         (uint32_t)tn.order_sample_shift, tn.order_both_strands ? 0u : 1u, key_cap);
+}
+
+hipError_t debug_order_bins(const DbDev& db, PlacePlan plan, const uint8_t* d_bases, const uint64_t* d_offsets, uint32_t n_reads, bool from_table,
+                            uint32_t* d_keys, uint32_t* d_bins, hipStream_t stream) {
+    if (!plan.ordered || (from_table && !plan.bin_keys)) return hipErrorInvalidValue;
+    hipError_t e;
+    if (from_table) e = launch_order_keys(db, plan, d_bases, d_offsets, n_reads, d_bins, stream);
+    else {
+        DbDev old = db;
+        old.bins16 = nullptr;
+        plan.bin_keys = false;
+        e = launch_order_keys(old, plan, d_bases, d_offsets, n_reads, d_keys, stream);
+        if (e == hipSuccess) e = order_bins_of_keys(reinterpret_cast<const uint64_t*>(d_keys), d_bins, n_reads, order_key_bits(old) - 1, stream);
+    }
+    return e;
 }
 
 hipError_t launch_place(const DbDev& db, const PlaceParams& prm, const PlacePlan& plan, const uint8_t* d_bases,
@@ -2363,25 +2499,12 @@
     uint32_t list0_n = 0, xcd_chunks = 0;
     if (!plan.ordered) e = classify(nullptr);
     else {
-        uint64_t* keys_in = reinterpret_cast<uint64_t*>(d_ws + plan.keys_off_words);
-        uint64_t* keys_out = keys_in + n_reads;
-        uint32_t* idx_in = reinterpret_cast<uint32_t*>(keys_out + n_reads);
-        uint32_t* idx_out = idx_in + n_reads;
-        const Tuning& tn = tuning();
-        const uint32_t key_mode = (uint32_t)tn.order_mode;
-        const uint32_t block_shift = (uint32_t)tn.order_block_shift;
-        const uint32_t key_cap = (plan.tiled && !tn.no_tile_order) ? 0xFFFFFFFFu : (uint32_t)(64 * CLS_SLOTS[1]);
-        const KeyKernel k = key_kernel(db, false);
-        const dim3 block(64 * WAVES_PER_BLOCK);
-        if (k.half) {
-            const uint32_t grid_half = std::max<uint32_t>(1, std::min<uint32_t>((n_reads + 2 * WAVES_PER_BLOCK - 1) / (2 * WAVES_PER_BLOCK), plan.grid_key));
-            e = launch_kernel(k.half, dim3(grid_half), block, k.smem, stream, db, d_bases, d_offsets, n_reads, keys_in, idx_in, key_mode, block_shift, key_cap);
-        } else {
-            e = launch_kernel(k.full, dim3(plan.grid_key), block, k.smem, stream, db, d_bases, d_offsets, n_reads, keys_in, idx_in, ascii_cap_of(db, 0), key_mode,
-                              block_shift, (uint32_t)tn.order_sample_shift, tn.order_both_strands ? 0u : 1u, key_cap);
-        }
+        uint32_t* keys = d_ws + plan.keys_off_words;
+        uint32_t* idx_out = d_ws + plan.idx_off_words;
+        e = launch_order_keys(db, plan, d_bases, d_offsets, n_reads, keys, stream);
         if (e != hipSuccess) return e;
-        e = order_reads(d_ws + plan.sort_off_words, keys_in, idx_out, n_reads, order_key_bits(db) - 1, stream);
+        if (plan.bin_keys) e = order_reads(d_ws + plan.sort_off_words, keys, idx_out, n_reads, stream);
+        else e = order_reads(d_ws + plan.sort_off_words, reinterpret_cast<const uint64_t*>(keys), idx_out, n_reads, order_key_bits(db) - 1, stream);
         if (e != hipSuccess) return e;
         list0 = idx_out;
         list0_n = n_reads;
diff --git a/classeq2_amd/csrc/cls_sort.h b/classeq2_amd/csrc/cls_sort.h
--- a/classeq2_amd/csrc/cls_sort.h
+++ b/classeq2_amd/csrc/cls_sort.h
@@ -8,4 +8,6 @@
 constexpr uint32_t ORDER_BINS = 1u << ORDER_BIN_BITS;
 size_t order_temp_bytes(uint32_t n);
 hipError_t order_reads(void* tmp, const uint64_t* keys, uint32_t* idx_out, uint32_t n, int key_bits, hipStream_t stream);
+hipError_t order_reads(void* tmp, const uint32_t* bins, uint32_t* idx_out, uint32_t n, hipStream_t stream);
+hipError_t order_bins_of_keys(const uint64_t* keys, uint32_t* bins, uint32_t n, int key_bits, hipStream_t stream);
 }
diff --git a/classeq2_amd/csrc/cls_sort.hip b/classeq2_amd/csrc/cls_sort.hip
--- a/classeq2_amd/csrc/cls_sort.hip
+++ b/classeq2_amd/csrc/cls_sort.hip
@@ -9,8 +9,10 @@
 __device__ __forceinline__ uint32_t bin_of(uint64_t key, int shift) {
     return key == ~0ull ? ORDER_BINS - 1 : (uint32_t)(key >> shift) & (ORDER_BINS - 1);
 }
+__device__ __forceinline__ uint32_t bin_of(uint32_t bin, int) { return bin & (ORDER_BINS - 1); }
 
-__global__ __launch_bounds__(SORT_THREADS) void order_hist_kernel(const uint64_t* __restrict__ keys, uint32_t n, int shift, uint32_t* __restrict__ hist,
+template <class T>
+__global__ __launch_bounds__(SORT_THREADS) void order_hist_kernel(const T* __restrict__ keys, uint32_t n, int shift, uint32_t* __restrict__ hist,
                                                                  uint32_t* __restrict__ block_base) {
     __shared__ uint32_t h[ORDER_BINS];
     for (uint32_t i = threadIdx.x; i < ORDER_BINS; i += SORT_THREADS) h[i] = 0;
@@ -45,7 +47,8 @@
     for (uint32_t q = 0; q < PER; ++q) { hist[threadIdx.x * PER + q] = at; at += v[q]; }
 }
 
-__global__ __launch_bounds__(SORT_THREADS) void order_scatter_kernel(const uint64_t* __restrict__ keys, uint32_t n, int shift, const uint32_t* __restrict__ start,
+template <class T>
+__global__ __launch_bounds__(SORT_THREADS) void order_scatter_kernel(const T* __restrict__ keys, uint32_t n, int shift, const uint32_t* __restrict__ start,
                                                                     const uint32_t* __restrict__ block_base, uint32_t* __restrict__ idx_out) {
     __shared__ uint32_t at[ORDER_BINS];
     for (uint32_t i = threadIdx.x; i < ORDER_BINS; i += SORT_THREADS) at[i] = start[i] + block_base[(size_t)blockIdx.x * ORDER_BINS + i];
@@ -58,22 +61,43 @@
     }
 }
 
+__global__ __launch_bounds__(256) void order_bin_of_kernel(const uint64_t* __restrict__ keys, uint32_t n, int shift, uint32_t* __restrict__ bins) {
+    const uint32_t r = blockIdx.x * 256 + threadIdx.x;
+    if (r < n) bins[r] = bin_of(keys[r], shift);
+}
+
 }
 
 static uint32_t order_blocks(uint32_t n) { return (n + SORT_THREADS * SORT_PER_THREAD - 1) / (SORT_THREADS * SORT_PER_THREAD); }
 
 size_t order_temp_bytes(uint32_t n) { return (1 + (size_t)order_blocks(n)) * ORDER_BINS * sizeof(uint32_t); }
 
-hipError_t order_reads(void* tmp, const uint64_t* keys, uint32_t* idx_out, uint32_t n, int key_bits, hipStream_t stream) {
+template <class T>
+static hipError_t order_reads_t(void* tmp, const T* keys, uint32_t* idx_out, uint32_t n, int shift, hipStream_t stream) {
     uint32_t* hist = static_cast<uint32_t*>(tmp);
     uint32_t* block_base = hist + ORDER_BINS;
-    const int shift = key_bits > ORDER_BIN_BITS ? key_bits - ORDER_BIN_BITS : 0;
     hipError_t e = hipMemsetAsync(hist, 0, ORDER_BINS * sizeof(uint32_t), stream);
     if (e != hipSuccess) return e;
     const uint32_t blocks = order_blocks(n);
-    hipLaunchKernelGGL(order_hist_kernel, dim3(blocks), dim3(SORT_THREADS), 0, stream, keys, n, shift, hist, block_base);
+    hipLaunchKernelGGL(order_hist_kernel<T>, dim3(blocks), dim3(SORT_THREADS), 0, stream, keys, n, shift, hist, block_base);
     hipLaunchKernelGGL(order_scan_kernel, dim3(1), dim3(1024), 0, stream, hist);
-    hipLaunchKernelGGL(order_scatter_kernel, dim3(blocks), dim3(SORT_THREADS), 0, stream, keys, n, shift, (const uint32_t*)hist, (const uint32_t*)block_base, idx_out);
+    hipLaunchKernelGGL(order_scatter_kernel<T>, dim3(blocks), dim3(SORT_THREADS), 0, stream, keys, n, shift, (const uint32_t*)hist, (const uint32_t*)block_base, idx_out);
+    return hipGetLastError();
+}
+
+static int key_shift(int key_bits) { return key_bits > ORDER_BIN_BITS ? key_bits - ORDER_BIN_BITS : 0; }
+
+hipError_t order_reads(void* tmp, const uint64_t* keys, uint32_t* idx_out, uint32_t n, int key_bits, hipStream_t stream) {
+    return order_reads_t(tmp, keys, idx_out, n, key_shift(key_bits), stream);
+}
+
+hipError_t order_reads(void* tmp, const uint32_t* bins, uint32_t* idx_out, uint32_t n, hipStream_t stream) {
+    return order_reads_t(tmp, bins, idx_out, n, 0, stream);
+}
+
+hipError_t order_bins_of_keys(const uint64_t* keys, uint32_t* bins, uint32_t n, int key_bits, hipStream_t stream) {
+    if (n == 0) return hipSuccess;
+    hipLaunchKernelGGL(order_bin_of_kernel, dim3((n + 255) / 256), dim3(256), 0, stream, keys, n, key_shift(key_bits), bins);
     return hipGetLastError();
 }
 
diff --git a/classeq2_amd/csrc/cls_tuning.h b/classeq2_amd/csrc/cls_tuning.h
--- a/classeq2_amd/csrc/cls_tuning.h
+++ b/classeq2_amd/csrc/cls_tuning.h
@@ -8,6 +8,7 @@
     int force_list = 0;
     int no_mask_halves = 0;
     int no_fat_direct = 0;
+    int no_bin_table = 0;
     int no_tile = 0;
     int tile_pass_codes = 0;
     int tile_set_words = 0;
diff --git a/classeq2_amd/engine.py b/classeq2_amd/engine.py
--- a/classeq2_amd/engine.py
+++ b/classeq2_amd/engine.py
@@ -152,6 +152,10 @@
         L.cls_tally_fastq_pairs_text.argtypes = [vp, vp, vp, C.c_char_p, C.c_size_t, C.c_char_p, C.c_size_t, C.POINTER(_abi.Params),
                                                  C.POINTER(_abi.FastqOpts), u32, C.POINTER(u32), C.POINTER(u32)]
         L.cls_tally_fastq_pairs_text.restype = i32
+        L.cls_db_debug_bin_table.argtypes = [C.POINTER(_abi.DbDesc), vp, vp, vp, C.c_uint64]
+        L.cls_db_debug_bin_table.restype = i32
+        L.cls_db_debug_order_bins.argtypes = [vp, vp, vp, u32, i32, vp]
+        L.cls_db_debug_order_bins.restype = i32
         L.cls_fasta_free.argtypes = [C.POINTER(_abi.Fasta)]
         L.cls_fasta_free.restype = None
         L.cls_last_error.restype = C.c_char_p
@@ -275,6 +279,16 @@
     _check(lib().cls_db_validate(C.byref(d)))
 
 
+def debug_bin_table(flat: FlatDb) -> dict:
+    d = flat.desc()
+    n = 1 << (2 * int(d.k_size)) if int(d.k_size) <= 15 else 0
+    meta = np.zeros(_abi.BIN_TABLE_META_WORDS, dtype=np.uint32)
+    direct = np.zeros(n, dtype=np.uint32)
+    bins = np.zeros(n, dtype=np.uint16)
+    _check(lib().cls_db_debug_bin_table(C.byref(d), meta.ctypes.data, direct.ctypes.data, bins.ctypes.data, n))
+    return {"set_bits": int(meta[0]), "canonical": bool(meta[2]), "direct": direct if meta[1] else None, "bins": bins if meta[3] else None}
+
+
 def fasta_parse(text: bytes, device: Optional[int] = None):
     f = _abi.Fasta()
     if device is None:
@@ -510,6 +524,9 @@
         _check(lib().cls_db_set_max_read_len(self._h, n_bases))
         _check(lib().cls_db_info_get(self._h, C.byref(self.info)))
 
+    def debug_order_bins(self, d_bases: int, d_offsets: int, n: int, d_bins: int, from_table: bool) -> None:
+        _check(lib().cls_db_debug_order_bins(self._h, d_bases, d_offsets, n, 1 if from_table else 0, d_bins))
+
     def place_batch_device(self, d_bases: int, d_offsets: int, n: int, d_out: int, params: Optional[_abi.Params] = None,
                            d_stats: int = 0, stream: int = 0) -> None:
         pp = C.byref(params) if params is not None else None
```

Result: faster. 162.1 million (median of 6 runs) (+2.6%).
